# bpp/bpp

Hardware: AMD Instinct MI355X
Metric: MCMC iterations/sec (A00) + site-lnL updates/sec, 10k loci, 1/2/4/8 GPU (higher is better)
Workload: dtype f64; 1 GPU; C2: A00, 10000 loci x 1000 sites, 4 taxa, JC69, 1 rate cat; 10000 loci on rank 0, 5.2 patterns/locus; parallelism=1 GPU, moves=program

## Files before the change

### bpp_amd/api.py

```python
import ctypes as C
import os
import numpy as np

HERE = os.path.dirname(os.path.abspath(__file__))
LIB_PATH = os.path.join(HERE, "libbpp_amd.so")

DATA_DNA, DATA_AA = 0, 1
MODEL_JC69, MODEL_GTR, MODEL_LG = 0, 7, 10
ATTRIB_ARCH_HIP = 1 << 6
SCALE_BUFFER_NONE = -1
PARAM_FREQS, PARAM_SUBST, PARAM_RATES = 1, 2, 4


class BpaError(RuntimeError):
    pass


class Op(C.Structure):
    _fields_ = [("parent_clv", C.c_uint32), ("parent_scaler", C.c_int32),
                ("left_clv", C.c_uint32), ("left_pmatrix", C.c_uint32), ("left_scaler", C.c_int32),
                ("right_clv", C.c_uint32), ("right_pmatrix", C.c_uint32), ("right_scaler", C.c_int32)]


OP_DTYPE = np.dtype([("parent_clv", "<u4"), ("parent_scaler", "<i4"), ("left_clv", "<u4"),
# ... 25 lines not shown
        return _lib
    if not os.path.exists(LIB_PATH):
        raise BpaError(f"{LIB_PATH} is missing: run `python -m bpp_amd.build` (hipcc, gfx950). "
                       "bpp_amd has no CPU fallback.")
    L = C.CDLL(LIB_PATH)
    vp, u, i, d = C.c_void_p, C.c_uint, C.c_int, C.c_double
    dp, up = C.POINTER(C.c_double), C.POINTER(C.c_uint)
    sig = {
        "bpa_version": (C.c_char_p, []),
        "bpa_last_error": (C.c_char_p, []),
        "bpa_experimental_build": (i, []),
        "bpa_device_count": (i, []),
        "bpa_engine_create": (vp, [i, vp]),
        "bpa_engine_destroy": (None, [vp]),
        "bpa_engine_synchronize": (i, [vp]),
        "bpa_engine_set_options": (None, [vp, i, d]),
        "bpa_locus_create": (vp, [vp] + [u] * 11),
        "bpa_locus_destroy": (None, [vp]),
        "bpa_set_tip_states": (i, [vp, u, up, C.c_char_p]),
        "bpa_set_pattern_weights": (None, [vp, up]),
        "bpa_set_frequencies": (None, [vp, u, dp]),
        "bpa_set_subst_params": (None, [vp, u, dp]),
        "bpa_set_category_rates": (None, [vp, dp]),
        "bpa_set_category_weights": (None, [vp, dp]),
        "bpa_set_param_indices": (None, [vp, up]),
        "bpa_set_diploid": (i, [vp, i, C.POINTER(C.c_ulong), C.POINTER(C.c_ulong), C.c_ulong, up]),
        "bpa_map_nt": (up, []),
        "bpa_map_aa": (up, []),
        "bpa_locus_update_matrices": (i, [vp, up, dp, u]),
        "bpa_locus_update_partials": (i, [vp, C.POINTER(Op), u]),
        "bpa_locus_root_loglikelihood": (d, [vp, u, i, up, dp]),
        "bpa_locus_update_all_matrices": (i, [vp, C.POINTER(GTreeView), dp]),
        "bpa_locus_update_all_partials": (i, [vp, C.POINTER(GTreeView)]),
        "bpa_core_update_pmatrix": (i, [vp, C.POINTER(dp), u, u, dp, dp, up, up, C.POINTER(dp),
                                        C.POINTER(dp), C.POINTER(dp), u, u]),
        "bpa_update_eigen": (i, [vp, dp, dp, dp, dp, dp, u]),
        "bpa_compute_gamma_cats": (i, [d, d, u, dp]),
        "bpa_compress_site_patterns": (i, [C.POINTER(C.c_char_p), up, i, C.POINTER(i), i, up]),
        "bpa_locus_get_clv": (i, [vp, u, dp]),
        "bpa_locus_set_clv": (i, [vp, u, dp]),
        "bpa_locus_get_pmatrix": (i, [vp, u, dp]),
        "bpa_locus_set_pmatrix": (i, [vp, u, dp]),
        "bpa_locus_get_scaler": (i, [vp, u, up]),
        "bpa_locus_set_scaler": (i, [vp, u, up]),
        "bpa_locus_get_eigen": (i, [vp, u, dp, dp, dp]),
        "bpa_locus_get_category_rates": (i, [vp, dp]),
        "bpa_plan_create": (vp, [vp, C.POINTER(Batch)]),
        "bpa_plan_destroy": (None, [vp]),
        "bpa_plan_set_lengths": (i, [vp, dp]),
        "bpa_plan_launch": (i, [vp]),
        "bpa_plans_launch": (i, [C.POINTER(vp), u]),
        "bpa_plan_get_lnl": (i, [vp, dp]),
        "bpa_plan_lnl_device": (vp, [vp]),
        "bpa_plan_enable_sum": (i, [vp, vp]),
        "bpa_plan_get_sum": (i, [vp, dp]),
        "bpa_plan_enable_partial_sums": (i, [vp, vp, C.POINTER(C.c_uint)]),
        "bpa_p2p_create": (vp, [vp, i, i, u, vp]),
        "bpa_p2p_connect": (i, [vp, vp]),
        "bpa_p2p_allreduce": (i, [vp, vp, u]),
        "bpa_p2p_status": (i, [vp]),
        "bpa_p2p_set_timeout": (None, [vp, u]),
        "bpa_plans_launch_exchange": (i, [vp, u, vp, vp, u]),
        "bpa_p2p_destroy": (None, [vp]),
        "bpa_batch_evaluate": (i, [vp, C.POINTER(Batch), dp]),
        "bpa_batch_begin": (i, [vp, C.POINTER(Batch)]),
        "bpa_batch_fill": (i, [vp, C.POINTER(Batch), u, u]),
        "bpa_batch_end": (i, [vp, C.POINTER(Batch), dp]),
        "bpa_batch_end_async": (i, [vp, C.POINTER(Batch)]),
        "bpa_batch_wait": (i, [vp, dp]),
        "bpa_engine_stage": (vp, [vp, vp, C.c_size_t]),
        "bpa_plan_set_params": (i, [vp, i, dp]),
        "bpa_plan_set_params_device": (i, [vp, i, vp]),
        "bpa_plan_work": (i, [vp, dp, dp, dp, C.POINTER(C.c_ulong), C.POINTER(C.c_ulong)]),
        "bpa_sampler_create": (vp, [vp, C.POINTER(vp), u, C.c_ulong]),
        "bpa_sampler_destroy": (None, [vp]),
        "bpa_sampler_set_tree": (i, [vp, u, C.POINTER(i), C.POINTER(i), dp, i]),
        "bpa_sampler_set_species_tree": (i, [vp, i, C.POINTER(i), dp, dp]),
        "bpa_sampler_set_tip_species": (i, [vp, u, C.POINTER(i)]),
        "bpa_sampler_set_finetune": (None, [vp, d, d, d, d]),
        "bpa_finetune_onestep": (d, [d, d]),
        "bpa_sampler_adapt_finetune": (i, [vp, dp, dp]),
        "bpa_sampler_burnin": (i, [vp, u, dp]),
        "bpa_burnin_schedule": (u, [u, C.POINTER(u), u]),
        "bpa_sampler_set_tau_prior": (None, [vp, d, d]),
        "bpa_sampler_set_theta_prior": (None, [vp, d, d, d]),
        "bpa_sampler_get_thetas": (i, [vp, dp]),
        "bpa_sampler_set_allreduce": (i, [vp, vp, vp, vp, u]),
        "bpa_sampler_get_taus": (i, [vp, dp]),
        "bpa_sampler_get_tree_msc": (i, [vp, u, C.POINTER(i), dp]),
        "bpa_sampler_initialize": (i, [vp]),
        "bpa_sampler_iterate": (i, [vp, u]),
        "bpa_sampler_get_tree": (i, [vp, u, C.POINTER(i), C.POINTER(i), C.POINTER(i), dp, C.POINTER(i),
                                     C.POINTER(i), C.POINTER(i), dp]),
        "bpa_sampler_summary": (i, [vp, dp, C.POINTER(C.c_ulong), C.POINTER(C.c_ulong), C.POINTER(C.c_ulong)]),
        "bpa_sampler_enable_timing": (i, [vp, u]),
        "bpa_sampler_set_subst_model": (i, [vp, u, dp, dp, d]),
        "bpa_sampler_get_subst_model": (i, [vp, u, dp, dp, dp]),
        "bpa_sampler_set_subst_moves": (None, [vp, d, d, d, d, d]),
        "bpa_sampler_set_locus_rates": (i, [vp, dp]),
        "bpa_sampler_get_locus_rates": (i, [vp, dp, dp]),
        "bpa_sampler_set_locusrate_moves": (i, [vp, d, d, d, d, d, d]),
        "bpa_sampler_locusrate_counters": (i, [vp, C.POINTER(C.c_ulong), C.POINTER(C.c_ulong)]),
        "bpa_sampler_timing": (i, [vp, dp, C.POINTER(C.c_ulong), dp, C.POINTER(C.c_ulong)]),
        "bpa_sampler_work": (i, [vp, dp, C.POINTER(C.c_ulong), C.POINTER(C.c_ulong), C.POINTER(C.c_ulong)]),
        "bpa_sampler_kind": (i, [vp]),
        "bpa_sampler_streams": (i, [vp]),
        "bpa_sampler_set_p2p": (i, [vp, vp, u]),
        "bpa_sampler_set_proposal_kernel": (i, [vp, i]),
        "bpa_sampler_set_program_moves": (i, [vp, i, d]),
        "bpa_sampler_gibbs_counters": (i, [vp, C.POINTER(C.c_ulong), C.POINTER(C.c_ulong)]),
        "bpa_engine_enable_timing": (None, [vp, i]),
        "bpa_engine_set_timing_stride": (None, [vp, u]),
        "bpa_engine_timing": (i, [vp, dp, dp, dp, C.POINTER(C.c_ulong)]),
        "bpa_engine_timing_work": (i, [vp, C.POINTER(C.c_ulong), dp]),
        "bpa_engine_timing_work_codes": (i, [vp, dp]),
        "bpa_plan_work_codes": (i, [vp, dp]),
    }
    for name, (res, args) in sig.items():
        f = getattr(L, name)
        f.restype, f.argtypes = res, args
    _lib = L
    return L


EXPORTED = ["bpa_version", "bpa_last_error", "bpa_experimental_build", "bpa_device_count", "bpa_engine_create",
            "bpa_engine_destroy", "bpa_engine_synchronize", "bpa_engine_set_options",
            "bpa_locus_create", "bpa_locus_destroy", "bpa_set_tip_states",
            "bpa_set_pattern_weights", "bpa_set_frequencies", "bpa_set_subst_params",
            "bpa_set_category_rates", "bpa_set_category_weights", "bpa_set_param_indices",
            "bpa_set_diploid", "bpa_map_nt", "bpa_map_aa", "bpa_locus_update_matrices",
            "bpa_locus_update_partials", "bpa_locus_root_loglikelihood",
            "bpa_locus_update_all_matrices", "bpa_locus_update_all_partials",
            "bpa_core_update_pmatrix", "bpa_update_eigen", "bpa_compute_gamma_cats",
            "bpa_compress_site_patterns", "bpa_locus_get_clv", "bpa_locus_set_clv",
            "bpa_locus_get_pmatrix", "bpa_locus_set_pmatrix", "bpa_locus_get_scaler", "bpa_locus_set_scaler",
            "bpa_locus_get_eigen", "bpa_locus_get_category_rates", "bpa_plan_create", "bpa_plan_destroy", "bpa_plan_set_lengths",
            "bpa_plan_launch", "bpa_plan_get_lnl", "bpa_plan_lnl_device", "bpa_batch_evaluate", "bpa_batch_begin", "bpa_batch_fill", "bpa_batch_end", "bpa_batch_end_async", "bpa_batch_wait",
            "bpa_plan_enable_sum", "bpa_plan_enable_partial_sums", "bpa_plan_get_sum",
            "bpa_p2p_create", "bpa_p2p_connect", "bpa_p2p_allreduce", "bpa_p2p_status", "bpa_p2p_destroy", "bpa_p2p_set_timeout", "bpa_plans_launch_exchange", "bpa_plans_launch",
            "bpa_plan_set_params", "bpa_plan_set_params_device", "bpa_engine_stage",
            "bpa_plan_work", "bpa_engine_enable_timing", "bpa_engine_timing", "bpa_engine_set_timing_stride", "bpa_engine_timing_work", "bpa_engine_timing_work_codes", "bpa_plan_work_codes",
            "bpa_sampler_create", "bpa_sampler_destroy", "bpa_sampler_set_tree", "bpa_sampler_initialize",
            "bpa_sampler_set_species_tree", "bpa_sampler_set_tip_species", "bpa_sampler_set_finetune",
            "bpa_finetune_onestep", "bpa_sampler_adapt_finetune", "bpa_sampler_burnin", "bpa_burnin_schedule",
            "bpa_sampler_set_tau_prior", "bpa_sampler_get_taus", "bpa_sampler_get_tree_msc",
            "bpa_sampler_set_theta_prior", "bpa_sampler_get_thetas", "bpa_sampler_set_allreduce",
            "bpa_sampler_iterate", "bpa_sampler_get_tree", "bpa_sampler_summary",
            "bpa_sampler_enable_timing", "bpa_sampler_timing", "bpa_sampler_work", "bpa_sampler_kind", "bpa_sampler_streams", "bpa_sampler_set_p2p", "bpa_sampler_set_proposal_kernel",
            "bpa_sampler_set_program_moves", "bpa_sampler_gibbs_counters",
            "bpa_sampler_set_subst_model", "bpa_sampler_get_subst_model", "bpa_sampler_set_subst_moves",
            "bpa_sampler_set_locus_rates", "bpa_sampler_get_locus_rates", "bpa_sampler_set_locusrate_moves", "bpa_sampler_locusrate_counters"]


def _err():
    return lib().bpa_last_error().decode()


def _chk(ok):
    if not ok:
        raise BpaError(_err())


def _dp(a):
    return a.ctypes.data_as(C.POINTER(C.c_double))


def _up(a):
    return a.ctypes.data_as(C.POINTER(C.c_uint))


def _f64(a):
    return np.ascontiguousarray(a, dtype=np.float64)


def _u32(a):
    return np.ascontiguousarray(a, dtype=np.uint32)


def map_nt():
    return np.ctypeslib.as_array(lib().bpa_map_nt(), shape=(256,)).copy()


def map_aa():
    return np.ctypeslib.as_array(lib().bpa_map_aa(), shape=(256,)).copy()


def compute_gamma_cats(alpha, beta, categories):
    out = np.zeros(categories)
    _chk(lib().bpa_compute_gamma_cats(alpha, beta, categories, _dp(out)))
    return out


def compress_site_patterns(seqs, dna=True, jc69=False):
    L = lib()
    count, length = len(seqs), len(seqs[0])
    bufs = [C.create_string_buffer(s.encode() if isinstance(s, str) else s, length + 1) for s in seqs]
    arr = (C.c_char_p * count)(*[C.cast(b, C.c_char_p) for b in bufs])
    ln = C.c_int(length)
    w = np.zeros(length, dtype=np.uint32)
    n = L.bpa_compress_site_patterns(arr, L.bpa_map_nt() if dna else L.bpa_map_aa(), count,
                                     C.byref(ln), int(jc69), _up(w))
    if not n:
        raise BpaError("compress_site_patterns failed")
    return [b.raw[:n].decode() for b in bufs], w[:n].copy()


class Engine:

    def __init__(self, device=0, stream=None):
        L = lib()
        self.h = L.bpa_engine_create(device, stream)
        if not self.h:
            raise BpaError(_err())
        self.loci = []

    def set_options(self, usedata=1, bfbeta=1.0):
        lib().bpa_engine_set_options(self.h, int(usedata), float(bfbeta))

    def stage(self, array):
        return _stage(self, array)

    def synchronize(self):
        _chk(lib().bpa_engine_synchronize(self.h))

    def enable_timing(self, on=True, stride=1):
        lib().bpa_engine_set_timing_stride(self.h, int(stride))
        lib().bpa_engine_enable_timing(self.h, int(on))
# ... 617 lines not shown
```

### bpp_amd/csrc/sampler.hpp

```cpp
#pragma once
#include "bpp_amd_host.h"

namespace smp {

constexpr int MAXTIPS = 8;
constexpr int MAXN    = 16;
constexpr int MAXBUF  = 2*(MAXTIPS - 1);
constexpr int MAXPM   = 2*(2*MAXTIPS - 2);
constexpr int MAXPOP  = 16;
constexpr int TPB     = 16;
constexpr int BS      = 64;

struct Tree
{
  int8_t   left[MAXN], right[MAXN], parent[MAXN], clv[MAXN], pmat[MAXN], pop[MAXN];
  double   time[MAXN];
  double   lnl, logpr;
  a00_rng_t rng;
  int32_t  root, tips;
  uint32_t proposals, accepted;
  uint32_t sw_nupd, sw_nbr;
  uint32_t al_nupd, al_nbr, al_neval, pad_;
};
static_assert(sizeof(Tree) % 16 == 0 && offsetof(Tree, lnl) % 16 == 0, "Tree is copied as uint4");
// ... 980 lines not shown
  double * wg_part = nullptr; unsigned long long * stamps = nullptr; int * dec_err = nullptr;
  bool fuse_decision = false;
  DevBuf<int8_t> pop_nc;
  smp::Species sp{};
  bool has_theta[smp::MAXPOP] = {};
  struct Timed { hipEvent_t e0, e1; int kind; };
  std::vector<Timed> timed;
  unsigned timing_stride = 0, timing_phase = 0;
  double timed_ms[2] = {0, 0}; unsigned long timed_n[2] = {0, 0};
  bpa_allreduce_fn allreduce = nullptr;
  void * allreduce_ctx = nullptr;
  double * sum_ext = nullptr;
  unsigned locus_offset = 0;
  std::vector<unsigned> stream_index;
  struct bpa_composite * comp = nullptr;
  std::vector<double> h_taus;
  std::vector<smp::Tree> h_trees;
  bool generic = false;
  std::vector<gsm::GTree> g_trees;
  DevBuf<gsm::GTree> g_dev, g_undo;
  DevBuf<gsm::GLocus> g_loc;
  DevBuf<double> g_lnl, g_lnlcur, g_hast, g_logpr, g_delta, g_site, g_len, g_lograt;
  DevBuf<double> g_t2h3, g_progout;
  DevBuf<gsm::GDecState> g_dst; DevBuf<double> g_dsum; bool gp_dev = false;
  hipEvent_t gp_pace[4] = {nullptr, nullptr, nullptr, nullptr}; unsigned long gp_pace_n = 0;
  unsigned long long gp_seq = 0;
  double * gp_pin = nullptr, * gp_pin_dev = nullptr;
  DevBuf<uint32_t> g_arrive;
  long long gp_k[smp::MAXPOP] = {}; double gp_T[smp::MAXPOP] = {}; bool gp_ok = false, gp_pre_valid = false; double gp_pre_window = 0;
  double gp_tau[smp::MAXPOP] = {}, gp_theta[smp::MAXPOP] = {}; bool gp_mirror = false;
  unsigned long long gp_pj[10] = {}, gp_pj_base[4] = {};
  bool g_split = false, g_forked = false;
  static constexpr int GPARTS = 4;
  unsigned g_np = 1, g_pi[GPARTS + 1] = {}, g_ps[GPARTS + 1] = {}, g_pb[GPARTS + 1] = {}, g_pt[GPARTS + 1] = {};
  hipStream_t g_st[GPARTS] = {nullptr, nullptr, nullptr, nullptr};
  hipEvent_t g_ev_fork = nullptr, g_ev_join[GPARTS] = {nullptr, nullptr, nullptr, nullptr};
  int env_parts = 0;
  DevBuf<uint8_t> g_active;
  DevBuf<uint4> g_recs;
  DevBuf<MatRec2> g_mat2;
  DevBuf<uint32_t> g_bmo;
  unsigned g_units = 0, g_maxmat = 0, g_pend = 0, g_npat = 0, g_rmax = 1, g_pack_epoch = 0;
  bool g_alljc = true;
  bool big = false;
  std::vector<gbig::BTree> b_trees;
  DevBuf<gbig::BTree> b_dev, b_undo;
  DevBuf<uint32_t> b_thr;
  bool g_s20 = false;
  unsigned g_ntiles = 0, g_maxops = 0;
  DevBuf<OpDev> g_ops20;
  DevBuf<uint32_t> g_oprng, g_root20, g_mtask, g_mpm, g_tlocus, g_tpat, g_ttask, g_tn0;
  DevBuf<int32_t> g_rscaler;
  std::vector<double> g_sm_host;
  DevBuf<double> g_sm, g_sm_old;
  DevBuf<uint32_t> g_ids;
  double g_ft[3] = {0, 0, 0}, g_alpha_a = 1, g_alpha_b = 1;
  unsigned g_pend_mode = 0, g_pend_k = 0;
  std::vector<double> g_mui_host;
  gsm::GLrState g_lr_host{1.0, 0.0, 0ull, 0ull};
  DevBuf<double> g_mui, g_mui_old;
  DevBuf<gsm::GLrState> g_lr;
  double g_lr_ft[2] = {0, 0}, g_a_mui = 0, g_a_mubar = 0, g_b_mubar = 0;
  bool g_eigen_dirty = false;
  bool g_level_eval = false;
  bool g_root_stale = false;
  bool g_pm_fused = false;
  unsigned long g_evals = 0;
  unsigned nblocks = 0, epoch = 0;
  bool logpr_stale = false;
  uint32_t env_dbg = 0; int env_gage = -1, env_gspr = -1; bool env_trace = false, env_nomix = false;
  int env_fusea = -1; bool env_noeigfuse = false, env_fusepm = true, env_pmgroup = true, env_hostdec = false, env_rootstore = false; int env_chain = -1, env_pinout = 2;
  long env_inject = 0; uint32_t env_inject_bit = 1024u; long v2_launch_no = 0;
  bool mix_pending = false;
  a00_rng_t grng = 0;
  unsigned long seed = 0, launches = 0, sweeps = 0;
  bool uploaded = false;
  uint32_t h_counters[4] = {0, 0, 0, 0};
  bool host_current = false;
  bool v2_ok = false, env_v1 = false;
  int v2_nt = 0;
  int v2_retries = 0;
  bool v2_prog = false;
  unsigned v2_nwaves = 0, v2_nwg = 0, v2_lwaves = 0;
  size_t v2_lds = 0;
  DevBuf<uint32_t> v2_wave_off;
  DevBuf<smp2::Loc> v2_loc;
  DevBuf<uint2> v2_pat;
  DevBuf<unsigned long long> v2_xbuf;
  DevBuf<a00_rng_t> v2_grng;
  DevBuf<int> v2_err;
  DevBuf<unsigned long long> v2_pj;
  DevBuf<double> v2_prof, v2_declog;
  DevBuf<smp::Species> v2_sp;
  smp::Species v2_sp_sent{};
  struct V2Launch { a00_rng_t grng_before; unsigned chunk; bool mix_pending, logpr_stale; };
  std::vector<V2Launch> v2_log;
  bool kernel_bpp = false, v2_grng_sent = false;
  bpa_p2p * p2p = nullptr;
  unsigned long v2_iters = 0;
};

static bpa_sampler * comp_create(bpa_engine_t * e, bpa_locus_t * const * loci, unsigned nloci, unsigned long seed, bool * plain);
static void comp_destroy(bpa_sampler * s);
static int comp_invalidate(bpa_sampler * s);
static int comp_upload(bpa_sampler * s);
static int comp_set_allreduce(bpa_sampler * s, bpa_allreduce_fn fn, void * ctx, double * device_sum, unsigned first_locus);
static int comp_run(bpa_sampler * s, int what, unsigned n);
static int comp_summary(bpa_sampler * s, double * total_lnl, unsigned long * proposals, unsigned long * accepted, unsigned long * launches);
static int comp_timing(bpa_sampler * s, double * sweep_ms, unsigned long * sweep_launches, double * allloci_ms, unsigned long * allloci_launches);
static int comp_work(bpa_sampler * s, double * bytes, unsigned long * node_updates, unsigned long * pattern_updates, unsigned long * sweeps);
static bpa_sampler * comp_part(bpa_sampler * s, unsigned i, unsigned * j);
static bpa_sampler * comp_part0(bpa_sampler * s);
template <class F> static int comp_each(bpa_sampler * s, F f);
#define COMP_FAIL(msg) do { if (s->comp) return fail(msg); } while (0)

static bpa_sampler * sampler_create_plain(bpa_engine_t * e, bpa_locus_t * const * loci, unsigned nloci, unsigned long seed);
extern "C" bpa_sampler_t * bpa_sampler_create(bpa_engine_t * e, bpa_locus_t * const * loci, unsigned nloci,
                                              unsigned long seed)
{
  if (!e || !loci || !nloci) { fail("bpa_sampler_create: null argument"); return nullptr; }
  std::lock_guard<std::recursive_mutex> lock_(e->mtx);
  bool plain = true;
  bpa_sampler * c = comp_create(e, loci, nloci, seed, &plain);
  if (c || !plain) return c;
  return sampler_create_plain(e, loci, nloci, seed);
}

static bpa_sampler * sampler_create_plain(bpa_engine_t * e, bpa_locus_t * const * loci, unsigned nloci, unsigned long seed)
{
  bpa_sampler * s = new bpa_sampler();
  s->eng = e; s->nloci = nloci; s->seed = seed; s->grng = a00_rng_seed(seed, A00_GLOBAL_STREAM);
  s->sp.theta_slide_prob = 0.1;
  s->loci.assign(loci, loci + nloci);
  bool fits_sweep = !smp_env_generic(), fits_generic = true, all_jc = true, all_kl = true;
  unsigned n20 = 0, nbig = 0;
  const bool force_big = smp_env_big();
  for (unsigned i = 0; i < nloci; ++i)
  {
    const bpa_locus * l = loci[i];
    const bool counts = l && l->eng == e && l->alive && l->tips >= 2 && l->clv_buffers == 2*(l->tips - 1) && l->prob_matrices == 2*(2*l->tips - 2);
    const bool wants_big = counts && l->states == 4 && (force_big || l->tips > (unsigned)gsm::NT || l->scale_buffers != 0 || l->dev.unphased_length);
    if (wants_big)
    {
      if (l->tips > (unsigned)gbig::BT || (l->scale_buffers != 0 && l->scale_buffers != 2*(l->tips - 1)))
      {
        fail("bpa_sampler_create: a locus of the big-tree sampler has <= 64 tips and no or 2 (tips - 1) scale buffers (method.c:4110-4146)");
        delete s; return nullptr;
      }
      ++nbig; s->maxtips = std::max(s->maxtips, l->tips); s->g_rmax = std::max(s->g_rmax, l->rate_cats);
      continue;
    }
    const bool base = counts && (l->states == 4 || l->states == 20) && l->scale_buffers == 0 && !l->dev.unphased_length;
    if (!base)
    {
      fail("bpa_sampler_create: loci must be 4- or 20-state (20-state: without scalers, not diploid), with the buffer counts of method.c:4110-4146");
      delete s; return nullptr;
    }
    if (l->states == 20) { ++n20; fits_sweep = false; fits_generic = fits_generic && l->tips <= (unsigned)gsm::NT && l->rate_cats <= 4; all_jc = false;
                           s->maxtips = std::max(s->maxtips, l->tips); s->g_rmax = std::max(s->g_rmax, l->rate_cats); continue; }
    fits_sweep = fits_sweep && l->rate_cats == 1 && l->dev.model == 0 && l->tips <= (unsigned)smp::MAXTIPS && l->sites <= (unsigned)smp::BS;
    fits_generic = fits_generic && l->tips <= (unsigned)gsm::NT && l->rate_cats <= 8 && l->sites*l->rate_cats < PACK_BS;
    all_jc = all_jc && l->rate_cats == 1 && l->dev.model == 0;
    all_kl = all_kl && l->rate_cats > 1;
    s->maxtips = std::max(s->maxtips, l->tips);
    s->g_rmax = std::max(s->g_rmax, l->rate_cats);
  }
  if (nbig)
  {
    for (unsigned i = 0; i < nloci; ++i)
      if (loci[i]->states != 4 || loci[i]->tips > (unsigned)gbig::BT || (loci[i]->scale_buffers != 0 && loci[i]->scale_buffers != 2*(loci[i]->tips - 1)))
      {
        fail("bpa_sampler_create: the loci of a big-tree sampler are all 4-state with <= 64 tips");
        delete s; return nullptr;
      }
    for (unsigned i = 0; i < nloci; ++i) { s->maxtips = std::max(s->maxtips, loci[i]->tips); s->g_rmax = std::max(s->g_rmax, loci[i]->rate_cats); }
    s->big = true;
    s->b_trees.assign(nloci, gbig::BTree{});
  }
  else if (n20)
  {
    if (n20 != nloci || !fits_generic)
    {
      fail("bpa_sampler_create: 20-state loci go together (no 4-state locus in the same sampler), with <= 16 tips and <= 4 rate categories");
      delete s; return nullptr;
    }
    s->generic = true; s->g_alljc = false; s->g_s20 = true;
    s->g_trees.assign(nloci, gsm::GTree{});
  }
  else if (!fits_sweep)
  {
    if (!fits_generic || !(all_jc || all_kl))
    {
      fail("bpa_sampler_create: beyond the sweep kernel (JC69, 1 rate category, <= 8 tips, <= 64 patterns) the loci must all be JC69 with "
           "one rate category or all have several categories, with <= 16 tips and < 256 patterns x categories");
      delete s; return nullptr;
    }
    s->generic = true; s->g_alljc = all_jc;
    s->g_trees.assign(nloci, gsm::GTree{});
  }
  s->h_trees.assign(nloci, smp::Tree{});
  if (const char * dv = getenv("BPA_SMP_DBG")) s->env_dbg = (uint32_t)atoi(dv);
  if (const char * st = BPA_EXP_SWITCH("BPA_SMP_STEPS")) { unsigned g = 0, q = 0; if (sscanf(st, "%u,%u", &g, &q) == 2) { s->env_gage = (int)g; s->env_gspr = (int)q; } }
  s->env_trace = getenv("BPA_SMP_TRACE") != nullptr; s->env_nomix = BPA_EXP_SWITCH("BPA_SMP_NOMIX") != nullptr;
  if (const char * inj = getenv("BPA_SMP_INJECT")) { s->env_inject = atol(inj); s->env_inject_bit = strstr(inj, ",w") ? 2048u : 1024u; }
  s->fuse_decision = BPA_EXP_SWITCH("BPA_SMP_FUSE") != nullptr;
  { const char * v;
    v = BPA_EXP_SWITCH("BPA_GS_FUSEA");     s->env_fusea = v ? (v[0] == '1' ? 1 : 0) : -1;
    v = BPA_EXP_SWITCH("BPA_GS_FUSEPM");    s->env_fusepm = !(v && v[0] == '0');
    v = BPA_EXP_SWITCH("BPA_S20_PMGROUP");  s->env_pmgroup = !(v && v[0] == '0');
    v = BPA_EXP_SWITCH("BPA_GS_PARTS");    s->env_parts = v ? atoi(v) : 0;
    s->env_noeigfuse = BPA_EXP_SWITCH("BPA_GS_NOEIGFUSE") != nullptr;
    v = getenv("BPA_GS_CHAIN");     s->env_chain = v ? (v[0] != '0' ? 1 : 0) : -1;
    v = BPA_EXP_SWITCH("BPA_GS_PINOUT");    s->env_pinout = v ? (v[0] == '0' ? 0 : v[0] == '1' ? 1 : 2) : 2;
    s->env_hostdec = getenv("BPA_GS_HOSTDEC") != nullptr;
    s->env_rootstore = BPA_EXP_SWITCH("BPA_GS_ROOTSTORE") != nullptr; }
  s->env_v1 = getenv("BPA_SMP_V1") != nullptr;
  s->sp.ft_gage = 0.004; s->sp.ft_gspr = 0.004; s->sp.ft_tau = 0.001; s->sp.ft_mix = 0.3;
  return s;
}

static int sampler_download(bpa_sampler * s);
extern "C" void bpa_sampler_destroy(bpa_sampler_t * s)
{
  if (!s) return;
  std::lock_guard<std::recursive_mutex> lock_(s->eng->mtx);
  if (s->comp) comp_destroy(s);
  (void)set_device(s->eng);
  if (s->generic && s->uploaded && s->g_root_stale && s->g_pack_epoch == s->eng->pack_epoch && !sampler_download(s)) fprintf(stderr, "[bpp_amd] bpa_sampler_destroy: the loci's root buffers could not be brought level (%s)\n", bpa_last_error());
  (void)hipStreamSynchronize(s->eng->stream);
  for (auto & t : s->timed) { (void)hipEventDestroy(t.e0); (void)hipEventDestroy(t.e1); }
  s->blk_task_off.free(); s->lane_rec.free(); s->task_rec.free(); s->flag.free();
  s->counters.free(); s->trees.free(); s->snap.free(); s->mix_delta.free(); s->mix_sum.free(); s->taus.free(); s->pop_t2h.free(); s->theta_sums.free(); s->pop_nc.free(); s->lograt.free(); s->uc.free();
  for (int p_ = 1; p_ < bpa_sampler::GPARTS; ++p_)
  {
    if (s->g_st[p_]) { (void)hipStreamSynchronize(s->g_st[p_]); (void)hipStreamDestroy(s->g_st[p_]); s->g_st[p_] = nullptr; }
    if (s->g_ev_join[p_]) { (void)hipEventDestroy(s->g_ev_join[p_]); s->g_ev_join[p_] = nullptr; }
  }
  if (s->g_ev_fork) { (void)hipEventDestroy(s->g_ev_fork); s->g_ev_fork = nullptr; }
  s->g_t2h3.free(); s->g_progout.free(); s->g_arrive.free(); s->gp_mirror = false; s->g_dst.free(); s->g_dsum.free();
  if (s->gp_pin) { (void)hipHostFree(s->gp_pin); s->gp_pin = s->gp_pin_dev = nullptr; }
  for (auto & ev : s->gp_pace) if (ev) { (void)hipEventDestroy(ev); ev = nullptr; }
  s->g_dev.free(); s->g_undo.free(); s->g_loc.free(); s->g_lnl.free(); s->g_lnlcur.free(); s->g_hast.free(); s->g_logpr.free(); s->g_delta.free(); s->g_site.free();
  s->g_len.free(); s->g_lograt.free(); s->g_active.free(); s->g_recs.free(); s->g_mat2.free(); s->g_bmo.free();
  s->g_sm.free(); s->g_sm_old.free(); s->g_ids.free();
  s->g_mui.free(); s->g_mui_old.free(); s->g_lr.free();
  s->b_dev.free(); s->b_undo.free(); s->b_thr.free();
  s->g_ops20.free(); s->g_oprng.free(); s->g_root20.free(); s->g_mtask.free(); s->g_mpm.free(); s->g_tlocus.free(); s->g_tpat.free(); s->g_ttask.free(); s->g_tn0.free(); s->g_rscaler.free();
  s->v2_wave_off.free(); s->v2_loc.free(); s->v2_pat.free(); s->v2_xbuf.free(); s->v2_grng.free(); s->v2_err.free(); s->v2_prof.free(); s->v2_declog.free(); s->v2_sp.free();
  delete s;
}

static int sampler_download(bpa_sampler * s);
static bool v2_wants_prog(const bpa_sampler * s);
static int sampler_invalidate(bpa_sampler * s)
{
  if (s->uploaded)
  {
    bpa_engine * e = s->eng;
    if (!set_device(e) || !sampler_download(s)) return 0;
    HIPCHK(hipMemcpy(s->h_taus.data(), s->taus.p, s->h_taus.size()*sizeof(double), hipMemcpyDeviceToHost));
    HIPCHK(hipMemcpy(s->h_counters, s->counters.p, sizeof s->h_counters, hipMemcpyDeviceToHost));
  }
  s->uploaded = false; s->host_current = false;
  return 1;
}

template <class TR, int MAXNODES>
static int set_tree_fields(TR & t, int tips, const int * left, const int * right, const double * times, int root, a00_rng_t rng)
{
  const int n = 2*tips - 1;
  std::memset(&t, 0, sizeof(t));
  for (int k = 0; k < MAXNODES; ++k) { t.left[k] = t.right[k] = t.parent[k] = -1; t.clv[k] = t.pmat[k] = (int8_t)k; t.pop[k] = (int8_t)(k < tips ? k : -1); }
  for (int k = 0; k < n; ++k)
  {
    t.left[k] = (int8_t)left[k]; t.right[k] = (int8_t)right[k]; t.time[k] = times[k];
    if ((left[k] < 0) != (k < tips) || (right[k] < 0) != (k < tips) || left[k] >= n || right[k] >= n)
      return fail("bpa_sampler_set_tree: nodes 0..tips-1 are the tips (no children), the others have two");
    if (left[k] >= 0) { t.parent[left[k]] = (int8_t)k; t.parent[right[k]] = (int8_t)k; }
  }
  t.root = root; t.tips = tips; t.rng = rng; t.lnl = 0;
  return 1;
}

static unsigned stream_of(const bpa_sampler * s, unsigned i) { return s->stream_index.empty() ? s->locus_offset + i : s->stream_index[i]; }
static a00_rng_t stream_seed(const bpa_sampler * s, unsigned stream)
{
  const a00_rng_t z = a00_rng_seed(s->seed, stream);
  return s->kernel_bpp ? (a00_rng_t)(unsigned int)(z >> 16) : z;
}

extern "C" int bpa_sampler_set_proposal_kernel(bpa_sampler_t * s, int kind)
{
  std::lock_guard<std::recursive_mutex> lock_(s->eng->mtx);
  if (s->comp && kind != BPA_KERNEL_UNIFORM) return fail("bpa_sampler_set_proposal_kernel: loci of several kinds run the library's own proposal kernel (BPP's lives inside the persistent kernel's single launch)");
  if (s->comp) return 1;
  if (kind != BPA_KERNEL_UNIFORM && kind != BPA_KERNEL_BPP) return fail("bpa_sampler_set_proposal_kernel: BPA_KERNEL_UNIFORM or BPA_KERNEL_BPP");
  if (s->uploaded) return fail("bpa_sampler_set_proposal_kernel: before bpa_sampler_initialize (as a00_set_proposal_kernel)");
  s->kernel_bpp = kind == BPA_KERNEL_BPP;
  for (unsigned i = 0; i < s->nloci; ++i) (s->big ? s->b_trees[i].rng : s->generic ? s->g_trees[i].rng : s->h_trees[i].rng) = stream_seed(s, stream_of(s, i));
  s->grng = stream_seed(s, A00_GLOBAL_STREAM);
  s->v2_grng_sent = false;
  return 1;
}

extern "C" int bpa_sampler_set_program_moves(bpa_sampler_t * s, int on, double slide_prob)
{
  std::lock_guard<std::recursive_mutex> lock_(s->eng->mtx);
  if (s->comp) return on ? fail("bpa_sampler_set_program_moves: loci of several kinds run the library's own moves") : 1;
  if (on && !(slide_prob >= 0 && slide_prob <= 1)) return fail("bpa_sampler_set_program_moves: slide_prob is a probability");
  if (on && !s->kernel_bpp) return fail("bpa_sampler_set_program_moves: the program's moves draw from BPP's proposal kernel (bpa_sampler_set_proposal_kernel(s, BPA_KERNEL_BPP) first)");
  s->sp.program_moves = on ? 1 : 0;
  if (on) s->sp.theta_slide_prob = slide_prob;
  if (s->uploaded && s->v2_ok && v2_wants_prog(s) != s->v2_prog) return sampler_invalidate(s);
  return 1;
}

extern "C" int bpa_sampler_gibbs_counters(bpa_sampler_t * s, unsigned long * proposals, unsigned long * accepted)
{
  std::lock_guard<std::recursive_mutex> lock_(s->eng->mtx);
  if (s->comp) { if (proposals) *proposals = 0; if (accepted) *accepted = 0; return 1; }
  if (!sampler_download(s)) return 0;
  uint32_t c[4];
  HIPCHK(hipMemcpy(c, s->counters.p, sizeof c, hipMemcpyDeviceToHost));
  if (proposals) *proposals = c[2];
  if (accepted) *accepted = c[3];
  return 1;
}

extern "C" int bpa_sampler_set_tree(bpa_sampler_t * s, unsigned i, const int * left, const int * right,
                                    const double * times, int root)
{
  std::lock_guard<std::recursive_mutex> lock_(s->eng->mtx);
  if (s->comp) { unsigned j; bpa_sampler * p = comp_part(s, i, &j); if (!p) return fail("bpa_sampler_set_tree: locus index out of range"); return comp_invalidate(s) && bpa_sampler_set_tree(p, j, left, right, times, root); }
  if (i >= s->nloci) return fail("bpa_sampler_set_tree: locus index out of range");
  const int tips = (int)s->loci[i]->tips;
  const a00_rng_t rng = stream_seed(s, stream_of(s, i));
  if (!sampler_invalidate(s)) return 0;
  if (s->big) return set_tree_fields<gbig::BTree, gbig::BN>(s->b_trees[i], tips, left, right, times, root, rng);
  if (s->generic) return set_tree_fields<gsm::GTree, gsm::NN>(s->g_trees[i], tips, left, right, times, root, rng);
  return set_tree_fields<smp::Tree, smp::MAXN>(s->h_trees[i], tips, left, right, times, root, rng);
}

template <class TR>
static int assign_pops_host(const bpa_sampler * s, TR & t)
{
  const int n = 2*t.tips - 1;
  std::vector<int> order;
  for (int k = t.tips; k < n; ++k) order.push_back(k);
  std::stable_sort(order.begin(), order.end(), [&](int a, int b) { return t.time[a] < t.time[b]; });
  for (int k = 0; k < t.tips; ++k) if (t.pop[k] < 0 || t.pop[k] >= s->sp.S) return fail("bpa_sampler: tip species out of range");
  for (int v : order)
  {
    int c = t.pop[t.left[v]];
    while (!((s->sp.anc[t.pop[t.right[v]]] >> c) & 1u)) c = s->sp.parent[c];
    if (t.time[v] < s->h_taus[c]) return fail("bpa_sampler: a gene-tree node is younger than the divergence of its descendants' species");
    while (s->sp.parent[c] >= 0 && s->h_taus[s->sp.parent[c]] <= t.time[v]) c = s->sp.parent[c];
    t.pop[v] = (int8_t)c;
  }
  return 1;
}
static int gs_upload(bpa_sampler * s);
static int sampler_launch(bpa_sampler * s, unsigned mode, double mix_c, double mix_lnc, unsigned tau_q, double tau_u, double dec_uacc);
static int gs_initialize(bpa_sampler * s);
static int gs_iterate(bpa_sampler * s, unsigned iterations);
static int gs_download(bpa_sampler * s);
static int gb_upload(bpa_sampler * s);
static int gb_initialize(bpa_sampler * s);
static int gb_iterate(bpa_sampler * s, unsigned iterations);
static int gb_download(bpa_sampler * s);

template <int NT> static size_t v2_lds_base(bool prog)
{
  return ((sizeof(smp2::WgLDS<NT>) + 15) & ~(size_t)15) + sizeof(smp2::WaveLDS<NT>)*(size_t)(smp2::Cfg<NT>::WAVES - (prog ? 1 : 0));
}
static bool v2_wants_prog(const bpa_sampler * s)
{
  if (!(s->kernel_bpp && s->sp.program_moves && s->sp.theta_alpha > 0 && s->sp.npop > s->sp.S)) return false;
  for (int p = 0; p < s->sp.npop; ++p) if (s->has_theta[p]) return true;
  return false;
}
static int sampler_upload_v2(bpa_sampler * s, const std::vector<smp::TaskRec> & task_rec)
{
  s->v2_ok = false;
  if (s->env_v1 || s->generic || s->big) return 1;
  const unsigned T = s->nloci;
  const int npop = s->sp.npop;
  if (s->maxtips > 8 || npop > 15) return 1;
  const int NT = (s->maxtips <= 4 && npop <= 7) ? 4 : 8;
  for (unsigned i = 0; i < T; ++i)
  {
    const smp::Tree & t = s->h_trees[i];
    const int n = 2*t.tips - 1, inner = t.tips - 1, edges = 2*t.tips - 2;
    if (t.root != n - 1) return 1;
    for (int k = 0; k < n; ++k)
    {
      if (k < t.tips ? t.clv[k] != k : (t.clv[k] != k && t.clv[k] != k + inner)) return 1;
      if (k != t.root && t.pmat[k] != k && t.pmat[k] != k + edges) return 1;
    }
  }
  const unsigned G = NT == 4 ? 8 : 16, LPW = 64/G, WAVES = NT == 4 ? (unsigned)smp2::Cfg<4>::WAVES : (unsigned)smp2::Cfg<8>::WAVES;
  std::vector<uint32_t> woff{0};
  std::vector<smp2::Loc> loc(T);
  std::vector<uint2> pat;
  unsigned cnt = 0, used = 0;
  for (unsigned t = 0; t < T; ++t)
  {
    const bpa_locus * l = s->loci[t];
    const unsigned np = l->sites, tips = l->tips;
    if (cnt == LPW || used + np > 64u) { woff.push_back(t); cnt = 0; used = 0; }
    ++cnt; used += np;
    smp2::Loc & L = loc[t];
    const smp::TaskRec & r = task_rec[t];
    L.clv = r.clv; L.pmat = r.pmat; L.rate = r.rate; L.rw = r.rw; L.f0 = r.f0; L.f1 = r.f1; L.f2 = r.f2; L.f3 = r.f3;
    L.np = np; L.tips = tips; L.pat_off = (uint32_t)pat.size(); L.pad = 0;
    for (int p = 0; p < 16; ++p) L.gl[p] = r.gl[p];
    for (unsigned n = 0; n < np; ++n)
    {
      uint32_t codes = 0;
      for (unsigned tip = 0; tip < tips; ++tip) codes |= (uint32_t)(l->tipcodes[(size_t)tip*np + n] & 15u) << (4*tip);
      pat.push_back(make_uint2(l->weights[n], codes));
    }
  }
  woff.push_back(T);
  const bool prog = v2_wants_prog(s);
  hipDeviceProp_t prop;
  HIPCHK(hipGetDeviceProperties(&prop, s->eng->device));
  const unsigned nwaves = (unsigned)woff.size() - 1;
  const unsigned LMAX = WAVES - (prog ? 1u : 0u), ncu = (unsigned)std::max(prop.multiProcessorCount, 1);
  unsigned LWAVES = (LMAX > 4u && nwaves <= 4u*ncu) ? 4u : LMAX;
  if (const char * ev = BPA_EXP_SWITCH("BPA_SMP_LWAVES")) { const unsigned v = (unsigned)std::atoi(ev); if (v >= 1 && v <= LMAX) LWAVES = v; }
  const unsigned nwg = (nwaves + LWAVES - 1)/LWAVES;
  const size_t base = NT == 4 ? v2_lds_base<4>(prog) : v2_lds_base<8>(prog);
  const size_t lds_max = std::min<size_t>((size_t)prop.sharedMemPerBlock > 65536 ? (size_t)prop.sharedMemPerBlock : 160*1024, 160*1024) - 256;
  if (base > lds_max) return 1;
  const unsigned per_cu = (unsigned)std::min<size_t>(std::max<size_t>(lds_max/base, 1), 8/WAVES ? 8/WAVES : 1);
  if (nwg > per_cu*(unsigned)prop.multiProcessorCount) return 1;
  s->v2_lds = base;
  s->v2_nt = NT; s->v2_nwaves = nwaves; s->v2_nwg = nwg; s->v2_prog = prog; s->v2_lwaves = LWAVES;
  const int zero2v[3] = {0, 0, 0};
  if (!upload(s->v2_wave_off, woff.data(), woff.size()) || !upload(s->v2_loc, loc.data(), loc.size()) ||
      !upload(s->v2_pat, pat.data(), pat.size()) || !s->v2_xbuf.reserve((size_t)2*smp2::XN) || !s->v2_grng.reserve(1) ||
      !upload(s->v2_err, zero2v, 3) || !s->v2_prof.reserve(40 + (size_t)nwg) || !s->v2_declog.reserve(4*2048) || !s->v2_sp.reserve(1) || !s->v2_pj.reserve(16))
    return 0;
  HIPCHK(hipMemset(s->v2_pj.p, 0, 16*sizeof(unsigned long long)));
  HIPCHK(hipMemset(s->v2_prof.p, 0, (40 + (size_t)nwg)*sizeof(double)));
  {
    void (*k0)(const smp2::Args) = NT == 4 ? smp2::iter_kernel<4, false> : smp2::iter_kernel<8, false>;
    void (*k1)(const smp2::Args) = NT == 4 ? smp2::iter_kernel<4, true> : smp2::iter_kernel<8, true>;
    HIPCHK(hipFuncSetAttribute(reinterpret_cast<const void *>(k0), hipFuncAttributeMaxDynamicSharedMemorySize, (int)s->v2_lds));
    HIPCHK(hipFuncSetAttribute(reinterpret_cast<const void *>(k1), hipFuncAttributeMaxDynamicSharedMemorySize, (int)s->v2_lds));
    void (*k2)(const smp2::Args) = NT == 4 ? smp2::iter_kernel<4, true, true> : smp2::iter_kernel<8, true, true>;
    HIPCHK(hipFuncSetAttribute(reinterpret_cast<const void *>(k2), hipFuncAttributeMaxDynamicSharedMemorySize, (int)s->v2_lds));
  }
  std::memset(&s->v2_sp_sent, 0xff, sizeof s->v2_sp_sent);
  s->v2_ok = true;
  return 1;
}

static int sampler_upload(bpa_sampler * s)
{
  bpa_engine * e = s->eng;
  if (s->uploaded) return 1;
  if (!set_device(e) || !flush(e)) return 0;
  const unsigned T = s->nloci;
  if (!s->sp.npop) return fail("bpa_sampler: set the species tree first (bpa_sampler_set_species_tree)");
  if (s->big) return gb_upload(s);
  if (s->generic) return gs_upload(s);
  for (unsigned i = 0; i < T; ++i) if (!assign_pops_host(s, s->h_trees[i])) return 0;
  for (int p = 0; p < smp::MAXPOP; ++p) s->has_theta[p] = p >= s->sp.S && p < s->sp.npop;
  for (unsigned i = 0; i < T; ++i)
  {
    int cnt[smp::MAXPOP] = {0};
    const smp::Tree & t = s->h_trees[i];
    for (int k = 0; k < t.tips; ++k) if (++cnt[t.pop[k]] >= 2) s->has_theta[t.pop[k]] = true;
  }
  std::vector<uint32_t> blk_off{0};
  std::vector<smp::LaneRec> lane_rec;
  std::vector<smp::TaskRec> task_rec(T);
  const smp::LaneRec idle{0xffffffffu, 0, 0, 0, nullptr, nullptr};
  unsigned used = 0, ntask = 0;
  for (unsigned t = 0; t < T; ++t)
  {
    const bpa_locus * l = s->loci[t];
    const unsigned np = l->sites, tips = l->tips;
    if (used + np > (unsigned)smp::BS || ntask == (unsigned)smp::TPB)
    { lane_rec.resize(blk_off.size()*smp::BS, idle); blk_off.push_back(t); used = 0; ntask = 0; }
    for (unsigned n = 0; n < np; ++n)
    {
      uint32_t codes = 0;
      for (unsigned tip = 0; tip < tips; ++tip) codes |= (uint32_t)(l->tipcodes[(size_t)tip*np + n] & 15u) << (4*tip);
      lane_rec.push_back(smp::LaneRec{t, l->weights[n], codes, n | np << 8 | tips << 16, l->dev.clv + (size_t)n*4, l->dev.pmat});
    }
    used += np; ++ntask;
    smp::TaskRec & r = task_rec[t];
    const double * f = l->par.data() + par_matrix(1, 4, 0) + pm_freqs(4);
    r.clv = l->dev.clv; r.pmat = l->dev.pmat; r.rate = l->par[par_rates(1)]; r.rw = l->par[par_rate_weights(1)];
    r.f0 = f[0]; r.f1 = f[1]; r.f2 = f[2]; r.f3 = f[3];
    const smp::Tree & tr = s->h_trees[t];
    for (int p = 0; p < smp::MAXPOP; ++p) r.gl[p] = r.nin[p] = 0;
    for (unsigned k = 0; k < tips; ++k)
    {
      r.nin[tr.pop[k]]++;
      for (int q = tr.pop[k]; q >= 0; q = s->sp.parent[q]) r.gl[q]++;
    }
  }
  lane_rec.resize(blk_off.size()*smp::BS, idle);
  blk_off.push_back(T);
  s->nblocks = (unsigned)blk_off.size() - 1;
  uint32_t zero2[2] = {0, 0};
  if (!upload(s->blk_task_off, blk_off.data(), blk_off.size()) ||
      !upload(s->lane_rec, lane_rec.data(), lane_rec.size()) || !upload(s->task_rec, task_rec.data(), T) ||
      !upload(s->trees, s->h_trees.data(), T) || !upload(s->snap, s->h_trees.data(), T) ||
      !upload(s->flag, zero2, 1) || !upload(s->counters, s->h_counters, 4) || !s->mix_delta.reserve(T) || !s->mix_sum.reserve(1) ||
      !upload(s->taus, s->h_taus.data(), s->h_taus.size()) || !s->pop_t2h.reserve((size_t)T*smp::MAXPOP) ||
      !s->pop_nc.reserve((size_t)T*smp::MAXPOP) || !s->theta_sums.reserve(smp::MAXPOP) || !s->lograt.reserve(smp::MAXN*smp::MAXN))
    return 0;
  {
    const size_t nb = ((size_t)s->nblocks + 1)*8;
    s->uc.free();
    if (!s->uc.reserve(2*nb + 64)) return fail("bpa_sampler: out of (uncached) device memory");
    s->wg_part = reinterpret_cast<double *>(s->uc.p);
    s->stamps = reinterpret_cast<unsigned long long *>(reinterpret_cast<char *>(s->uc.p) + nb);
    s->dec_err = reinterpret_cast<int *>(reinterpret_cast<char *>(s->uc.p) + 2*nb);
  }
  if (s->allreduce)
  {
    double m[smp::MAXPOP];
    for (int p = 0; p < smp::MAXPOP; ++p) m[p] = s->has_theta[p] ? 1.0 : 0.0;
    double * ar = s->sum_ext ? s->sum_ext : s->theta_sums.p;
    HIPCHK(hipMemcpyAsync(ar, m, sizeof m, hipMemcpyHostToDevice, e->stream));
    if (!s->allreduce(s->allreduce_ctx, ar, (unsigned)smp::MAXPOP, (void *)e->stream)) return fail("bpa_sampler: the all-reduce callback failed");
    HIPCHK(hipMemcpyAsync(m, ar, sizeof m, hipMemcpyDeviceToHost, e->stream));
    HIPCHK(hipStreamSynchronize(e->stream));
    for (int p = 0; p < smp::MAXPOP; ++p) s->has_theta[p] = m[p] > 0.5;
  }
// ... 312 lines not shown
extern "C" int bpa_sampler_get_taus(bpa_sampler_t * s, double * taus)
{
  bpa_engine * e = s->eng;
  std::lock_guard<std::recursive_mutex> lock_(e->mtx);
  if (s->comp) return comp_upload(s) && bpa_sampler_get_taus(comp_part0(s), taus);
  if (!set_device(e)) return 0;
  const size_t np = (size_t)s->sp.npop;
  if (!s->uploaded) { for (size_t i = 0; i < np; ++i) taus[i] = s->h_taus[i]; return (int)np; }
  HIPCHK(hipStreamSynchronize(e->stream));
  HIPCHK(hipMemcpy(taus, s->taus.p, np*sizeof(double), hipMemcpyDeviceToHost));
  return (int)np;
}

extern "C" int bpa_sampler_initialize(bpa_sampler_t * s)
{
  std::lock_guard<std::recursive_mutex> lock_(s->eng->mtx);
  if (s->comp) return comp_run(s, 0, 0);
  if (!sampler_upload(s)) return 0;
  s->host_current = false;
  if (s->big) return gb_initialize(s);
  if (s->generic) return gs_initialize(s);
  return sampler_launch(s, 3, 1.0);
}

static int sampler_sum(bpa_sampler * s)
{
  bpa_engine * e = s->eng;
  double * out = s->sum_ext ? s->sum_ext : s->mix_sum.p;
  hipLaunchKernelGGL(lnl_sum_kernel, dim3(1), dim3(1024), 0, e->stream, s->wg_part, s->nblocks, out);
  HIPCHK(hipGetLastError());
  if (s->allreduce && !s->allreduce(s->allreduce_ctx, out, 1u, (void *)e->stream)) return fail("bpa_sampler: the all-reduce callback failed");
  return 1;
}

static int sampler_decide(bpa_sampler * s, double uacc, int tau_q, int theta_p, double win_u, double mix_c, double mix_lnc)
{
  bpa_engine * e = s->eng;
  s->epoch++;
  if (!s->allreduce)
    hipLaunchKernelGGL(smp::sum_decide_kernel, dim3(1), dim3(1024), 0, e->stream, s->wg_part, s->nblocks, uacc, s->epoch,
                       s->flag.p, s->counters.p, s->taus.p, s->sp, tau_q, theta_p, win_u, mix_c, mix_lnc);
  else
  {
    if (!sampler_sum(s)) return 0;
    hipLaunchKernelGGL(smp::decide_kernel, dim3(1), dim3(1), 0, e->stream, s->sum_ext ? s->sum_ext : s->mix_sum.p, uacc, s->epoch,
                       s->flag.p, s->counters.p, s->taus.p, s->sp, tau_q, theta_p, win_u, mix_c, mix_lnc);
  }
  HIPCHK(hipGetLastError());
  s->launches += s->allreduce ? 2 : 1;
  s->mix_pending = true;
  return 1;
}

extern "C" int bpa_sampler_set_allreduce(bpa_sampler_t * s, bpa_allreduce_fn fn, void * ctx, double * device_sum,
                                         unsigned first_locus)
{
  std::lock_guard<std::recursive_mutex> lock_(s->eng->mtx);
  if (s->comp) return comp_set_allreduce(s, fn, ctx, device_sum, first_locus);
  s->allreduce = fn; s->allreduce_ctx = ctx; s->sum_ext = device_sum;
  if (first_locus != s->locus_offset)
  {
    if (!sampler_invalidate(s)) return 0;
    s->locus_offset = first_locus;
    for (unsigned i = 0; i < s->nloci; ++i)
      (s->big ? s->b_trees[i].rng : s->generic ? s->g_trees[i].rng : s->h_trees[i].rng) = stream_seed(s, first_locus + i);
    s->uploaded = false;
  }
  return 1;
}

static int sampler_iterate_v2(bpa_sampler * s, unsigned iterations, bool in_kernel_allloci)
{
  bpa_engine * e = s->eng;
  const int npop = s->sp.npop, S = s->sp.S;
  uint32_t theta_mask = 0;
  if (s->sp.theta_alpha > 0) for (int p = 0; p < npop; ++p) if (s->has_theta[p]) theta_mask |= 1u << p;
  const bool allloci = in_kernel_allloci && !s->env_nomix;
  const bool program = s->v2_prog;
  const unsigned XV = (unsigned)smp2::XV;
  const bool merged = program;
  const unsigned x_theta = !theta_mask ? 0u : program ? (2u*(unsigned)__builtin_popcount(theta_mask) + (merged ? 5u : 0u) + XV - 1u)/XV : ((unsigned)npop + XV - 1u)/XV;
  const unsigned x_per_iter = allloci ? x_theta + (unsigned)(npop - S) - (merged ? 1u : 0u) + 1u : 0u;
  const unsigned draws_per_iter = allloci ? 2u*(unsigned)__builtin_popcount(theta_mask) + 2u*(unsigned)(npop - S) + 2u : 0u;
  void (*kern)(const smp2::Args) = s->v2_prog   ? (s->v2_nt == 4 ? smp2::iter_kernel<4, true, true> : smp2::iter_kernel<8, true, true>)
                                 : s->kernel_bpp ? (s->v2_nt == 4 ? smp2::iter_kernel<4, true> : smp2::iter_kernel<8, true>)
                                                 : (s->v2_nt == 4 ? smp2::iter_kernel<4, false> : smp2::iter_kernel<8, false>);
  const unsigned bs = s->v2_nt == 4 ? smp2::Cfg<4>::BS : smp2::Cfg<8>::BS;
  while (iterations)
  {
    const unsigned chunk = std::min(iterations, 4096u);
    smp2::Args a{};
    a.wave_off = s->v2_wave_off.p; a.loc = s->v2_loc.p; a.pat = s->v2_pat.p; a.trees = s->trees.p; a.taus = s->taus.p;
    if (s->v2_log.size() >= 65536u && !sampler_download(s)) return 0;
    s->v2_log.push_back({s->grng, chunk, s->mix_pending, s->logpr_stale});
    a.snap = s->snap.p; a.mix_flag = s->flag.p; a.epoch = s->mix_pending ? s->epoch : 0u; a.refresh_logpr = s->logpr_stale ? 1u : 0u;
    s->mix_pending = false; s->logpr_stale = false;
    a.counters = s->counters.p; a.lograt = s->lograt.p; a.pop_nc = s->pop_nc.p; a.pop_t2h = s->pop_t2h.p;
    a.ntasks = s->nloci; a.nwaves = s->v2_nwaves; a.nwg = s->v2_nwg; a.lwaves = s->v2_lwaves; a.xbuf = s->v2_xbuf.p;
    a.err = s->v2_err.p; a.grng = s->v2_grng.p; a.niter = chunk; a.pj = s->v2_pj.p;
    a.nsteps_gage = s->maxtips - 1; a.nsteps_gspr = 2*s->maxtips - 2;
    if (s->env_gage >= 0) { a.nsteps_gage = (uint32_t)s->env_gage; a.nsteps_gspr = (uint32_t)s->env_gspr; }
    a.theta_mask = theta_mask; a.do_allloci = allloci ? 1u : 0u; a.dbg = s->env_dbg;
    if (allloci && ++s->v2_launch_no == s->env_inject) a.dbg |= s->env_inject_bit;
    if (s->p2p && allloci)
    {
      a.peers = s->p2p->d_peer.p; a.mail = s->p2p->mail; a.rank = s->p2p->rank; a.world = s->p2p->world; a.slot_bytes = s->p2p->slot_bytes;
      a.seq0 = s->p2p->seq; a.spin_limit = s->p2p->spin_limit; a.p2p_err = s->p2p->d_err.p;
      s->p2p->seq += (unsigned long long)chunk*x_per_iter;
    }
    else { a.world = 1; a.rank = 0; }
    a.bfbeta = e->usedata ? e->bfbeta : 0.0; a.prof = s->v2_prof.p; a.declog = s->v2_declog.p; a.sp = s->v2_sp.p;
    if (std::memcmp(&s->v2_sp_sent, &s->sp, sizeof(smp::Species)) != 0)
    {
      HIPCHK(hipMemcpyAsync(s->v2_sp.p, &s->sp, sizeof(smp::Species), hipMemcpyHostToDevice, e->stream));
      s->v2_sp_sent = s->sp;
    }
    if (s->env_dbg & 256u) HIPCHK(hipMemsetAsync(s->v2_declog.p, 0, 4*2048*sizeof(double), e->stream));
    if (allloci)
    {
      if (!s->kernel_bpp || !s->v2_grng_sent)
        HIPCHK(hipMemcpyAsync(s->v2_grng.p, &s->grng, sizeof(a00_rng_t), hipMemcpyHostToDevice, e->stream));
      s->v2_grng_sent = true;
      HIPCHK(hipMemsetAsync(s->v2_xbuf.p, 0, (size_t)2*smp2::XN*sizeof(unsigned long long), e->stream));
    }
    if (s->timing_stride && (s->timing_phase++ % s->timing_stride) == 0)
    {
      if (s->timed.size() >= 4096 && !sampler_timing_drain(s)) return 0;
      bpa_sampler::Timed t{nullptr, nullptr, 0};
      HIPCHK(hipEventCreate(&t.e0)); HIPCHK(hipEventCreate(&t.e1));
      hipExtLaunchKernelGGL(kern, dim3(s->v2_nwg), dim3(bs), s->v2_lds, e->stream, t.e0, t.e1, 0, a);
      s->timed.push_back(t);
    }
    else
      hipLaunchKernelGGL(kern, dim3(s->v2_nwg), dim3(bs), s->v2_lds, e->stream, a);
    HIPCHK(hipGetLastError());
    if (!s->kernel_bpp) for (unsigned long k = 0; k < (unsigned long)chunk*draws_per_iter; ++k) (void)a00_rndu(&s->grng);
    s->launches++; s->sweeps += chunk; s->v2_iters += chunk;
    iterations -= chunk;
  }
  return 1;
}

extern "C" int bpa_sampler_set_p2p(bpa_sampler_t * s, bpa_p2p_t * p, unsigned first_locus)
{
  std::lock_guard<std::recursive_mutex> lock_(s->eng->mtx);
  COMP_FAIL("bpa_sampler_set_p2p: loci of several kinds exchange through bpa_sampler_set_allreduce (the mailboxes are read by the persistent kernel's single launch)");
  if (p && (!p->connected || p->eng != s->eng)) return fail("bpa_sampler_set_p2p: connect the exchange first (same engine)");
  if (p && p->nmax < 16u) return fail("bpa_sampler_set_p2p: the mailboxes must hold at least 16 values");
  if (p && (s->generic || s->big)) return fail("bpa_sampler_set_p2p: the in-kernel exchange needs the persistent kernel (JC69 loci of <= 8 tips, <= 64 patterns); use bpa_sampler_set_allreduce");
  if (!sampler_invalidate(s)) return 0;
  s->p2p = p;
  if (first_locus != s->locus_offset)
  {
    s->locus_offset = first_locus;
    for (unsigned i = 0; i < s->nloci; ++i)
    {
      const a00_rng_t r = stream_seed(s, first_locus + i);
      if (s->big) s->b_trees[i].rng = r; else if (s->generic) s->g_trees[i].rng = r; else s->h_trees[i].rng = r;
    }
  }
  return 1;
}

extern "C" int bpa_sampler_iterate(bpa_sampler_t * s, unsigned iterations)
{
  bpa_engine * e = s->eng;
  std::lock_guard<std::recursive_mutex> lock_(e->mtx);
  if (s->comp) return comp_run(s, 1, iterations);
  if (s->generic && (s->g_lr_ft[0] > 0 || s->g_lr_ft[1] > 0) && (s->allreduce || s->p2p))
    return fail("bpa_sampler_iterate: the locus-rate moves run on one rank (an all-reduce callback or the mailboxes are installed: the sum of the rates over the ranks is not exchanged)");
  if (!sampler_upload(s)) return 0;
  s->host_current = false;
  if (s->big) return gb_iterate(s, iterations);
  if (s->generic) return gs_iterate(s, iterations);
  if (s->v2_ok && !s->allreduce && !s->env_trace) return sampler_iterate_v2(s, iterations, true);
  if (s->kernel_bpp) return fail("bpa_sampler: BPP's proposal kernel runs in the persistent iteration kernel only (one GPU, or several with bpa_sampler_set_p2p)");
  const bool v2_sweep = s->v2_ok && !s->env_trace;
  const bool fused = s->fuse_decision && !s->allreduce && !s->env_trace;
  for (unsigned it = 0; it < iterations; ++it)
  {
    if (v2_sweep) { if (!sampler_iterate_v2(s, 1, false)) return 0; }
    else
    {
      if (!sampler_launch(s, 0, 1.0)) return 0;
      s->sweeps++;
    }
    if (s->env_nomix) continue;
    if (s->sp.theta_alpha > 0)
    {
      smp::ThetaArgs ta{};
      for (int p = 0; p < s->sp.npop; ++p)
        if (s->has_theta[p]) { ta.on[p] = 1u; ta.win_u[p] = a00_rndu(&s->grng); ta.uacc[p] = a00_rndu(&s->grng); }
      if (!s->allreduce)
        hipLaunchKernelGGL(smp::theta_sum_decide_kernel, dim3(s->sp.npop), dim3(1024), 0, e->stream, s->pop_nc.p, s->pop_t2h.p,
                           s->nloci, s->taus.p, s->sp, ta, s->counters.p, (double *)nullptr, (const double *)nullptr, 1);
      else
      {
        hipLaunchKernelGGL(smp::theta_sum_decide_kernel, dim3(s->sp.npop), dim3(1024), 0, e->stream, s->pop_nc.p, s->pop_t2h.p,
                           s->nloci, s->taus.p, s->sp, ta, s->counters.p, s->theta_sums.p, (const double *)nullptr, 0);
        double * ar = s->sum_ext ? s->sum_ext : s->theta_sums.p;
        const size_t nb = (size_t)s->sp.npop*sizeof(double);
        if (ar != s->theta_sums.p) HIPCHK(hipMemcpyAsync(ar, s->theta_sums.p, nb, hipMemcpyDeviceToDevice, e->stream));
        if (!s->allreduce(s->allreduce_ctx, ar, (unsigned)s->sp.npop, (void *)e->stream)) return fail("bpa_sampler: the all-reduce callback failed");
        if (ar != s->theta_sums.p) HIPCHK(hipMemcpyAsync(s->theta_sums.p, ar, nb, hipMemcpyDeviceToDevice, e->stream));
        hipLaunchKernelGGL(smp::theta_sum_decide_kernel, dim3(s->sp.npop), dim3(1024), 0, e->stream, s->pop_nc.p, s->pop_t2h.p,
                           s->nloci, s->taus.p, s->sp, ta, s->counters.p, (double *)nullptr, (const double *)s->theta_sums.p, 1);
      }
      s->logpr_stale = true;
      HIPCHK(hipGetLastError());
      s->launches += 1;
    }
    for (int q = s->sp.S; q < s->sp.npop; ++q)
    {
      const double uprop = a00_rndu(&s->grng), uacc_t = a00_rndu(&s->grng);
      if (fused)
      {
        if (!sampler_launch(s, 4, 1.0, 0.0, (unsigned)q, uprop, uacc_t)) return 0;
        s->epoch++; s->mix_pending = true;
        continue;
      }
      if (!sampler_launch(s, 4, 1.0, 0.0, (unsigned)q, uprop)) return 0;
      if (!sampler_decide(s, uacc_t, q, -1, uprop, 1.0, 0.0)) return 0;
    }
    const double lnc = s->sp.ft_mix*(a00_rndu(&s->grng) - 0.5), c = std::exp(lnc);
    const double uacc = a00_rndu(&s->grng);
    if (fused)
    {
      if (!sampler_launch(s, 1, c, lnc, 0, 0.0, uacc)) return 0;
      s->epoch++; s->mix_pending = true;
      continue;
    }
    if (!sampler_launch(s, 1, c, lnc)) return 0;
    if (!sampler_decide(s, uacc, -1, -1, 0.0, c, lnc)) return 0;
  }
  return 1;
}

static int sampler_download(bpa_sampler * s)
{
  bpa_engine * e = s->eng;
  if (!sampler_upload(s)) return 0;
  if (s->host_current) return 1;
  if (s->big) { if (!gb_download(s)) return 0; s->host_current = true; return 1; }
  if (s->generic) { if (!gs_download(s)) return 0; s->host_current = true; return 1; }
  if (!sampler_launch(s, 2, 1.0)) return 0;
  HIPCHK(hipMemcpyAsync(s->h_trees.data(), s->trees.p, s->nloci*sizeof(smp::Tree), hipMemcpyDeviceToHost, e->stream));
  HIPCHK(hipStreamSynchronize(e->stream));
  int err = 0;
  HIPCHK(hipMemcpy(&err, s->dec_err, sizeof err, hipMemcpyDeviceToHost));
  if (err) return fail("bpa_sampler: an in-launch decision timed out waiting for a workgroup's sum (BPA_SMP_FUSE is set: unset it)");
  if (s->v2_ok)
  {
    if (s->env_dbg & 16u)
    {
      double pr[16]; HIPCHK(hipMemcpy(pr, s->v2_prof.p, sizeof pr, hipMemcpyDeviceToHost));
      fprintf(stderr, "[smp2] cycles of lane 0 of workgroup 0, last launch: propose %.0f evaluate %.0f decide %.0f theta %.0f tau %.0f mix %.0f | exchange: theta %.0f tau+mix %.0f | inside the exchanges: first barrier %.0f sums %.0f barrier %.0f arrival + poll %.0f last barrier %.0f | of theta / tau / mix: the decision's arithmetic after the totals %.0f %.0f, MIX's re-draws inside the wait %.0f\n",
              pr[0], pr[1], pr[2], pr[3], pr[4], pr[5], pr[6], pr[7], pr[8], pr[9], pr[10], pr[11], pr[12], pr[13], pr[14], pr[15]);
      double p2[24]; HIPCHK(hipMemcpy(p2, s->v2_prof.p + 16 + s->v2_nwg, sizeof p2, hipMemcpyDeviceToHost));
      fprintf(stderr, "[smp2] sweep cycles of the waves of workgroup 0:");
      for (int w = 0; w < 8; ++w) fprintf(stderr, " %.0f", p2[8 + w]);
      fprintf(stderr, "\n");
      if (s->v2_prog)
        fprintf(stderr, "[smp2] (program-moves kernel: the numbers above are the control wave's — before B1 | wait for the loci | push | poll | THETA decision | TAU decisions | MIX decision | next proposal)\n");
    }
    if (s->env_dbg & 256u)
    {
      std::vector<double> r(4*2048); HIPCHK(hipMemcpy(r.data(), s->v2_declog.p, r.size()*sizeof(double), hipMemcpyDeviceToHost));
      for (unsigned k = 1000; k < 2048; ++k) if (r[4*k] != 0) fprintf(stderr, "[smp2dbg] %u: %g %.17g %.17g %.17g\n", k, r[4*k], r[4*k+1], r[4*k+2], r[4*k+3]);
      for (unsigned k = 0; k < 1000 && r[4*k] != 0; ++k)
        fprintf(stderr, "[smp2] %s %d lnacc %.17g u %.17g -> %d\n", r[4*k] >= 300 ? "mix" : r[4*k] >= 200 ? "tau" : "theta",
                (int)r[4*k] % 100, r[4*k + 1], r[4*k + 2], (int)r[4*k + 3]);
    }
    if (s->env_dbg & 32u)
    {
      std::vector<double> w(s->v2_nwg); HIPCHK(hipMemcpy(w.data(), s->v2_prof.p + 16, w.size()*sizeof(double), hipMemcpyDeviceToHost));
      double mn = 1e300, mx = 0, sm = 0; unsigned imx = 0;
      for (unsigned i = 0; i < w.size(); ++i) { mn = std::min(mn, w[i]); if (w[i] > mx) { mx = w[i]; imx = i; } sm += w[i]; }
      fprintf(stderr, "[smp2] sweep cycles per workgroup, last launch: min %.0f mean %.0f max %.0f (workgroup %u of %u)\n", mn, sm/w.size(), mx, imx, s->v2_nwg);
    }
    int verr[3] = {0, 0, 0};
    HIPCHK(hipMemcpy(verr, s->v2_err.p, sizeof verr, hipMemcpyDeviceToHost));
    err = verr[0];
    if (!err && s->p2p) { HIPCHK(hipMemcpy(&err, s->p2p->d_err.p, sizeof err, hipMemcpyDeviceToHost)); if (err) return fail("bpa_sampler: the exchange between the GPUs timed out inside the persistent kernel (a rank is missing or slow; install an all-reduce callback instead)"); }
    if (err)
    {
      const int zero2[2] = {0, 0};
      HIPCHK(hipMemcpy(s->v2_err.p, zero2, sizeof zero2, hipMemcpyHostToDevice));
      if (s->p2p || verr[1] <= 0) return fail("bpa_sampler: the persistent iteration kernel timed out waiting for a workgroup's sum (is the device shared? BPA_SMP_V1=1 selects one launch per step)");
      fprintf(stderr, "[bpp_amd] the persistent iteration kernel timed out waiting for a workgroup (is the device shared?): %d iterations are run again\n", verr[1]);
      {
        long left = verr[1];
        while (left > 0 && !s->v2_log.empty())
        {
          const bpa_sampler::V2Launch l = s->v2_log.back(); s->v2_log.pop_back();
          left -= (long)l.chunk;
          s->launches--; s->sweeps -= l.chunk; s->v2_iters -= l.chunk;
          if (!s->kernel_bpp) s->grng = l.grng_before;
          s->mix_pending = l.mix_pending; s->logpr_stale = l.logpr_stale;
        }
        if (left != 0) return fail("bpa_sampler: the persistent kernel reports iterations it did not run that no launch of the log accounts for");
      }
      s->v2_log.clear();
      if (++s->v2_retries > 3)
      {
        if (s->kernel_bpp) return fail("bpa_sampler: the persistent iteration kernel keeps timing out (a shared device: its workgroups must all be resident at once) and BPP's proposal kernel has no other path");
        s->v2_ok = false;
      }
      if (!bpa_sampler_iterate(s, (unsigned)verr[1])) return 0;
      return sampler_download(s);
    }
    s->v2_retries = 0; s->v2_log.clear();
    if (verr[2])
    {
      const int z = 0;
      HIPCHK(hipMemcpy(s->v2_err.p + 2, &z, sizeof z, hipMemcpyHostToDevice));
      return fail("bpa_sampler: an all-loci step was ACCEPTED with a locus's term of 256 log units or more in its sum (the coarse companion accumulator: 2^-10 resolution); the chain is not to be trusted from there on");
    }
  }
  s->host_current = true;
  return 1;
}

extern "C" int bpa_sampler_get_tree(bpa_sampler_t * s, unsigned i, int * left, int * right, int * parent,
                                    double * times, int * clv, int * pmat, int * root, double * lnl)
{
  std::lock_guard<std::recursive_mutex> lock_(s->eng->mtx);
  if (s->comp) { unsigned j; bpa_sampler * p = comp_part(s, i, &j); if (!p) return fail("bpa_sampler_get_tree: locus index out of range"); return comp_upload(s) && bpa_sampler_get_tree(p, j, left, right, parent, times, clv, pmat, root, lnl); }
  if (i >= s->nloci) return fail("bpa_sampler_get_tree: locus index out of range");
  if (!sampler_download(s)) return 0;
  auto out = [&](const auto & t)
  {
    const int n = 2*t.tips - 1;
    for (int k = 0; k < n; ++k)
    {
      if (left) left[k] = t.left[k]; if (right) right[k] = t.right[k]; if (parent) parent[k] = t.parent[k];
      if (times) times[k] = t.time[k]; if (clv) clv[k] = t.clv[k]; if (pmat) pmat[k] = t.pmat[k];
    }
    if (root) *root = t.root;
    if (lnl) *lnl = t.lnl;
  };
  if (s->big) out(s->b_trees[i]); else if (s->generic) out(s->g_trees[i]); else out(s->h_trees[i]);
  return 1;
}

// ... 104 lines not shown
```

### bpp_amd/csrc/sweep2.hpp

```cpp
#pragma once

namespace smp2 {

using smp::Tree; using smp::Species; using smp::ByteArr; using smp::MAXPOP; using smp::MAXN;
using smp::rndu; using smp::reflect; using smp::msc_term; using smp::nth_bit; using smp::Op; using smp::make_op;

template <int NT> struct Cfg
{
  static constexpr int G     = NT <= 4 ? 8 : NT <= 8 ? 16 : 32;
  static constexpr int LPW   = 64/G;
  static constexpr int NN    = 2*NT;
  static constexpr int W     = NN/4;
  static constexpr int NBUF  = 2*(NT - 1);
  static constexpr int NPM   = 2*(2*NT - 2);
#ifndef SMP2_WAVES
#define SMP2_WAVES 8
#endif
  static constexpr int WAVES = NT <= 4 ? SMP2_WAVES : 4;
  static constexpr int BS    = 64*WAVES;
  static_assert(G == NN, "lane i of a group is node i");
};

struct Loc
{
  double * clv, * pmat;
  double rate, rw, f0, f1, f2, f3;
  uint32_t np, tips, pat_off, pad;
  int8_t gl[16];
};

struct Args
{
  const uint32_t * wave_off;
  const Loc * loc;
  const uint2 * pat;
  Tree * trees;
  const Tree * snap; const uint32_t * mix_flag; uint32_t epoch, refresh_logpr;
  double * taus;
  uint32_t * counters;
  const double * lograt;
  int8_t * pop_nc; double * pop_t2h;
  uint32_t ntasks, nwaves, nwg;
  uint32_t lwaves;
  unsigned long long * xbuf;
  int * err;
  a00_rng_t * grng;
  uint32_t niter, nsteps_gage, nsteps_gspr, theta_mask, do_allloci, dbg;
  double bfbeta;
  double * prof, * declog;
  unsigned char * const * peers; unsigned char * mail; int32_t rank, world; unsigned long long slot_bytes, seq0, spin_limit; int * p2p_err;
  const Species * sp;
  unsigned long long * pj;
};

constexpr int XN = 128;
constexpr int XV = 15;

template <int NT> struct Slot
{
  double time[Cfg<NT>::NN];
  double ab[Cfg<NT>::NPM][2];
  double contrib[Cfg<NT>::G], contrib_new[Cfg<NT>::G];
  double rate, rw, f[4];
};
template <int NT> struct WaveLDS
{
  double clv[Cfg<NT>::NBUF][64][4];
  double term[64];
  uint2  pat[64];
  Slot<NT> slot[Cfg<NT>::LPW];
};
struct PopFit { double k, T, a, b, c; };
struct Redraw { double tn, l2t, T, a, b, c; };
struct WgBase
{
  double tau[3*MAXPOP];
  double xtot[32];
  Species sp;
  struct { unsigned long long grng; uint32_t accm, rd_mask, acc_step, run_ok; double lnacc_step, lnacc_theta; double tn[16], l2t[16], lnacc[16]; } dec;
  PopFit pf[16];
  Redraw rd[16];
  struct { int32_t q, mix; double tq_old, tq_lo, tq_hi, tq_new, minf, maxf, lminf, lmaxf, mix_c, mix_lnc; } stepp;
};
template <int NT> struct WgLDS : WgBase
{
  double lograt[(2*NT)*(2*NT)];
  unsigned long long accfx[32];
  uint32_t anc[16];
  uint32_t abort_, bad_, xbad_, coarse_;
  unsigned long long xprev[2][XN];
  long long prof[24];
  long long wsweep[16];
  uint32_t xcoarse_, late_;
};

template <int G> __device__ __forceinline__ uint32_t gballot(bool p, uint32_t gbase)
{
  return (uint32_t)(__ballot(p) >> gbase) & (G >= 32 ? 0xffffffffu : ((1u << (G & 31)) - 1u));
}
__device__ __forceinline__ void wsync()
{
  __builtin_amdgcn_fence(__ATOMIC_ACQ_REL, "wavefront");
  __builtin_amdgcn_wave_barrier();
}

template <int NT> struct GTree
{
  ByteArr<Cfg<NT>::W> left, right, parent, pop;
  uint32_t cf, pf;
  int32_t root, tips;
  __device__ __forceinline__ int cidx(int i) const { return i + (((cf >> i) & 1u) ? tips - 1 : 0); }
  __device__ __forceinline__ int pidx(int i) const { return i + (((pf >> i) & 1u) ? 2*tips - 2 : 0); }
};

__device__ __forceinline__ uint32_t splat(int v) { return (uint32_t)(v & 0xff)*0x01010101u; }
__device__ __forceinline__ uint32_t byte_eq(uint32_t w, uint32_t s)
{
  const uint32_t x = w ^ s;
  const uint32_t z = ~(((x & 0x7f7f7f7fu) + 0x7f7f7f7fu) | x | 0x7f7f7f7fu);
  return (z - (z >> 7)) | z;
}
template <int NT> __device__ __forceinline__ void swap_ids(GTree<NT> & t, double * time, int a, int b)
{
  constexpr int W = Cfg<NT>::W;
  const uint32_t sa = splat(a), sb = splat(b), x = sa ^ sb;
#pragma unroll
  for (int k = 0; k < W; ++k)
  {
    t.left.w[k]   ^= x & (byte_eq(t.left.w[k], sa)   | byte_eq(t.left.w[k], sb));
    t.right.w[k]  ^= x & (byte_eq(t.right.w[k], sa)  | byte_eq(t.right.w[k], sb));
    t.parent.w[k] ^= x & (byte_eq(t.parent.w[k], sa) | byte_eq(t.parent.w[k], sb));
  }
  const int la = t.left[a], ra = t.right[a], pa = t.parent[a], qa = t.pop[a];
  const int lb = t.left[b], rb = t.right[b], pb = t.parent[b], qb = t.pop[b];
  t.left.set(a, lb); t.right.set(a, rb); t.parent.set(a, pb); t.pop.set(a, qb);
  t.left.set(b, la); t.right.set(b, ra); t.parent.set(b, pa); t.pop.set(b, qa);
  const double ta = time[a], tb = time[b];
  time[a] = tb; time[b] = ta;
  t.root = t.root == a ? b : t.root == b ? a : t.root;
}
template <int NT> __device__ __forceinline__ uint32_t path_mask(const GTree<NT> & t, int v)
{
  uint32_t m = 0;
#pragma unroll
  for (int d = 0; d < NT; ++d) { if (v >= 0) { m |= 1u << v; v = t.parent[v]; } }
  return m;
}

struct PopLane
{
  double tau, ptau, theta, l2t;
  int32_t parent;
  uint32_t anc, below;
};

struct Prop { uint32_t chain, brm, ndm; double hast; };

template <bool BPP> struct Stream
{
  a00_rng_t r;
  __device__ __forceinline__ double u()
  {
    if (!BPP) return rndu(&r);
    uint32_t z = (uint32_t)r*69069u + 1u;
    if (z == 0u) z = 12345671u;
    r = z;
    return (double)z*(1.0/4294967296.0);
  }
  __device__ __forceinline__ double window()
  {
    if (!BPP) return rndu(&r) - 0.5;
    const double uu = u() - 0.5;
    const double rr = log(1 - 2*fabs(uu))*0.70710678118654752440;
    const double lap = uu >= 0 ? -rr : rr;
    double v = 0.90 + lap*sqrt(1 - 0.90*0.90);
    if (u() < 0.5) v = -v;
// ... 287 lines not shown
    wg.dec.lnacc[lane] = lnacc_p; wg.dec.l2t[lane] = l2_p;
    if (apply_now && ((accm >> lane) & 1u)) { wg.tau[MAXPOP + lane] = tn; wg.tau[2*MAXPOP + lane] = l2_p; }
  }
  if (lane == 0) { wg.dec.accm = accm; wg.dec.run_ok = run_ok ? 1u : 0u; }
  __builtin_amdgcn_fence(__ATOMIC_ACQ_REL, "wavefront");
  __builtin_amdgcn_wave_barrier();
  return z;
}

__device__ __forceinline__ uint32_t prog_tau_decide(uint32_t z, uint32_t theta_mask, int q, int base, double lnacc0, bool prefit = false)
{
  WgBase & wg = wg_base();
  const uint32_t lane = threadIdx.x & 63u, pl16 = lane & 15u, role = lane >> 4;
  const double qnan = prog_qnan();
  constexpr double FX = 1099511627776.0, FXC = 1024.0;
  double lnacc = (wg.xtot[base] + wg.xtot[base + 1]*(FX/FXC)) + lnacc0;
  const int cl = wg.sp.left[q], cr = wg.sp.right[q];
  const bool run_ok = wg.dec.run_ok != 0u;
  const PopFit f = wg.pf[pl16];
  const bool aff = lane < 16u && ((int)lane == q || (int)lane == cl || (int)lane == cr);
  const bool have = aff && ((theta_mask >> pl16) & 1u) && run_ok;
  const double Cn = have ? wg.xtot[base + ((int)lane == q ? 2 : (int)lane == cl ? 3 : 4)] : qnan;
  double fa = qnan, fb = qnan, tn = qnan, l2t = 0;
  if (prefit) { if (have && Cn == Cn) { fa = wg.rd[pl16].a; fb = wg.rd[pl16].b; } }
  else if (have && Cn == Cn) a00_theta_conditional_invgamma_fast(wg.sp.theta_alpha, wg.sp.theta_beta, (long)f.k, Cn, &fa, &fb);
  const uint32_t rd_mask = (uint32_t)__ballot(have && fa == fa && f.a == f.a) & 0xffffu;
  double xl;
  const double s_fa = __shfl(fa, (int)pl16, 64), s_fb = __shfl(fb, (int)pl16, 64);
  const double g = draw_gammas(z, lane, (unsigned long long)q | ((unsigned long long)cl << 4) | ((unsigned long long)cr << 8), 3, rd_mask, fa, role == 1u ? s_fb : s_fa, xl);
  const double lb = __shfl(xl, 16 + (int)pl16, 64), la = __shfl(xl, 32 + (int)pl16, 64);
  const double c1 = fa*lb - lgamma_with_log(fa, la);
  if (lane < 16u && ((rd_mask >> pl16) & 1u)) tn = 1.0/(g/fb);
  const double x = redraw_ratio(wg, lane, f.k, tn, fa, fb, c1, Cn, f.a, f.b, f.c, f.T, l2t);
  for (int j = 0; j < 3; ++j)
  {
    const int p = j == 0 ? q : j == 1 ? cl : cr;
    if (!((theta_mask >> p) & 1u)) continue;
    const double xp = __shfl(x, p, 64);
    lnacc += run_ok && ((rd_mask >> p) & 1u) ? xp : qnan;
  }
  const bool accept = lnacc >= -1e-10 || prog_lcg(z) < exp(lnacc);
  if (lane < 16u) { Redraw & r = wg.rd[lane]; r.tn = tn; r.l2t = l2t; r.T = Cn; r.a = fa; r.b = fb; r.c = c1; }
  if (lane == 0) { wg.dec.acc_step = accept ? 1u : 0u; wg.dec.rd_mask = rd_mask; wg.dec.lnacc_step = lnacc; }
  __builtin_amdgcn_fence(__ATOMIC_ACQ_REL, "wavefront");
  __builtin_amdgcn_wave_barrier();
  return z;
}

__device__ __forceinline__ uint32_t prog_mix_redraw(uint32_t z, uint32_t theta_mask, double mix_c)
{
  WgBase & wg = wg_base();
  const uint32_t lane = threadIdx.x & 63u, pl16 = lane & 15u, role = lane >> 4;
  const int npop = wg.sp.npop, pm = (int)pl16;
  const double qnan = prog_qnan();
  const bool run_ok = wg.dec.run_ok != 0u;
  const PopFit f = wg.pf[pl16];
  const bool have = lane < 32u && pm < npop && ((theta_mask >> pm) & 1u) && run_ok;
  const double Ts = f.T*mix_c;
  double fa = qnan, fb = qnan, tn = qnan, l2t = 0;
  if (have) a00_theta_conditional_invgamma_fast(wg.sp.theta_alpha, wg.sp.theta_beta, (long)f.k, role == 0u ? Ts : Ts/mix_c, &fa, &fb);
  const double fao = __shfl(fa, 16 + pm, 64), fbo = __shfl(fb, 16 + pm, 64);
  const uint32_t rd_mask = (uint32_t)__ballot(lane < 16u && have && fa == fa && fao == fao) & 0xffffu;
  double xl;
  const double s_fa = __shfl(fa, pm, 64), s_fb = __shfl(fb, pm, 64);
  const double g = draw_gammas(z, lane, 0xfedcba9876543210ull, npop, rd_mask, fa, role == 1u ? s_fb : role == 2u ? s_fa : fbo, xl);
  const double lb = __shfl(xl, 16 + pm, 64), la = __shfl(xl, 32 + pm, 64), lbo = __shfl(xl, 48 + pm, 64), lao = log(fao);
  const double c1 = fa*lb - lgamma_with_log(fa, la), co = fao*lbo - lgamma_with_log(fao, lao);
  if (lane < 16u && ((rd_mask >> pl16) & 1u)) tn = 1.0/(g/fb);
  const double x = redraw_ratio(wg, lane, f.k, tn, fa, fb, c1, Ts, fao, fbo, co, f.T, l2t);
  double lnacc_theta = 0;
  for (int p = 0; p < npop; ++p)
    if ((theta_mask >> p) & 1u)
    {
      const double xp = __shfl(x, p, 64);
      lnacc_theta += run_ok && ((rd_mask >> p) & 1u) ? xp : qnan;
    }
  if (lane < 16u) { Redraw & r = wg.rd[lane]; r.tn = tn; r.l2t = l2t; r.T = Ts; r.a = fa; r.b = fb; r.c = c1; }
  if (lane == 0) { wg.dec.rd_mask = rd_mask; wg.dec.lnacc_theta = lnacc_theta; }
  __builtin_amdgcn_fence(__ATOMIC_ACQ_REL, "wavefront");
  __builtin_amdgcn_wave_barrier();
  return z;
}

template <int NT, bool BPP, bool PROG = false>
__global__ void __launch_bounds__(Cfg<NT>::BS) iter_kernel(const Args A)
{
  using C = Cfg<NT>;
  constexpr int G = C::G, LPW = C::LPW, NN = C::NN, W = C::W, NBUF = C::NBUF, NPM = C::NPM, WAVES = C::WAVES;
  extern __shared__ __attribute__((aligned(16))) unsigned char smem[];
  WgLDS<NT> & wg = *reinterpret_cast<WgLDS<NT> *>(smem);
  WaveLDS<NT> * wl_all = reinterpret_cast<WaveLDS<NT> *>(smem + ((sizeof(WgLDS<NT>) + 15) & ~(size_t)15));
  const uint32_t tid = threadIdx.x, wv = tid >> 6, lane = tid & 63u, b = blockIdx.x;
  const int li = (int)(lane & (uint32_t)(G - 1)); const uint32_t gbase = lane - (uint32_t)li, slot = lane/(uint32_t)G;
  WaveLDS<NT> & wl = wl_all[PROG ? (wv ? wv - 1u : 0u) : wv];
  Slot<NT> & S = wl.slot[slot];
  const uint32_t lw = PROG ? wv - 1u : wv;
  const uint32_t gw = lw < A.lwaves ? b*A.lwaves + lw : 0xffffffffu;
  {
    const uint32_t * src = reinterpret_cast<const uint32_t *>(A.sp);
    uint32_t * dst = reinterpret_cast<uint32_t *>(&wg.sp);
    for (uint32_t i = tid; i < sizeof(Species)/4; i += C::BS) dst[i] = src[i];
    if (tid < 24u) wg.prof[tid] = 0;
    if (tid < 16u) wg.wsweep[tid] = 0;
  }
  __syncthreads();
  const Species & SP = wg.sp;
  const int npop = SP.npop, nsp = SP.S;

  for (uint32_t i = tid; i < (uint32_t)(3*MAXPOP); i += C::BS) wg.tau[i] = A.taus[i];
  for (uint32_t i = tid; i < (uint32_t)((2*NT)*(2*NT)); i += C::BS) wg.lograt[i] = A.lograt[(i/(2*NT))*MAXN + i % (2*NT)];
  if (tid < 16u) wg.anc[tid] = tid < (uint32_t)MAXPOP ? (uint32_t)SP.anc[tid] : 0u;
  if (tid == 0) { wg.abort_ = __hip_atomic_load(A.err, __ATOMIC_RELAXED, __HIP_MEMORY_SCOPE_AGENT) != 0 ? 2u : 0u; wg.late_ = 0; wg.bad_ = 0; wg.xbad_ = 0; wg.coarse_ = 0; wg.xcoarse_ = 0; }
  if (tid < 32u) wg.accfx[tid] = 0ull;
  for (uint32_t i = tid; i < 2u*XN; i += C::BS) (&wg.xprev[0][0])[i] = 0ull;
  PopLane pl;
  {
    pl.parent = li < npop ? (int)SP.parent[li < MAXPOP ? li : 0] : -1;
    pl.anc = li < npop ? (uint32_t)SP.anc[li < MAXPOP ? li : 0] : 0u;
    uint32_t below = 0;
    for (int q2 = 0; q2 < npop; ++q2) if (q2 != li && (((uint32_t)SP.anc[q2] >> li) & 1u)) below |= 1u << q2;
    pl.below = li < npop ? below : 0u;
  }
  __syncthreads();
  if (wg.abort_ == 2u)
  {
    if (b == 0 && tid == 0) (void)atomicAdd(A.err + 1, (int)A.niter);
    return;
  }
  auto load_pop = [&]()
  {
    const int i = li < MAXPOP ? li : 0;
    pl.tau = wg.tau[i]; pl.theta = wg.tau[MAXPOP + i]; pl.l2t = wg.tau[2*MAXPOP + i];
    pl.ptau = pl.parent >= 0 ? wg.tau[pl.parent] : -1.0;
  };
  load_pop();
  Stream<BPP> grng{*A.grng};

  const bool prof_on = (A.dbg & 16u) && b == 0 && tid == 0;
  long long pf_t = prof_on ? clock64() : 0;
#define SMP2_TICK(i_) do { if (prof_on) { const long long t1_ = clock64(); wg.prof[i_] += t1_ - pf_t; pf_t = t1_; } } while (0)
  long long pf_s = 0;
#define SMP2_SUB0() do { if (prof_on) pf_s = clock64(); } while (0)
#define SMP2_SUB(i_) do { if (prof_on) wg.prof[i_] += clock64() - pf_s; } while (0)

  constexpr double FX = 1099511627776.0;
  constexpr double FXC = 1024.0;
  auto fx_add = [&](int v, double x, bool coarse)
  {
    if (fabs(x) < 256.0)
      (void)__hip_atomic_fetch_add(&wg.accfx[v], (unsigned long long)__double2ll_rn(x*FX), __ATOMIC_RELAXED, __HIP_MEMORY_SCOPE_WORKGROUP);
    else if (coarse && fabs(x) < 274877906944.0)
    {
      wg.coarse_ = 1u;
      (void)__hip_atomic_fetch_add(&wg.accfx[v + 1], (unsigned long long)__double2ll_rn(x*FXC), __ATOMIC_RELAXED, __HIP_MEMORY_SCOPE_WORKGROUP);
    }
    else wg.bad_ = 1u;
  };
  uint32_t nx = 0;
  unsigned long long gseq = A.seq0;
#define XT(i_) do { if (prof_on) { const long long t1_ = clock64(); wg.prof[8 + i_] += t1_ - xt0; xt0 = t1_; } } while (0)
  long long xt0 = 0;
  constexpr bool solo = PROG;
  auto xpush = [&](int v0, int nv)
  {
    const uint32_t par = nx & 1u; ++nx;
    unsigned long long * acc = A.xbuf + (size_t)par*XN + (size_t)(b & 7u)*16u;
    if (tid < (uint32_t)nv)
    {
      const unsigned long long fx = wg.accfx[v0 + (int)tid];
      wg.accfx[v0 + (int)tid] = 0ull;
      const unsigned long long old = __hip_atomic_fetch_add(acc + tid, fx, __ATOMIC_RELAXED, __HIP_MEMORY_SCOPE_AGENT);
      asm volatile("s_waitcnt vmcnt(0)" :: "v"(old) : "memory");
    }
    XT(1);
    if (!solo) __syncthreads();
    XT(2);
    if (tid == 0) (void)__hip_atomic_fetch_add(acc + XV, 1ull + ((unsigned long long)wg.bad_ << 32) + ((unsigned long long)wg.coarse_ << 48), __ATOMIC_RELAXED, __HIP_MEMORY_SCOPE_AGENT);
  };
  auto xpoll = [&](int v0, int nv, bool last, bool hold) -> bool
  {
    const uint32_t par = (nx - 1u) & 1u;
    unsigned long long * set = A.xbuf + (size_t)par*XN;
    if (wv == 0)
    {
      const unsigned long long t_wait = wall_clock64();
      const unsigned long long prev0 = wg.xprev[par][lane], prev1 = wg.xprev[par][64u + lane];
// ... 90 lines not shown
    if (hold || solo)
    {
      if (wv == 0 && nval > XV && wg.xbad_) { if (lane < (uint32_t)nval) wg.xtot[lane] = __longlong_as_double(0x7ff8000000000000ll); wsync(); }
      return true;
    }
    if (nval > XV && wg.xbad_)
    {
      __syncthreads();
      if (tid < (uint32_t)nval) wg.xtot[tid] = __longlong_as_double(0x7ff8000000000000ll);
      __syncthreads();
    }
    mine_tot = wg.xtot[want & 31];
    return true;
  };
  auto exchange = [&](int nval, int want, double & mine_tot) -> bool
  {
    exchange_begin(nval);
    return exchange_end(want, mine_tot);
  };
#undef XT

  if constexpr (PROG)
  {
    if (wv == 0)
    {
      Stream<true> g{*A.grng};
      const uint32_t tm = A.theta_mask;
      const int nth = 2*__popc(tm);
      const double qnan = __longlong_as_double(0x7ff8000000000000ll);
      uint32_t cnt_prop = 0, cnt_acc = 0, cnt_gprop = 0, cnt_gacc = 0, ndec = 0;
      uint32_t pj_tau = 0, pj_tau_acc = 0, pj_mix = 0, pj_mix_acc = 0;
      const bool declog = (A.dbg & 256u) && b == 0;
      int q = -1; bool mix = false;
      double tq_old = 0, tq_new = 0, mix_c = 1, mix_lnc = 0, lnprior = 0;
      auto make_step = [&](int stepq)
      {
        mix = stepq == npop; q = mix ? -1 : stepq;
        const double wprop = g.window();
        double tq_lo = 0, tq_hi = 0, minf = 1, maxf = 1, lminf = 0, lmaxf = 0;
        tq_old = 0; tq_new = 0; mix_c = 1; mix_lnc = 0; lnprior = 0;
        if (!mix)
        {
          const int pq = SP.parent[q], cl = SP.left[q], cr = SP.right[q];
          tq_old = wg.tau[q]; tq_lo = fmax(wg.tau[cl], wg.tau[cr]); tq_hi = pq >= 0 ? wg.tau[pq] : 999.0;
          tq_new = reflect(tq_old + SP.ft_tau*wprop, tq_lo, tq_hi);
          minf = (tq_new - tq_lo)/(tq_old - tq_lo); maxf = (tq_new - tq_hi)/(tq_old - tq_hi);
          const double lg = log(lane == 0 ? minf : lane == 1u ? maxf : tq_new/tq_old);
          lminf = __shfl(lg, 0, 64); lmaxf = __shfl(lg, 1, 64);
          if (pq < 0 && SP.tau_alpha > 0) lnprior = (SP.tau_alpha - 1 - (nsp - 1) + 1)*__shfl(lg, 2, 64) - SP.tau_beta*(tq_new - tq_old);
        }
        else { mix_lnc = SP.ft_mix*wprop; mix_c = exp(mix_lnc); }
        if (lane == 0)
        {
          wg.stepp.q = q; wg.stepp.mix = mix ? 1 : 0; wg.stepp.tq_old = tq_old; wg.stepp.tq_lo = tq_lo; wg.stepp.tq_hi = tq_hi; wg.stepp.tq_new = tq_new;
          wg.stepp.minf = minf; wg.stepp.maxf = maxf; wg.stepp.lminf = lminf; wg.stepp.lmaxf = lmaxf; wg.stepp.mix_c = mix_c; wg.stepp.mix_lnc = mix_lnc;
        }
      };
      uint32_t slidem = 0; double tslide = 0;
      auto theta_choices = [&]()
      {
        slidem = 0; tslide = 0;
        for (int p = 0; p < npop; ++p)
          if ((tm >> p) & 1u)
          {
            if (!(g.u() < SP.theta_slide_prob)) continue;
            slidem |= 1u << p;
            const double tn = reflect(wg.tau[MAXPOP + p] + SP.ft_theta*g.window(), 0.0, 999.0);
            if (p == (int)lane) tslide = tn;
          }
      };
      bool aborted = false;
      if (A.do_allloci && A.niter) { make_step(nsp); theta_choices(); }
      __syncthreads();
      for (uint32_t it = 0; it < A.niter && A.do_allloci && !aborted; ++it)
      {
        for (int stepq = nsp; stepq <= npop && !aborted; ++stepq)
        {
          const bool first = stepq == nsp;
          const int base = first ? nth : 0;
          if (mix) { SMP2_SUB0(); g.r = prog_mix_redraw((uint32_t)g.r, tm, mix_c); SMP2_SUB(15); }
          SMP2_TICK(0);
          __syncthreads();
          SMP2_TICK(1);
          double dummy = 0;
          exchange_begin(base + (mix ? 2 : 5));
          SMP2_TICK(2);
          const bool okx = exchange_end(0, dummy);
          SMP2_TICK(3);
          if (!okx) { aborted = true; __syncthreads(); __syncthreads(); break; }
          bool accept = false; double lnacc = 0; uint32_t rd_mask = 0;
          if (first)
          {
            g.r = prog_theta_decide((uint32_t)g.r, tm, slidem, tslide, 1, q, base);
            const uint32_t accm = wg.dec.accm;
            cnt_prop += (uint32_t)__popc(tm); cnt_acc += (uint32_t)__popc(accm);
            cnt_gprop += (uint32_t)__popc(tm & ~slidem); cnt_gacc += (uint32_t)__popc(accm & tm & ~slidem);
            if (declog && lane < (uint32_t)npop && ((tm >> lane) & 1u))
            {
              const uint32_t k = ndec + (uint32_t)__popc(tm & ((1u << lane) - 1u));
              if (k < 1000u) { double * r = A.declog + 4*k; r[0] = (((slidem >> lane) & 1u) ? 100 : 200) + (int)lane; r[1] = wg.dec.lnacc[lane]; r[2] = -1.0; r[3] = (accm >> lane) & 1u ? 1 : 0; }
            }
            ndec += (uint32_t)__popc(tm);
            SMP2_TICK(4);
          }
          if (!mix)
          {
            g.r = prog_tau_decide((uint32_t)g.r, tm, q, base, lnprior, first);
            accept = wg.dec.acc_step != 0u; rd_mask = wg.dec.rd_mask; lnacc = wg.dec.lnacc_step;
          }
          else
          {
            lnacc = (wg.xtot[0] + wg.xtot[1]*(FX/FXC)) + (double)(nsp - 1)*mix_lnc;
            if (SP.tau_alpha > 0)
            {
              const double troot = wg.tau[npop - 1];
              lnacc += (SP.tau_alpha - 1)*mix_lnc - SP.tau_beta*(troot*mix_c - troot) - (double)(nsp - 2)*mix_lnc;
            }
            lnacc += wg.dec.lnacc_theta; rd_mask = wg.dec.rd_mask;
            accept = g.accept(lnacc);
            if (lane == 0) wg.dec.acc_step = accept ? 1u : 0u;
          }
          if (accept && wg.xcoarse_ && b == 0 && lane == 0) (void)atomicAdd(A.err + 2, 1);
          ++cnt_prop; cnt_acc += accept ? 1u : 0u;
          if (mix) { ++pj_mix; pj_mix_acc += accept ? 1u : 0u; } else { ++pj_tau; pj_tau_acc += accept ? 1u : 0u; }
          if (declog && lane == 0 && ndec < 1000u) { double * r = A.declog + 4*ndec; r[0] = mix ? 300 : 200 + q; r[1] = lnacc; r[2] = -1.0; r[3] = accept ? 1 : 0; }
          ++ndec;
          if (accept)
          {
            if (!mix) { if (lane == 0) wg.tau[q] = tq_new; }
            else if (lane < (uint32_t)npop) wg.tau[lane] *= mix_c;
            if (lane < 16u)
            {
              const Redraw r = wg.rd[lane];
              if ((rd_mask >> lane) & 1u) { wg.tau[MAXPOP + lane] = r.tn; wg.tau[2*MAXPOP + lane] = r.l2t; }
              const bool moved = mix ? lane < (uint32_t)npop && ((tm >> lane) & 1u)
                                     : ((tm >> lane) & 1u) && ((int)lane == q || (int)lane == SP.left[q] || (int)lane == SP.right[q]);
              if (moved) { PopFit & f = wg.pf[lane]; f.T = r.T; f.a = r.a; f.b = r.b; f.c = r.c; }
            }
          }
          wsync();
          if (mix) SMP2_TICK(6); else SMP2_TICK(5);
          SMP2_TICK(7);
          __syncthreads();
          if (stepq < npop) make_step(stepq + 1);
          else if (it + 1 < A.niter) { make_step(nsp); theta_choices(); }
          __syncthreads();
        }
      }
      if (!aborted)
      {
        if (lane == 0) wg.late_ = __hip_atomic_load(A.err, __ATOMIC_ACQUIRE, __HIP_MEMORY_SCOPE_AGENT) != 0 ? 1u : 0u;
        __syncthreads();
        if (wg.late_) { aborted = true; if (b == 0 && lane == 0) (void)atomicAdd(A.err + 1, (int)A.niter); }
      }
      if (b == 0)
      {
        if (lane == 0 && !aborted)
        {
          *A.grng = g.r;
          A.counters[0] += cnt_prop; A.counters[1] += cnt_acc; A.counters[2] += cnt_gprop; A.counters[3] += cnt_gacc;
          A.pj[4] += pj_tau; A.pj[5] += pj_tau_acc; A.pj[6] += pj_mix; A.pj[7] += pj_mix_acc;
          A.pj[8] += (cnt_prop - pj_tau - pj_mix) - cnt_gprop; A.pj[9] += (cnt_acc - pj_tau_acc - pj_mix_acc) - cnt_gacc;
        }
        if (!aborted && lane < (uint32_t)(3*MAXPOP)) A.taus[lane] = wg.tau[lane];
        if (prof_on) for (int i = 0; i < 24; ++i) A.prof[(i < 16 ? 0 : (int)A.nwg) + i] = (double)wg.prof[i];
        if (prof_on) for (int i = 0; i < 16; ++i) A.prof[(int)A.nwg + 24 + i] = (double)wg.wsweep[i];
      }
      return;
    }
  }

  const uint32_t t0 = gw < A.nwaves ? A.wave_off[gw] : 0u, nt = gw < A.nwaves ? A.wave_off[gw + 1] - t0 : 0u;
  const bool act = slot < nt;
  const uint32_t task = t0 + (act ? slot : 0u);
  GTree<NT> T;
  Stream<BPP> rng{0};
  double lnl_cur = 0, logpr_cur = 0;
  uint32_t np = 0, pb = 0, nprop_done = 0, nacc = 0, w_nupd = 0, w_nbr = 0, a_nupd = 0, a_nbr = 0, a_neval = 0;
  int gl_i = 0;
  for (int k = 0; k < W; ++k) { T.left.w[k] = T.right.w[k] = T.parent.w[k] = T.pop.w[k] = 0xffffffffu; }
  T.cf = T.pf = 0; T.root = 0; T.tips = 2;
  if (act && nt)
  {
    const Loc & L = A.loc[task];
    const uint32_t flag_now = __hip_atomic_load(A.mix_flag, __ATOMIC_RELAXED, __HIP_MEMORY_SCOPE_AGENT);
    const bool restore_mix = A.epoch != 0u && flag_now == A.epoch;
    const Tree * trp = A.trees + task;
    if (restore_mix) trp = A.snap + task;
    const Tree & tr = *trp;
    const Tree & cur = A.trees[task];
    np = L.np;
    double * g_pmat = L.pmat;
    if (li == 0) { S.rate = L.rate; S.rw = L.rw; S.f[0] = L.f0; S.f[1] = L.f1; S.f[2] = L.f2; S.f[3] = L.f3; }
    gl_i = L.gl[li & 15];
    for (int k = 0; k < W; ++k)
    {
      T.left.w[k] = reinterpret_cast<const uint32_t *>(tr.left)[k]; T.right.w[k] = reinterpret_cast<const uint32_t *>(tr.right)[k];
      T.parent.w[k] = reinterpret_cast<const uint32_t *>(tr.parent)[k]; T.pop.w[k] = reinterpret_cast<const uint32_t *>(tr.pop)[k];
    }
    T.root = tr.root; T.tips = tr.tips; rng.r = cur.rng; lnl_cur = tr.lnl; logpr_cur = tr.logpr;
    const int n = 2*T.tips - 1;
    T.cf = gballot<G>(li >= T.tips && li < n && tr.clv[li] != li, gbase);
    T.pf = gballot<G>(li < n && tr.pmat[li] != li, gbase);
    S.time[li] = li < n ? tr.time[li] : 0.0;
    for (uint32_t i = (uint32_t)li; i < (uint32_t)(4*(2*T.tips - 2)); i += G) (&S.ab[0][0])[i] = g_pmat[i];
  }
  {
    uint32_t acc = 0;
#pragma unroll
    for (int s2 = 0; s2 < LPW; ++s2)
    {
      const uint32_t n2 = (uint32_t)__builtin_amdgcn_readlane((int)np, s2*G);
      if ((uint32_t)s2 == slot) pb = acc;
      acc += n2;
    }
  }
  if (act)
  {
    const Loc & L = A.loc[task];
    const double * g_clv = L.clv;
    for (uint32_t q = (uint32_t)li; q < np; q += G) wl.pat[pb + q] = A.pat[L.pat_off + q];
    const uint32_t nbuf = 2u*(uint32_t)(T.tips - 1);
    for (uint32_t i = (uint32_t)li; i < nbuf*np; i += G)
    {
      const uint32_t c = i/np, q = i - c*np;
      const double2 * src = reinterpret_cast<const double2 *>(g_clv + ((size_t)c*np + q)*4);
      const double2 u = src[0], w = src[1];
      double * d = wl.clv[c][pb + q];
      d[0] = u.x; d[1] = u.y; d[2] = w.x; d[3] = w.y;
    }
  }
  const int tips = T.tips, n = 2*tips - 1;
  const bool inner_i = li >= tips && li < n;

  uint32_t mync = 0; double t2h_cur = 0, t2h_new = 0;
  uint32_t mynodes = 0, mync_new = 0; int mynin_new = 0;
  Op opw[NT - 1]; int nops = 0;
  for (int k = 0; k < NT - 1; ++k) opw[k] = 0;

  auto density_counts = [&]()
  {
    const int pop_i = T.pop[li];
    int below = 0;
#pragma unroll
    for (int q = 0; q < G - 1; ++q)
    {
      const uint32_t m = gballot<G>(inner_i && pop_i == q, gbase);
      if (li == q) mynodes = m;
      below += ((pl.below >> q) & 1u) ? __popc(m) : 0;
    }
    mync_new = (uint32_t)__popc(mynodes);
    mynin_new = gl_i - below;
  };
  auto density_term = [&](const double * tk)
  {
    uint32_t nodes = mynodes;
    const int ncoal = (int)mync_new, nin = mynin_new;
    int steps = ncoal + (pl.ptau >= 0 ? 1 : 0);
    if (nin == steps) --steps;
    double T2h = 0, prev = pl.tau;
    int nn = nin;
#pragma unroll
    for (int k = 0; k < NT; ++k)
      if (k < steps)
      {
        double tkk = pl.ptau;
        if (k < ncoal)
        {
          int best = -1; double tb = 0;
#pragma unroll
          for (int j = 0; j < NT - 1; ++j)
            if (((nodes >> (tips + j)) & 1u) && (best < 0 || tk[j] < tb)) { best = tips + j; tb = tk[j]; }
          tkk = tb; nodes &= ~(1u << best);
        }
        T2h += nn*(nn - 1)*(tkk - prev);
        prev = tkk; --nn;
      }
    double c = 0;
    if (ncoal) c += ncoal*pl.l2t;
    if (T2h) c -= T2h/(pl.theta*1.0);
    S.contrib_new[li] = c; t2h_new = T2h;
  };
  auto evaluate = [&](const Prop & pr, bool with_lnl, double & lp_new) -> double
  {
    double tk[NT - 1];
#pragma unroll
    for (int j = 0; j < NT - 1; ++j) tk[j] = S.time[(tips + j) & (NN - 1)];
    const double myage = S.time[li];
    density_counts();
    if ((pr.chain >> li) & 1u) density_term(tk);
    T.pf ^= pr.brm; T.cf ^= pr.ndm;
    if ((pr.brm >> li) & 1u)
    {
      const int par = T.parent[li];
      const double len = (S.time[par & (NN - 1)] - myage)*1.0;
      double a_, b_;
      jc69_ab(len, S.rate, a_, b_);
      const int pi = T.pidx(li);
      S.ab[pi][0] = a_; S.ab[pi][1] = b_;
    }
    nops = __popc(pr.ndm);
    {
      int rank = 0;
#pragma unroll
      for (int j = 0; j < NT - 1; ++j)
        rank += (((pr.ndm >> (tips + j)) & 1u) && (tk[j] < myage || (tk[j] == myage && tips + j < li))) ? 1 : 0;
      const bool mine = (pr.ndm >> li) & 1u;
#pragma unroll
      for (int k = 0; k < NT - 1; ++k)
        if (k < nops)
        {
          const int x = __ffs(gballot<G>(mine && rank == k, gbase)) - 1;
          const int l = T.left[x], r = T.right[x];
          opw[k] = make_op(T.cidx(x), T.cidx(l), T.pidx(l), T.cidx(r), T.pidx(r));
        }
    }
    wsync();
    double lnl = 0;
    if (with_lnl)
    {
      for (uint32_t base = 0; base < np; base += G)
      {
        const uint32_t q = base + (uint32_t)li; const bool pact = q < np;
        const uint32_t ps = pb + (pact ? q : 0u);
        const uint2 pi = wl.pat[ps];
        double last[4] = {0, 0, 0, 0}; uint32_t last_c = 0xffffffffu;
#pragma unroll
        for (int k = 0; k < NT - 1; ++k)
          if (k < nops)
          {
            const Op o = opw[k];
            const uint32_t opar = (uint32_t)o & 255u, lc = (uint32_t)(o >> 8) & 255u, lp = (uint32_t)(o >> 16) & 255u,
                           rc = (uint32_t)(o >> 24) & 255u, rp = (uint32_t)(o >> 32) & 255u;
            double lv[4], rv[4], x[4], y[4];
            if (lc < (uint32_t)tips) expand_code((pi.y >> (4*lc)) & 15u, lv);
            else if (lc == last_c) { lv[0] = last[0]; lv[1] = last[1]; lv[2] = last[2]; lv[3] = last[3]; }
            else { const double * c = wl.clv[lc - tips][ps]; lv[0] = c[0]; lv[1] = c[1]; lv[2] = c[2]; lv[3] = c[3]; }
            if (rc < (uint32_t)tips) expand_code((pi.y >> (4*rc)) & 15u, rv);
            else if (rc == last_c) { rv[0] = last[0]; rv[1] = last[1]; rv[2] = last[2]; rv[3] = last[3]; }
            else { const double * c = wl.clv[rc - tips][ps]; rv[0] = c[0]; rv[1] = c[1]; rv[2] = c[2]; rv[3] = c[3]; }
            matvec4_ab(S.ab[lp][0], S.ab[lp][1], lv, x);
            matvec4_ab(S.ab[rp][0], S.ab[rp][1], rv, y);
            last[0] = x[0]*y[0]; last[1] = x[1]*y[1]; last[2] = x[2]*y[2]; last[3] = x[3]*y[3]; last_c = opar;
            if (pact) { double * out = wl.clv[opar - tips][ps]; out[0] = last[0]; out[1] = last[1]; out[2] = last[2]; out[3] = last[3]; }
          }
        const double tr_ = dot4_pair(S.f[0], S.f[1], S.f[2], S.f[3], last);
        if (pact) wl.term[ps] = log(0 + tr_*S.rw)*pi.x;
      }
      wsync();
      for (uint32_t base = 0; base < np; base += 8)
      {
        double v[8];
#pragma unroll
        for (int j = 0; j < 8; ++j) v[j] = base + (uint32_t)j < np ? wl.term[pb + base + (uint32_t)j] : 0.0;
#pragma unroll
        for (int j = 0; j < 8; ++j) lnl += v[j];
      }
      lnl = A.bfbeta == 1.0 ? lnl : A.bfbeta == 0.0 ? 0.0 : A.bfbeta*lnl;
    }
    else wsync();
    double lp = 0;
    {
      double v[G];
#pragma unroll
      for (int p = 0; p < G; ++p) v[p] = p < npop ? (((pr.chain >> p) & 1u) ? S.contrib_new[p] : S.contrib[p]) : 0.0;
#pragma unroll
      for (int p = 0; p < G; ++p) lp += v[p];
    }
    lp_new = lp;
    return lnl;
  };
  auto commit_density = [&](uint32_t chain)
  {
    if ((chain >> li) & 1u) { S.contrib[li] = S.contrib_new[li]; t2h_cur = t2h_new; }
    mync = mync_new;
  };

  const uint32_t allpop = (1u << npop) - 1u;
  if (act)
  {
    wsync();
    double tk[NT - 1];
#pragma unroll
    for (int j = 0; j < NT - 1; ++j) tk[j] = S.time[(tips + j) & (NN - 1)];
    density_counts();
    if (li < npop) density_term(tk);
    commit_density(allpop);
    wsync();
    if (A.refresh_logpr)
    {
      double lp = 0;
      for (int p = 0; p < npop; ++p) lp += S.contrib[p];
      logpr_cur = lp;
    }
  }

  const double qnan = __longlong_as_double(0x7ff8000000000000ll);
  uint32_t cnt_prop = 0, cnt_acc = 0;
  uint32_t cnt_gprop = 0, cnt_gacc = 0;
  uint32_t pj_tau = 0, pj_tau_acc = 0, pj_mix = 0, pj_mix_acc = 0, pj_gage = 0, pj_gage_acc = 0;
  const bool declog = (A.dbg & 256u) && b == 0;
  uint32_t ndec = 0;
  const bool wgprof = (A.dbg & 32u) && tid == 0;
  long long wg_sweep = 0;
  bool aborted = false;

  if constexpr (PROG) __syncthreads();
  for (uint32_t it = 0; it < A.niter && !aborted; ++it)
  {
    const uint32_t nprop = A.nsteps_gage + A.nsteps_gspr;
    const long long wg_t0 = wgprof ? clock64() : 0;
    const bool wvprof = (A.dbg & 16u) && b == 0 && lane == 0;
    const long long wv_t0 = wvprof ? clock64() : 0;
    for (uint32_t step = 0; step < nprop; ++step)
    {
      const GTree<NT> U = T;
      double tsave = 0, lnl = 0, lp_new = 0;
      Prop pr{0, 0, 0, 0.0};
      bool ok = false;
      if (act)
      {
        tsave = S.time[li];
        ok = step < A.nsteps_gage
          ? propose_gage<NT, BPP>(T, rng, S.time, (int)step, pl, wg.anc, wg.tau, SP.ft_gage, li, gbase, pr)
          : propose_gspr<NT, BPP>(T, rng, S.time, (int)(step - A.nsteps_gage), pl, gl_i, wg.anc, wg.tau, wg.lograt, SP.ft_gspr, li, gbase, pr);
      }
      SMP2_TICK(0);
      if (ok)
      {
        wsync();
        lnl = evaluate(pr, true, lp_new);
        SMP2_TICK(1);
      }
      if (ok)
      {
        w_nupd += (uint32_t)nops; w_nbr += (uint32_t)__popc(pr.brm);
        const double lnacc = (lp_new - logpr_cur) + (lnl - lnl_cur) + pr.hast;
        ++nprop_done;
        const bool gage_step = step < A.nsteps_gage;
        pj_gage += gage_step ? 1u : 0u;
        if (rng.accept(lnacc)) { lnl_cur = lnl; logpr_cur = lp_new; ++nacc; pj_gage_acc += gage_step ? 1u : 0u; commit_density(pr.chain); }
        else { T = U; S.time[li] = tsave; }
        wsync();
        SMP2_TICK(2);
      }
      else if (act) { T = U; S.time[li] = tsave; wsync(); }
    }
    if (wgprof) wg_sweep += clock64() - wg_t0;
    if (wvprof) wg.wsweep[wv] += clock64() - wv_t0;
    if (!A.do_allloci) continue;

    constexpr bool program = PROG;
    bool mix = false; int q = -1;
    double wprop = 0, uacc = -1.0;
    double tq_old = 0, tq_lo = 0, tq_hi = 0, minf = 1, maxf = 1, lminf = 0, lmaxf = 0, tq_new = 0, mix_c = 1, mix_lnc = 0;
    double lnacc_theta = 0;
    double rd_tn = qnan, rd_l2t = 0, rd_T = 0, rd_a = qnan, rd_b = qnan, rd_c = qnan;
    uint32_t rd_mask = 0;
    uint32_t cf0 = 0, pf0 = 0;
    double tsave = 0, lnl_new = 0, lp_new = 0, lnprior = 0, dl_tot = 0, lnacc = 0;
    bool evaluated = false, accept = false;
    auto step_begin = [&](int stepq)
    {
      rd_mask = 0; lnprior = 0; accept = false; lnacc_theta = 0;
      if constexpr (PROG)
      {
        (void)stepq;
        mix = wg.stepp.mix != 0; q = wg.stepp.q;
        tq_old = wg.stepp.tq_old; tq_lo = wg.stepp.tq_lo; tq_hi = wg.stepp.tq_hi; tq_new = wg.stepp.tq_new;
        minf = wg.stepp.minf; maxf = wg.stepp.maxf; lminf = wg.stepp.lminf; lmaxf = wg.stepp.lmaxf; mix_c = wg.stepp.mix_c; mix_lnc = wg.stepp.mix_lnc;
      }
      else
      {
        mix = stepq == npop;
        q = mix ? -1 : stepq;
        wprop = mix && !BPP ? grng.u() - 0.5 : grng.window(); uacc = BPP ? -1.0 : grng.u();
        tq_old = 0; tq_lo = 0; tq_hi = 0; minf = 1; maxf = 1; lminf = 0; lmaxf = 0; tq_new = 0; mix_c = 1; mix_lnc = 0;
        if (!mix)
        {
          const int pq = SP.parent[q], cl = SP.left[q], cr = SP.right[q];
          tq_old = wg.tau[q]; tq_lo = fmax(wg.tau[cl], wg.tau[cr]); tq_hi = pq >= 0 ? wg.tau[pq] : 999.0;
          tq_new = reflect(tq_old + SP.ft_tau*wprop, tq_lo, tq_hi);
          minf = (tq_new - tq_lo)/(tq_old - tq_lo); maxf = (tq_new - tq_hi)/(tq_old - tq_hi);
          lminf = log(minf); lmaxf = log(maxf);
        }
        else { mix_lnc = SP.ft_mix*wprop; mix_c = exp(mix_lnc); }
      }
      if (!mix)
      {
        if (li == q) pl.tau = tq_new;
        if (pl.parent == q) pl.ptau = tq_new;
      }
      else
      {
        pl.tau *= mix_c;
        if (pl.parent >= 0) pl.ptau *= mix_c;
      }
    };
    auto step_locus = [&](int base)
    {
      cf0 = T.cf; pf0 = T.pf;
      tsave = act ? S.time[li] : 0.0;
      lnl_new = lnl_cur; lp_new = logpr_cur;
      evaluated = false;
      if (act)
      {
        Prop pr{allpop, 0, 0, 0.0};
        double hast = 0, hast2 = 0;
        if (!mix)
        {
          const int cl = SP.left[q], cr = SP.right[q];
          const int pk = T.pop[li];
          const double tk_ = tsave;
          const bool moved = inner_i && (pk == q || pk == cl || pk == cr) && !(tk_ < tq_lo || tk_ > tq_hi);
          const bool up = moved && tk_ >= tq_old;
          if (moved) S.time[li] = up ? tq_hi + maxf*(tk_ - tq_hi) : tq_lo + minf*(tk_ - tq_lo);
          const uint32_t mm = gballot<G>(moved, gbase);
          const int above = __popc(gballot<G>(up, gbase)), below = __popc(mm) - above;
          const int par = T.parent[li];
          pr.brm = gballot<G>(li < n && par >= 0 && (((mm >> li) & 1u) || ((mm >> (par & 31)) & 1u)), gbase);
          uint32_t m = mm;
          const int l = T.left[li], r = T.right[li];
#pragma unroll
          for (int d = 0; d < NT - 2; ++d) m |= gballot<G>(inner_i && (((m >> (l & 31)) & 1u) || ((m >> (r & 31)) & 1u)), gbase);
          pr.ndm = m;
          hast = below*lminf; hast2 = above*lmaxf;
        }
        else
        {
          if (inner_i) S.time[li] = tsave*mix_c;
          pr.ndm = gballot<G>(inner_i, gbase);
          pr.brm = gballot<G>(li < n && (int)T.parent[li] >= 0, gbase);
          hast = (double)(tips - 1)*mix_lnc;
        }
        wsync();
        evaluated = pr.ndm != 0;
        const double lnl = evaluate(pr, evaluated, lp_new);
        if (evaluated) { lnl_new = lnl; a_nupd += (uint32_t)nops; a_nbr += (uint32_t)__popc(pr.brm); ++a_neval; }
        const double dpr = program ? 0.0 : lp_new - logpr_cur;
        const double h = mix ? dpr + hast : (dpr + hast) + hast2;
        const double dl = evaluated ? (lnl_new - lnl_cur) + h : h;
        if (li == 0) fx_add(base, dl, true);
        if (program && !mix && li < npop && ((A.theta_mask >> li) & 1u))
        {
          const int slot = li == q ? 2 : li == SP.left[q] ? 3 : li == SP.right[q] ? 4 : -1;
          if (slot >= 0) fx_add(base + slot, t2h_new, false);
        }
      }
    };
    auto step_decide = [&](int base)
    {
      dl_tot = wg.xtot[base] + wg.xtot[base + 1]*(FX/FXC);
      lnacc = dl_tot;
      if (!mix) lnacc += lnprior;
      else
      {
        lnacc += (double)(nsp - 1)*mix_lnc;
        if (SP.tau_alpha > 0)
        {
          const double troot = wg.tau[npop - 1];
          lnacc += (SP.tau_alpha - 1)*mix_lnc - SP.tau_beta*(troot*mix_c - troot) - (double)(nsp - 2)*mix_lnc;
        }
      }
      accept = BPP ? grng.accept(lnacc) : (lnacc >= 0 || uacc < exp(lnacc));
    };
    auto step_apply = [&](bool refresh)
    {
      if constexpr (!PROG)
      {
        if (accept && wg.xcoarse_ && b == 0 && tid == 0) (void)atomicAdd(A.err + 2, 1);
        ++cnt_prop; cnt_acc += accept ? 1u : 0u;
        if (mix) { ++pj_mix; pj_mix_acc += accept ? 1u : 0u; } else { ++pj_tau; pj_tau_acc += accept ? 1u : 0u; }
        if (declog && tid == 0 && ndec < 1000u) { double * r = A.declog + 4*ndec; r[0] = mix ? 300 : 200 + q; r[1] = lnacc; r[2] = uacc; r[3] = accept ? 1 : 0; }
        ++ndec;
        __syncthreads();
        if (accept)
        {
          if (!mix) { if (tid == 0) wg.tau[q] = tq_new; }
          else if (tid < (uint32_t)npop) wg.tau[tid] *= mix_c;
        }
      }
      if (accept) { if (act) { lnl_cur = lnl_new; logpr_cur = lp_new; commit_density(allpop); } }
      else if (act) { T.cf = cf0; T.pf = pf0; S.time[li] = tsave; }
      if constexpr (!PROG) __syncthreads();
      load_pop();
      wsync();
      if (PROG && (refresh || accept) && act)
      {
        if (li < npop) S.contrib[li] = msc_term((int)mync, t2h_cur, pl.theta, pl.l2t);
        wsync();
        double lp = 0;
        for (int p = 0; p < npop; ++p) lp += S.contrib[p];
        logpr_cur = lp;
        wsync();
      }
    };
    if constexpr (PROG)
    {
      const bool on = li < npop && ((A.theta_mask >> li) & 1u);
      const int kidx = __popc(A.theta_mask & ((1u << li) - 1u)), nth = 2*__popc(A.theta_mask);
      for (int stepq = nsp; stepq <= npop && !aborted; ++stepq)
      {
        const bool first = stepq == nsp;
        step_begin(stepq);
        if (first && act && on) { fx_add(2*kidx, (double)mync, false); fx_add(2*kidx + 1, t2h_cur, false); }
        step_locus(first ? nth : 0);
        __syncthreads();
        __syncthreads();
        const bool ab = wg.abort_ != 0u;
        accept = wg.dec.acc_step != 0u;
        if (!ab) step_apply(first);
        __syncthreads();
        if (ab) { aborted = true; break; }
      }
    }
    else
    {
    if (SP.theta_alpha > 0 && A.theta_mask)
    {
      const bool on = li < npop && ((A.theta_mask >> li) & 1u);
      const double told = pl.theta, l2t_old = pl.l2t;
      double tnew = told, uacc = -1.0, my_lnacc = 0;
      bool accept = false, gibbs_me = false;
      {
        double win = 0;
        for (int p = 0; p < npop; ++p)
          if ((A.theta_mask >> p) & 1u)
          {
            const double w_ = grng.window(), a_ = BPP ? -1.0 : grng.u();
            if (p == li) { win = w_; uacc = a_; }
          }
        tnew = reflect(told + SP.ft_theta*win, 0.0, 999.0);
        const double l2t_new = log(2.0/(1.0*tnew));
        if (act && on) fx_add(li, msc_term((int)mync, t2h_cur, tnew, l2t_new) - msc_term((int)mync, t2h_cur, told, l2t_old), false);
        SMP2_TICK(3);
        double th_tot = 0;
        if (!exchange(npop, li, th_tot)) { aborted = true; break; }
        SMP2_TICK(6);
        if (BPP)
        {
          if (on) { wl.term[li] = tnew; wl.term[16 + li] = told; }
          wsync();
          for (int p = 0; p < npop; ++p)
            if ((A.theta_mask >> p) & 1u)
            {
              const double tn = wl.term[p], to = wl.term[16 + p];
              const double lnacc = wg.xtot[p] + ((SP.theta_alpha - 1)*log(tn/to) - SP.theta_beta*(tn - to));
              const bool acc = tn > 0 && grng.accept(lnacc);
              if (p == li) { accept = acc; my_lnacc = lnacc; }
            }
          wsync();
        }
        else if (on)
        {
          my_lnacc = th_tot + ((SP.theta_alpha - 1)*log(tnew/told) - SP.theta_beta*(tnew - told));
          accept = tnew > 0 && (my_lnacc >= 0 || uacc < exp(my_lnacc));
        }
      }
      const double l2t_new = log(2.0/(1.0*tnew));
      if (accept) { pl.theta = tnew; pl.l2t = l2t_new; }
      if (declog && tid < (uint32_t)G && on)
      {
        const uint32_t k = ndec + (uint32_t)__popc(A.theta_mask & ((1u << li) - 1u));
        if (k < 2048u) { double * r = A.declog + 4*k; r[0] = (gibbs_me ? 200 : 100) + li; r[1] = my_lnacc; r[2] = uacc; r[3] = accept ? 1 : 0; }
      }
      ndec += (uint32_t)__popc(A.theta_mask);
      {
        const uint32_t onm = gballot<G>(on, gbase), accm = gballot<G>(accept, gbase), gm = gballot<G>(on && gibbs_me, gbase);
        cnt_prop += (uint32_t)__popc(onm); cnt_acc += (uint32_t)__popc(accm);
        cnt_gprop += (uint32_t)__popc(gm); cnt_gacc += (uint32_t)__popc(gm & accm);
      }
      __syncthreads();
      if (tid < (uint32_t)G && accept) { wg.tau[MAXPOP + li] = tnew; wg.tau[2*MAXPOP + li] = l2t_new; }
      __syncthreads();
      if (act)
      {
        if (li < npop) S.contrib[li] = msc_term((int)mync, t2h_cur, pl.theta, pl.l2t);
        wsync();
        double lp = 0;
        for (int p = 0; p < npop; ++p) lp += S.contrib[p];
        logpr_cur = lp;
        wsync();
      }
    }
    SMP2_TICK(3);

    for (int stepq = nsp; stepq <= npop && !aborted; ++stepq)
    {
      step_begin(stepq);
      step_locus(0);
      if (mix) SMP2_TICK(5); else SMP2_TICK(4);
      if (!mix && SP.parent[q] < 0 && SP.tau_alpha > 0)
        lnprior = (SP.tau_alpha - 1 - (nsp - 1) + 1)*log(tq_new/tq_old) - SP.tau_beta*(tq_new - tq_old);
      if (!exchange(2, 0, dl_tot)) { aborted = true; break; }
      if (A.dbg & 64u) { SMP2_TICK(7); double dummy; if (!exchange(2, 0, dummy)) { aborted = true; break; } SMP2_TICK(6); }
      SMP2_TICK(7);
      SMP2_SUB0();
      step_decide(0);
      SMP2_SUB(14);
      step_apply(false);
      if (mix) SMP2_TICK(5); else SMP2_TICK(4);
    }
    }
  }
#undef SMP2_TICK
#undef SMP2_SUB0
#undef SMP2_SUB
  if (aborted || wg.abort_) return;
  if constexpr (!PROG) { if (tid == 0) wg.late_ = __hip_atomic_load(A.err, __ATOMIC_ACQUIRE, __HIP_MEMORY_SCOPE_AGENT) != 0 ? 1u : 0u; }
  __syncthreads();
  if (wg.late_)
  {
    if constexpr (!PROG) { if (b == 0 && tid == 0) (void)atomicAdd(A.err + 1, (int)A.niter); }
    return;
  }

  if (act)
  {
    Tree & tr = A.trees[task];
    double * g_clv = A.loc[task].clv, * g_pmat = A.loc[task].pmat;
    {
      uint32_t wl_ = 0, wr_ = 0, wp_ = 0, wq_ = 0;
#pragma unroll
      for (int k = 0; k < W; ++k) if (li == k) { wl_ = T.left.w[k]; wr_ = T.right.w[k]; wp_ = T.parent.w[k]; wq_ = T.pop.w[k]; }
      if (li < W)
      {
        reinterpret_cast<uint32_t *>(tr.left)[li] = wl_; reinterpret_cast<uint32_t *>(tr.right)[li] = wr_;
        reinterpret_cast<uint32_t *>(tr.parent)[li] = wp_; reinterpret_cast<uint32_t *>(tr.pop)[li] = wq_;
      }
    }
    if (li < n) { tr.time[li] = S.time[li]; tr.clv[li] = (int8_t)T.cidx(li); tr.pmat[li] = (int8_t)T.pidx(li); }
    if (li == 0)
    {
      tr.lnl = lnl_cur; tr.logpr = logpr_cur; tr.rng = rng.r; tr.root = T.root;
      tr.proposals += nprop_done; tr.accepted += nacc; tr.sw_nupd += w_nupd; tr.sw_nbr += w_nbr;
      tr.al_nupd += a_nupd; tr.al_nbr += a_nbr; tr.al_neval += a_neval;
      (void)atomicAdd(A.pj + 0, (unsigned long long)pj_gage); (void)atomicAdd(A.pj + 1, (unsigned long long)pj_gage_acc);
      (void)atomicAdd(A.pj + 2, (unsigned long long)(nprop_done - pj_gage)); (void)atomicAdd(A.pj + 3, (unsigned long long)(nacc - pj_gage_acc));
    }
    if (li < npop) { A.pop_nc[(size_t)li*A.ntasks + task] = (int8_t)mync; A.pop_t2h[(size_t)li*A.ntasks + task] = t2h_cur; }
    for (uint32_t i = (uint32_t)li; i < (uint32_t)(4*(2*tips - 2)); i += G) g_pmat[i] = (&S.ab[0][0])[i];
    const uint32_t nbuf = 2u*(uint32_t)(tips - 1);
    for (uint32_t i = (uint32_t)li; i < nbuf*np; i += G)
    {
      const uint32_t c = i/np, q = i - c*np;
      const double * d = wl.clv[c][pb + q];
      double2 u, w; u.x = d[0]; u.y = d[1]; w.x = d[2]; w.y = d[3];
      double2 * dst = reinterpret_cast<double2 *>(g_clv + ((size_t)c*np + q)*4);
      dst[0] = u; dst[1] = w;
    }
  }
  if (b == 0 && tid == 0)
  {
    *A.grng = grng.r;
    A.counters[0] += cnt_prop; A.counters[1] += cnt_acc; A.counters[2] += cnt_gprop; A.counters[3] += cnt_gacc;
    if constexpr (!PROG)
    {
      A.pj[4] += pj_tau; A.pj[5] += pj_tau_acc; A.pj[6] += pj_mix; A.pj[7] += pj_mix_acc;
      A.pj[8] += (cnt_prop - pj_tau - pj_mix) - cnt_gprop; A.pj[9] += (cnt_acc - pj_tau_acc - pj_mix_acc) - cnt_gacc;
    }
  }
  if (b == 0 && tid < (uint32_t)(3*MAXPOP)) A.taus[tid] = wg.tau[tid];
  if (prof_on) for (int i = 0; i < 24; ++i) A.prof[(i < 16 ? 0 : (int)A.nwg) + i] = (double)wg.prof[i];
  if (prof_on) for (int i = 0; i < 16; ++i) A.prof[(int)A.nwg + 24 + i] = (double)wg.wsweep[i];
  if (wgprof) A.prof[16 + b] = (double)wg_sweep;
}

}
```

### include/bpp_amd.h

```cpp
#ifndef BPP_AMD_H
#define BPP_AMD_H

#include <stddef.h>
#include <stdint.h>

#ifdef __cplusplus
extern "C" {
#endif

#define BPA_DATA_DNA          0
#define BPA_DATA_AA           1
#define BPA_DNA_MODEL_JC69    0
#define BPA_DNA_MODEL_K80     1
#define BPA_DNA_MODEL_F81     2
#define BPA_DNA_MODEL_HKY     3
#define BPA_DNA_MODEL_T92     4
#define BPA_DNA_MODEL_TN93    5
#define BPA_DNA_MODEL_F84     6
#define BPA_DNA_MODEL_GTR     7
#define BPA_AA_MODEL_MIN      9
#define BPA_AA_MODEL_LG      10
#define BPA_AA_MODEL_MAX     27

#define BPA_ATTRIB_ARCH_HIP   (1u << 6)
// ... 61 lines not shown
  const int *      right;
  const int *      parent;
  const double *   time;
  const unsigned * clv_index;
  const int *      scaler_index;
  const unsigned * pmatrix_index;
  double           rate_mui;
} bpa_gtree_view_t;
int  bpa_locus_update_all_matrices(bpa_locus_t *, const bpa_gtree_view_t *, double * lengths_out);
int  bpa_locus_update_all_partials(bpa_locus_t *, const bpa_gtree_view_t *);

int  bpa_core_update_pmatrix(bpa_engine_t * engine, double ** pmatrix, unsigned states,
                             unsigned rate_cats, const double * rates,
                             const double * branch_lengths,
                             const unsigned * matrix_indices,
                             const unsigned * param_indices,
                             double * const * eigenvals, double * const * eigenvecs,
                             double * const * inv_eigenvecs, unsigned count,
                             unsigned attrib);
int  bpa_update_eigen(bpa_engine_t * engine, double * eigenvecs, double * inv_eigenvecs,
                      double * eigenvals, const double * freqs,
                      const double * subst_params, unsigned states);
int  bpa_compute_gamma_cats(double alpha, double beta, unsigned categories, double * rates);
int  bpa_compress_site_patterns(char ** sequences, const unsigned * map, int count,
                                int * length, int jc69, unsigned * weights);

int  bpa_locus_get_clv(bpa_locus_t *, unsigned clv_index, double * out);
int  bpa_locus_set_clv(bpa_locus_t *, unsigned clv_index, const double * in);
int  bpa_locus_get_pmatrix(bpa_locus_t *, unsigned pmatrix_index, double * out);
int  bpa_locus_set_pmatrix(bpa_locus_t *, unsigned pmatrix_index, const double * in);
int  bpa_locus_get_scaler(bpa_locus_t *, unsigned scaler_index, unsigned * out);
int  bpa_locus_set_scaler(bpa_locus_t *, unsigned scaler_index, const unsigned * in);
int  bpa_locus_get_eigen(bpa_locus_t *, unsigned index, double * eigenvecs,
                         double * inv_eigenvecs, double * eigenvals);
int  bpa_locus_get_category_rates(bpa_locus_t *, double * out);

typedef struct bpa_batch
{
  unsigned             nloci;
  bpa_locus_t * const * loci;
  const unsigned *     mat_off;
  const unsigned *     mat_pmatrix;
  const double *       mat_length;
  const unsigned *     op_off;
  const bpa_op_t *     ops;
  const unsigned *     root_clv;
  const int *          root_scaler;
} bpa_batch_t;

bpa_plan_t * bpa_plan_create(bpa_engine_t *, const bpa_batch_t *);
void         bpa_plan_destroy(bpa_plan_t *);
int          bpa_plan_set_lengths(bpa_plan_t *, const double * mat_length);
int          bpa_plan_launch(bpa_plan_t *);
int          bpa_plans_launch(bpa_plan_t * const * plans, unsigned count);
int          bpa_plan_get_lnl(bpa_plan_t *, double * lnl);
void *       bpa_plan_lnl_device(bpa_plan_t *);
int          bpa_plan_enable_sum(bpa_plan_t *, void * device_out);
int          bpa_plan_enable_partial_sums(bpa_plan_t *, void * device_out, unsigned * count);
int          bpa_plan_get_sum(bpa_plan_t *, double * sum);
void *       bpa_engine_stage(bpa_engine_t *, const void * host, size_t bytes);
int          bpa_plan_set_params(bpa_plan_t *, int which, const double * values);
int          bpa_plan_set_params_device(bpa_plan_t *, int which, const double * device_values);
int          bpa_batch_evaluate(bpa_engine_t *, const bpa_batch_t *, double * lnl);
int          bpa_batch_begin(bpa_engine_t *, const bpa_batch_t *);
int          bpa_batch_fill(bpa_engine_t *, const bpa_batch_t *, unsigned t0, unsigned t1);
int          bpa_batch_end(bpa_engine_t *, const bpa_batch_t *, double * lnl);
int          bpa_batch_end_async(bpa_engine_t *, const bpa_batch_t *);
int          bpa_batch_wait(bpa_engine_t *, double * lnl);

typedef struct bpa_sampler bpa_sampler_t;
bpa_sampler_t * bpa_sampler_create(bpa_engine_t *, bpa_locus_t * const * loci, unsigned nloci,
                                   unsigned long seed);
void bpa_sampler_destroy(bpa_sampler_t *);
int  bpa_sampler_set_tree(bpa_sampler_t *, unsigned i, const int * left, const int * right,
                          const double * times, int root);
int  bpa_sampler_set_species_tree(bpa_sampler_t *, int species, const int * parent, const double * tau,
                                  const double * theta);
int  bpa_sampler_set_tip_species(bpa_sampler_t *, unsigned i, const int * species);
void bpa_sampler_set_finetune(bpa_sampler_t *, double gage, double gspr, double tau, double mix);
double bpa_finetune_onestep(double pjump, double finetune);
int  bpa_sampler_adapt_finetune(bpa_sampler_t *, double * pjump, double * finetune);
int  bpa_sampler_burnin(bpa_sampler_t *, unsigned iterations, double * finetune);
unsigned bpa_burnin_schedule(unsigned burnin, unsigned * after, unsigned cap);
#define BPA_KERNEL_UNIFORM 0
#define BPA_KERNEL_BPP     1
int  bpa_sampler_set_proposal_kernel(bpa_sampler_t *, int kind);
int  bpa_sampler_set_program_moves(bpa_sampler_t *, int on, double slide_prob);
int  bpa_sampler_gibbs_counters(bpa_sampler_t *, unsigned long * proposals, unsigned long * accepted);
void bpa_sampler_set_tau_prior(bpa_sampler_t *, double alpha, double beta);
void bpa_sampler_set_theta_prior(bpa_sampler_t *, double alpha, double beta, double finetune);
int  bpa_sampler_get_thetas(bpa_sampler_t *, double * theta);
int  bpa_sampler_get_taus(bpa_sampler_t *, double * tau);
#define BPA_SAMPLER_SUMS 16
typedef int (*bpa_allreduce_fn)(void * ctx, double * device_sums, unsigned count, void * stream);
int  bpa_sampler_set_allreduce(bpa_sampler_t *, bpa_allreduce_fn fn, void * ctx, double * device_sums,
                               unsigned first_locus);
struct bpa_p2p;
int  bpa_sampler_set_p2p(bpa_sampler_t *, struct bpa_p2p * p2p, unsigned first_locus);
int  bpa_sampler_initialize(bpa_sampler_t *);
int  bpa_sampler_iterate(bpa_sampler_t *, unsigned iterations);
int  bpa_sampler_get_tree(bpa_sampler_t *, unsigned i, int * left, int * right, int * parent,
                          double * times, int * clv, int * pmat, int * root, double * lnl);
int  bpa_sampler_get_tree_msc(bpa_sampler_t *, unsigned i, int * pop, double * logpr);
int  bpa_sampler_summary(bpa_sampler_t *, double * total_lnl, unsigned long * proposals,
                         unsigned long * accepted, unsigned long * launches);
int  bpa_sampler_set_subst_model(bpa_sampler_t *, unsigned i, const double * freqs , const double * qrates , double alpha);
int  bpa_sampler_get_subst_model(bpa_sampler_t *, unsigned i, double * freqs, double * qrates, double * alpha);
void bpa_sampler_set_subst_moves(bpa_sampler_t *, double ft_freqs, double ft_qrates, double ft_alpha, double alpha_a, double alpha_b);
int  bpa_sampler_set_locus_rates(bpa_sampler_t *, const double * mui );
int  bpa_sampler_get_locus_rates(bpa_sampler_t *, double * mui , double * mubar );
int  bpa_sampler_set_locusrate_moves(bpa_sampler_t *, double ft_mui, double ft_mubar, double a_mui, double a_mubar, double b_mubar, double mubar);
int  bpa_sampler_locusrate_counters(bpa_sampler_t *, unsigned long prop[2], unsigned long acc[2]);
int  bpa_sampler_enable_timing(bpa_sampler_t *, unsigned stride);
int  bpa_sampler_timing(bpa_sampler_t *, double * sweep_ms, unsigned long * sweep_launches,
                        double * allloci_ms, unsigned long * allloci_launches);
int  bpa_sampler_work(bpa_sampler_t *, double * bytes, unsigned long * node_updates,
                      unsigned long * pattern_updates, unsigned long * sweeps);
#define BPA_SAMPLER_SWEEP      0
#define BPA_SAMPLER_GENERIC    1
#define BPA_SAMPLER_PERSISTENT 2
#define BPA_SAMPLER_HYBRID     3
#define BPA_SAMPLER_COMPOSITE  5
#define BPA_SAMPLER_BIG        4
int  bpa_sampler_kind(bpa_sampler_t *);
int  bpa_sampler_streams(bpa_sampler_t *);

int  bpa_plan_work(bpa_plan_t *, double * bytes_partials, double * flops_partials,
                   double * bytes_pmatrix, unsigned long * node_updates,
                   unsigned long * pattern_updates);
void bpa_engine_enable_timing(bpa_engine_t *, int on);
void bpa_engine_set_timing_stride(bpa_engine_t *, unsigned stride);
int  bpa_engine_timing(bpa_engine_t *, double * pmatrix_ms, double * partials_ms,
                       double * reduce_ms, unsigned long * launches);
int  bpa_engine_timing_work(bpa_engine_t *, unsigned long * steps, double * bytes);
int  bpa_plan_work_codes(bpa_plan_t *, double * bytes_codes);
int  bpa_engine_timing_work_codes(bpa_engine_t *, double * bytes_codes);

#define BPA_P2P_HANDLE_BYTES 64
typedef struct bpa_p2p bpa_p2p_t;
bpa_p2p_t *  bpa_p2p_create(bpa_engine_t *, int rank, int world, unsigned max_doubles, void * handle_out);
int          bpa_p2p_connect(bpa_p2p_t *, const void * handles);
int          bpa_p2p_allreduce(bpa_p2p_t *, double * device_values, unsigned n);
int          bpa_plans_launch_exchange(bpa_plan_t * const * plans, unsigned count, bpa_p2p_t *, double * device_values, unsigned n);
void         bpa_p2p_set_timeout(bpa_p2p_t *, unsigned milliseconds);
int          bpa_p2p_status(bpa_p2p_t *);
void         bpa_p2p_destroy(bpa_p2p_t *);

#ifdef __cplusplus
}
#endif
#endif
```

Baseline: 8074 iterations/s.

## Hand over locus sets between waves sharing a SIMD to balance sweep makespan

For the program-moves kernel with 4 taxa, workgroups now hold five locus waves instead of four when the CU count allows it. A host-side simulator picks a schedule in which waves that share a SIMD with a partner (and so run slower) hand their locus sets to waves that run alone at chosen sweep steps. The handover state is parked in extra LDS. The aim is to shorten the slowest wave's gene-tree sweep before the barrier and to pack more loci per workgroup. The cost is larger LDS per workgroup, handover synchronisation, and hard-coded cycle-cost constants that may not match the hardware.

```diff
diff --git a/bpp_amd/api.py b/bpp_amd/api.py
--- a/bpp_amd/api.py
+++ b/bpp_amd/api.py
@@ -131,6 +131,7 @@
         "bpa_sampler_adapt_finetune": (i, [vp, dp, dp]),
         "bpa_sampler_burnin": (i, [vp, u, dp]),
         "bpa_burnin_schedule": (u, [u, C.POINTER(u), u]),
+        "bpa_sweep_schedule": (i, [u, u, d, d, u, C.c_char_p]),
         "bpa_sampler_set_tau_prior": (None, [vp, d, d]),
         "bpa_sampler_set_theta_prior": (None, [vp, d, d, d]),
         "bpa_sampler_get_thetas": (i, [vp, dp]),
@@ -191,7 +192,7 @@
             "bpa_plan_work", "bpa_engine_enable_timing", "bpa_engine_timing", "bpa_engine_set_timing_stride", "bpa_engine_timing_work", "bpa_engine_timing_work_codes", "bpa_plan_work_codes",
             "bpa_sampler_create", "bpa_sampler_destroy", "bpa_sampler_set_tree", "bpa_sampler_initialize",
             "bpa_sampler_set_species_tree", "bpa_sampler_set_tip_species", "bpa_sampler_set_finetune",
-            "bpa_finetune_onestep", "bpa_sampler_adapt_finetune", "bpa_sampler_burnin", "bpa_burnin_schedule",
+            "bpa_finetune_onestep", "bpa_sampler_adapt_finetune", "bpa_sampler_burnin", "bpa_burnin_schedule", "bpa_sweep_schedule",
             "bpa_sampler_set_tau_prior", "bpa_sampler_get_taus", "bpa_sampler_get_tree_msc",
             "bpa_sampler_set_theta_prior", "bpa_sampler_get_thetas", "bpa_sampler_set_allreduce",
             "bpa_sampler_iterate", "bpa_sampler_get_tree", "bpa_sampler_summary",
diff --git a/bpp_amd/csrc/sampler.hpp b/bpp_amd/csrc/sampler.hpp
--- a/bpp_amd/csrc/sampler.hpp
+++ b/bpp_amd/csrc/sampler.hpp
@@ -1086,6 +1086,7 @@
   int v2_retries = 0;
   bool v2_prog = false;
   unsigned v2_nwaves = 0, v2_nwg = 0, v2_lwaves = 0;
+  bool v2_sched_on = false; DevBuf<smp2::Sched> v2_sched;
   size_t v2_lds = 0;
   DevBuf<uint32_t> v2_wave_off;
   DevBuf<smp2::Loc> v2_loc;
@@ -1250,7 +1251,7 @@
   s->g_mui.free(); s->g_mui_old.free(); s->g_lr.free();
   s->b_dev.free(); s->b_undo.free(); s->b_thr.free();
   s->g_ops20.free(); s->g_oprng.free(); s->g_root20.free(); s->g_mtask.free(); s->g_mpm.free(); s->g_tlocus.free(); s->g_tpat.free(); s->g_ttask.free(); s->g_tn0.free(); s->g_rscaler.free();
-  s->v2_wave_off.free(); s->v2_loc.free(); s->v2_pat.free(); s->v2_xbuf.free(); s->v2_grng.free(); s->v2_err.free(); s->v2_prof.free(); s->v2_declog.free(); s->v2_sp.free();
+  s->v2_wave_off.free(); s->v2_loc.free(); s->v2_pat.free(); s->v2_xbuf.free(); s->v2_grng.free(); s->v2_err.free(); s->v2_prof.free(); s->v2_sched.free(); s->v2_declog.free(); s->v2_sp.free();
   delete s;
 }
 
@@ -1376,6 +1377,121 @@
 template <int NT> static size_t v2_lds_base(bool prog)
 {
   return ((sizeof(smp2::WgLDS<NT>) + 15) & ~(size_t)15) + sizeof(smp2::WaveLDS<NT>)*(size_t)(smp2::Cfg<NT>::WAVES - (prog ? 1 : 0));
+}
+template <int NT> static size_t v2_lds_handover(unsigned L)
+{
+  return ((sizeof(smp2::WgLDS<NT>) + 15) & ~(size_t)15) + (sizeof(smp2::WaveLDS<NT>) + (size_t)smp2::Cfg<NT>::PARK*64*sizeof(uint32_t))*(size_t)L;
+}
+
+struct SweepSim { double makespan; bool ok; };
+static SweepSim sweep_simulate(const smp2::Sched & sc, unsigned steps, double c_alone, double c_young)
+{
+  const unsigned R = sc.nroles, nalone = R - 2u*sc.npairs;
+  struct Lane { unsigned seg, left, done_total; double frac; bool waiting, finished; int set; } ln[8];
+  double parked_at[8][smp2::SCHED_SEGS]; int parked_set[8][smp2::SCHED_SEGS]; unsigned set_steps[8];
+  for (unsigned r = 0; r < 8; ++r) for (int k = 0; k < smp2::SCHED_SEGS; ++k) { parked_at[r][k] = -1; parked_set[r][k] = -1; }
+  auto seg_steps = [&](unsigned r, unsigned seg, unsigned done) { return seg + 1u < sc.nseg && done + sc.n[r][seg] < steps ? (unsigned)sc.n[r][seg] : steps - done; };
+  for (unsigned r = 0; r < R; ++r) { set_steps[r] = 0; ln[r] = Lane{0, seg_steps(r, 0, 0), 0, 0.0, false, false, (int)r}; }
+  double t = 0;
+  for (unsigned guard = 0; guard < 4096; ++guard)
+  {
+    bool moved = true;
+    while (moved)
+    {
+      moved = false;
+      for (unsigned r = 0; r < R; ++r)
+      {
+        Lane & l = ln[r];
+        if (l.finished) continue;
+        if (!l.waiting && l.left == 0)
+        {
+          if (l.seg + 1u >= sc.nseg) { l.finished = true; moved = true; continue; }
+          ++l.seg;
+          if (sc.src[r][l.seg] != r) { parked_at[r][l.seg] = t; parked_set[r][l.seg] = l.set; l.set = -1; l.waiting = true; }
+          else l.left = seg_steps(r, l.seg, set_steps[l.set]);
+          moved = true;
+        }
+        if (l.waiting)
+        {
+          const unsigned src = sc.src[r][l.seg];
+          if (src < R && parked_at[src][l.seg] >= 0 && parked_set[src][l.seg] >= 0)
+          {
+            l.set = parked_set[src][l.seg]; parked_set[src][l.seg] = -1; l.waiting = false;
+            l.left = seg_steps(r, l.seg, set_steps[l.set]);
+            moved = true;
+          }
+        }
+      }
+    }
+    double dt = -1; double rate[8];
+    bool any = false;
+    for (unsigned r = 0; r < R; ++r)
+    {
+      const Lane & l = ln[r];
+      rate[r] = 0;
+      if (l.finished || l.waiting || l.left == 0) continue;
+      double c = c_alone;
+      if (r >= nalone && ((r - nalone) & 1u)) { const Lane & o = ln[r - 1]; if (!(o.finished || o.waiting || o.left == 0)) c = c_young; }
+      rate[r] = 1.0/c; any = true;
+      const double need = (1.0 - l.frac)/rate[r];
+      if (dt < 0 || need < dt) dt = need;
+    }
+    if (!any)
+    {
+      bool all = true;
+      for (unsigned r = 0; r < R; ++r) all = all && ln[r].finished;
+      if (!all) return SweepSim{0, false};
+      for (unsigned r = 0; r < R; ++r) if (set_steps[r] != steps) return SweepSim{0, false};
+      return SweepSim{t, true};
+    }
+    t += dt;
+    for (unsigned r = 0; r < R; ++r)
+      if (rate[r] > 0)
+      {
+        Lane & l = ln[r];
+        l.frac += dt*rate[r];
+        if (l.frac >= 1.0 - 1e-12) { l.frac = 0; --l.left; ++set_steps[l.set]; }
+      }
+  }
+  return SweepSim{0, false};
+}
+extern "C" int bpa_sweep_schedule(unsigned lwaves, unsigned steps, double cost_alone, double cost_young, unsigned hand_overs, unsigned char * out)
+{
+  if (!out || lwaves < 1 || lwaves > 8 || steps < 1 || steps > 255 || !(cost_alone > 0) || !(cost_young >= cost_alone)) return 0;
+  smp2::Sched id{};
+  const unsigned npairs = lwaves > 4 ? lwaves - 4 : 0, nalone = lwaves - 2*npairs;
+  id.nseg = 1; id.nroles = (uint8_t)lwaves; id.npairs = (uint8_t)npairs;
+  for (unsigned r = 0; r < 8; ++r) for (int k = 0; k < smp2::SCHED_SEGS; ++k) { id.src[r][k] = (uint8_t)r; id.n[r][k] = 0; }
+  for (unsigned r = 0; r < lwaves; ++r) id.n[r][0] = (uint8_t)steps;
+  if (hand_overs > 3) return 0;
+  smp2::Sched sc = id; double best = 0;
+  const unsigned m = hand_overs, groups = m ? std::min(nalone/m, npairs) : 0u;
+  if (groups)
+  {
+    const SweepSim t_id = sweep_simulate(id, steps, cost_alone, cost_young);
+    best = t_id.ok ? t_id.makespan : 0;
+    for (unsigned d = 1; m*(1 + d) < steps; ++d)
+    {
+      smp2::Sched c = id;
+      c.nseg = (uint8_t)(m + 1);
+      for (unsigned j = 0; j < groups; ++j)
+      {
+        const unsigned y = nalone + 2*j + 1;
+        for (unsigned i = 0; i < m; ++i)
+        {
+          const unsigned ai = j*m + i, q = (i + 1)*(1 + d);
+          c.n[y][i] = 1; c.src[y][i + 1] = (uint8_t)ai; c.n[y][i + 1] = i + 1 < m ? 1 : (uint8_t)(steps - q);
+          c.n[ai][0] = (uint8_t)q;
+          for (unsigned k = 1; k <= i; ++k) c.n[ai][k] = 0;
+          c.src[ai][i + 1] = (uint8_t)y; c.n[ai][i + 1] = (uint8_t)(steps - (i ? i*(1 + d) + 1 : 1));
+        }
+      }
+      const SweepSim t = sweep_simulate(c, steps, cost_alone, cost_young);
+      if (t.ok && t_id.ok && t.makespan < best) { best = t.makespan; sc = c; }
+    }
+  }
+  std::memcpy(out, &sc, sizeof sc);
+  return sc.nseg;
 }
 static bool v2_wants_prog(const bpa_sampler * s)
 {
@@ -1431,23 +1547,30 @@
   HIPCHK(hipGetDeviceProperties(&prop, s->eng->device));
   const unsigned nwaves = (unsigned)woff.size() - 1;
   const unsigned LMAX = WAVES - (prog ? 1u : 0u), ncu = (unsigned)std::max(prop.multiProcessorCount, 1);
-  unsigned LWAVES = (LMAX > 4u && nwaves <= 4u*ncu) ? 4u : LMAX;
+  unsigned LWAVES = (LMAX > 4u && nwaves <= 4u*ncu) ? 4u : (prog && NT == 4 && LMAX >= 5u && nwaves <= 5u*ncu) ? 5u : LMAX;
+  if (s->env_dbg & 4096u) { const unsigned g = (nwaves + LMAX - 1)/LMAX; LWAVES = std::max((nwaves + g - 1)/std::max(g, 1u), 1u); }
   if (const char * ev = BPA_EXP_SWITCH("BPA_SMP_LWAVES")) { const unsigned v = (unsigned)std::atoi(ev); if (v >= 1 && v <= LMAX) LWAVES = v; }
   const unsigned nwg = (nwaves + LWAVES - 1)/LWAVES;
-  const size_t base = NT == 4 ? v2_lds_base<4>(prog) : v2_lds_base<8>(prog);
+  smp2::Sched sched{};
+  const unsigned nprop_sweep = s->env_gage >= 0 ? (unsigned)(s->env_gage + s->env_gspr) : (unsigned)(3*s->maxtips - 3);
+  constexpr double SWEEP_STEP_ALONE = 11.9, SWEEP_STEP_YOUNG = 18.1;
+  bool sched_on = false;
+  if (prog && NT == 4 && LWAVES == 5 && !(s->env_dbg & 8192u) && nprop_sweep <= 255u)
+    sched_on = bpa_sweep_schedule(LWAVES, nprop_sweep, SWEEP_STEP_ALONE, SWEEP_STEP_YOUNG, ((s->env_dbg >> 14) & 3u) ? (s->env_dbg >> 14) & 3u : 3u, reinterpret_cast<unsigned char *>(&sched)) > 1;
+  const size_t base = sched_on ? v2_lds_handover<4>(LWAVES) : NT == 4 ? v2_lds_base<4>(prog) : v2_lds_base<8>(prog);
   const size_t lds_max = std::min<size_t>((size_t)prop.sharedMemPerBlock > 65536 ? (size_t)prop.sharedMemPerBlock : 160*1024, 160*1024) - 256;
   if (base > lds_max) return 1;
   const unsigned per_cu = (unsigned)std::min<size_t>(std::max<size_t>(lds_max/base, 1), 8/WAVES ? 8/WAVES : 1);
   if (nwg > per_cu*(unsigned)prop.multiProcessorCount) return 1;
   s->v2_lds = base;
-  s->v2_nt = NT; s->v2_nwaves = nwaves; s->v2_nwg = nwg; s->v2_prog = prog; s->v2_lwaves = LWAVES;
+  s->v2_nt = NT; s->v2_nwaves = nwaves; s->v2_nwg = nwg; s->v2_prog = prog; s->v2_lwaves = LWAVES; s->v2_sched_on = sched_on;
   const int zero2v[3] = {0, 0, 0};
   if (!upload(s->v2_wave_off, woff.data(), woff.size()) || !upload(s->v2_loc, loc.data(), loc.size()) ||
       !upload(s->v2_pat, pat.data(), pat.size()) || !s->v2_xbuf.reserve((size_t)2*smp2::XN) || !s->v2_grng.reserve(1) ||
-      !upload(s->v2_err, zero2v, 3) || !s->v2_prof.reserve(40 + (size_t)nwg) || !s->v2_declog.reserve(4*2048) || !s->v2_sp.reserve(1) || !s->v2_pj.reserve(16))
+      !upload(s->v2_err, zero2v, 3) || !s->v2_prof.reserve(64 + (size_t)nwg) || !upload(s->v2_sched, &sched, 1) || !s->v2_declog.reserve(4*2048) || !s->v2_sp.reserve(1) || !s->v2_pj.reserve(16))
     return 0;
   HIPCHK(hipMemset(s->v2_pj.p, 0, 16*sizeof(unsigned long long)));
-  HIPCHK(hipMemset(s->v2_prof.p, 0, (40 + (size_t)nwg)*sizeof(double)));
+  HIPCHK(hipMemset(s->v2_prof.p, 0, (64 + (size_t)nwg)*sizeof(double)));
   {
     void (*k0)(const smp2::Args) = NT == 4 ? smp2::iter_kernel<4, false> : smp2::iter_kernel<8, false>;
     void (*k1)(const smp2::Args) = NT == 4 ? smp2::iter_kernel<4, true> : smp2::iter_kernel<8, true>;
@@ -1455,6 +1578,11 @@
     HIPCHK(hipFuncSetAttribute(reinterpret_cast<const void *>(k1), hipFuncAttributeMaxDynamicSharedMemorySize, (int)s->v2_lds));
     void (*k2)(const smp2::Args) = NT == 4 ? smp2::iter_kernel<4, true, true> : smp2::iter_kernel<8, true, true>;
     HIPCHK(hipFuncSetAttribute(reinterpret_cast<const void *>(k2), hipFuncAttributeMaxDynamicSharedMemorySize, (int)s->v2_lds));
+    if (sched_on)
+    {
+      void (*k3)(const smp2::Args) = smp2::iter_kernel<4, true, true, true>;
+      HIPCHK(hipFuncSetAttribute(reinterpret_cast<const void *>(k3), hipFuncAttributeMaxDynamicSharedMemorySize, (int)s->v2_lds));
+    }
   }
   std::memset(&s->v2_sp_sent, 0xff, sizeof s->v2_sp_sent);
   s->v2_ok = true;
@@ -1933,7 +2061,8 @@
   const unsigned x_theta = !theta_mask ? 0u : program ? (2u*(unsigned)__builtin_popcount(theta_mask) + (merged ? 5u : 0u) + XV - 1u)/XV : ((unsigned)npop + XV - 1u)/XV;
   const unsigned x_per_iter = allloci ? x_theta + (unsigned)(npop - S) - (merged ? 1u : 0u) + 1u : 0u;
   const unsigned draws_per_iter = allloci ? 2u*(unsigned)__builtin_popcount(theta_mask) + 2u*(unsigned)(npop - S) + 2u : 0u;
-  void (*kern)(const smp2::Args) = s->v2_prog   ? (s->v2_nt == 4 ? smp2::iter_kernel<4, true, true> : smp2::iter_kernel<8, true, true>)
+  void (*kern)(const smp2::Args) = s->v2_sched_on ? smp2::iter_kernel<4, true, true, true>
+                                 : s->v2_prog   ? (s->v2_nt == 4 ? smp2::iter_kernel<4, true, true> : smp2::iter_kernel<8, true, true>)
                                  : s->kernel_bpp ? (s->v2_nt == 4 ? smp2::iter_kernel<4, true> : smp2::iter_kernel<8, true>)
                                                  : (s->v2_nt == 4 ? smp2::iter_kernel<4, false> : smp2::iter_kernel<8, false>);
   const unsigned bs = s->v2_nt == 4 ? smp2::Cfg<4>::BS : smp2::Cfg<8>::BS;
@@ -1949,6 +2078,7 @@
     a.counters = s->counters.p; a.lograt = s->lograt.p; a.pop_nc = s->pop_nc.p; a.pop_t2h = s->pop_t2h.p;
     a.ntasks = s->nloci; a.nwaves = s->v2_nwaves; a.nwg = s->v2_nwg; a.lwaves = s->v2_lwaves; a.xbuf = s->v2_xbuf.p;
     a.err = s->v2_err.p; a.grng = s->v2_grng.p; a.niter = chunk; a.pj = s->v2_pj.p;
+    a.sched = s->v2_sched.p; a.sched_on = s->v2_sched_on ? 1u : 0u;
     a.nsteps_gage = s->maxtips - 1; a.nsteps_gspr = 2*s->maxtips - 2;
     if (s->env_gage >= 0) { a.nsteps_gage = (uint32_t)s->env_gage; a.nsteps_gspr = (uint32_t)s->env_gspr; }
     a.theta_mask = theta_mask; a.do_allloci = allloci ? 1u : 0u; a.dbg = s->env_dbg;
@@ -2111,6 +2241,14 @@
       fprintf(stderr, "[smp2] sweep cycles of the waves of workgroup 0:");
       for (int w = 0; w < 8; ++w) fprintf(stderr, " %.0f", p2[8 + w]);
       fprintf(stderr, "\n");
+      double p3[17]; HIPCHK(hipMemcpy(p3, s->v2_prof.p + 40 + s->v2_nwg, sizeof p3, hipMemcpyDeviceToHost));
+      fprintf(stderr, "[smp2] %u waves of loci a workgroup, sets change waves: %s%s", s->v2_lwaves, s->v2_sched_on ? "yes" : "no", s->v2_sched_on ? "; cycles waited at hand-overs:" : "\n");
+      if (s->v2_sched_on) {
+      for (int w = 0; w < 8; ++w) fprintf(stderr, " %.0f", p3[w]);
+      fprintf(stderr, " | sweeps of the last wave to reach B1: %.0f | SIMD:role of the waves:", p3[8]);
+      for (int w = 0; w < 8; ++w) { const unsigned v = (unsigned)p3[9 + w]; fprintf(stderr, " %u:%d%s", v & 15u, ((v >> 4) & 255u) == 255u ? -1 : (int)((v >> 4) & 255u), (v & 0x1000u) ? "*" : ""); }
+      fprintf(stderr, "\n");
+      }
       if (s->v2_prog)
         fprintf(stderr, "[smp2] (program-moves kernel: the numbers above are the control wave's — before B1 | wait for the loci | push | poll | THETA decision | TAU decisions | MIX decision | next proposal)\n");
     }
diff --git a/bpp_amd/csrc/sweep2.hpp b/bpp_amd/csrc/sweep2.hpp
--- a/bpp_amd/csrc/sweep2.hpp
+++ b/bpp_amd/csrc/sweep2.hpp
@@ -18,6 +18,7 @@
 #endif
   static constexpr int WAVES = NT <= 4 ? SMP2_WAVES : 4;
   static constexpr int BS    = 64*WAVES;
+  static constexpr int PARK  = 28 + 4*W;
   static_assert(G == NN, "lane i of a group is node i");
 };
 
@@ -28,6 +29,9 @@
   uint32_t np, tips, pat_off, pad;
   int8_t gl[16];
 };
+
+struct Sched { uint8_t nseg, nroles, npairs, pad; uint8_t src[8][4], n[8][4]; };
+constexpr int SCHED_SEGS = 4;
 
 struct Args
 {
@@ -51,6 +55,7 @@
   unsigned char * const * peers; unsigned char * mail; int32_t rank, world; unsigned long long slot_bytes, seq0, spin_limit; int * p2p_err;
   const Species * sp;
   unsigned long long * pj;
+  const Sched * sched; uint32_t sched_on;
 };
 
 constexpr int XN = 128;
@@ -91,7 +96,11 @@
   unsigned long long xprev[2][XN];
   long long prof[24];
   long long wsweep[16];
+  uint32_t roles[8];
   uint32_t xcoarse_, late_;
+  uint32_t simd[8];
+  uint32_t handoff[8][SCHED_SEGS];
+  unsigned long long b1abs; long long hwait[8], b1last;
 };
 
 template <int G> __device__ __forceinline__ uint32_t gballot(bool p, uint32_t gbase)
@@ -545,9 +554,10 @@
   return z;
 }
 
-template <int NT, bool BPP, bool PROG = false>
+template <int NT, bool BPP, bool PROG = false, bool HO = false>
 __global__ void __launch_bounds__(Cfg<NT>::BS) iter_kernel(const Args A)
 {
+  static_assert(!HO || PROG, "sets change waves in the program-moves kernel only");
   using C = Cfg<NT>;
   constexpr int G = C::G, LPW = C::LPW, NN = C::NN, W = C::W, NBUF = C::NBUF, NPM = C::NPM, WAVES = C::WAVES;
   extern __shared__ __attribute__((aligned(16))) unsigned char smem[];
@@ -555,9 +565,9 @@
   WaveLDS<NT> * wl_all = reinterpret_cast<WaveLDS<NT> *>(smem + ((sizeof(WgLDS<NT>) + 15) & ~(size_t)15));
   const uint32_t tid = threadIdx.x, wv = tid >> 6, lane = tid & 63u, b = blockIdx.x;
   const int li = (int)(lane & (uint32_t)(G - 1)); const uint32_t gbase = lane - (uint32_t)li, slot = lane/(uint32_t)G;
-  WaveLDS<NT> & wl = wl_all[PROG ? (wv ? wv - 1u : 0u) : wv];
-  Slot<NT> & S = wl.slot[slot];
   const uint32_t lw = PROG ? wv - 1u : wv;
+  WaveLDS<NT> * wl = wl_all + (PROG ? (wv && !(HO && wv > A.lwaves) ? wv - 1u : 0u) : wv);
+  Slot<NT> * S = &wl->slot[slot];
   const uint32_t gw = lw < A.lwaves ? b*A.lwaves + lw : 0xffffffffu;
   {
     const uint32_t * src = reinterpret_cast<const uint32_t *>(A.sp);
@@ -565,6 +575,13 @@
     for (uint32_t i = tid; i < sizeof(Species)/4; i += C::BS) dst[i] = src[i];
     if (tid < 24u) wg.prof[tid] = 0;
     if (tid < 16u) wg.wsweep[tid] = 0;
+    if constexpr (HO)
+    {
+      if (tid < 8u) { wg.hwait[tid] = 0; wg.roles[tid] = 0xff0u; }
+      if (tid < 8u*SCHED_SEGS) (&wg.handoff[0][0])[tid] = 0u;
+      if (tid == 0) { wg.b1last = 0; wg.b1abs = 0ull; }
+      if (lane == 0) wg.simd[wv & 7u] = (uint32_t)__builtin_amdgcn_s_getreg((1 << 11) | (4 << 6) | 4);
+    }
   }
   __syncthreads();
   const Species & SP = wg.sp;
@@ -821,6 +838,7 @@
           SMP2_TICK(0);
           __syncthreads();
           SMP2_TICK(1);
+          if constexpr (HO) if (wg.abort_) { if (b == 0 && lane == 0) (void)atomicAdd(A.err + 1, (int)A.niter); aborted = true; __syncthreads(); __syncthreads(); break; }
           double dummy = 0;
           exchange_begin(base + (mix ? 2 : 5));
           SMP2_TICK(2);
@@ -904,14 +922,15 @@
         if (!aborted && lane < (uint32_t)(3*MAXPOP)) A.taus[lane] = wg.tau[lane];
         if (prof_on) for (int i = 0; i < 24; ++i) A.prof[(i < 16 ? 0 : (int)A.nwg) + i] = (double)wg.prof[i];
         if (prof_on) for (int i = 0; i < 16; ++i) A.prof[(int)A.nwg + 24 + i] = (double)wg.wsweep[i];
+        if (HO && prof_on) { for (int i = 0; i < 8; ++i) { A.prof[(int)A.nwg + 40 + i] = (double)wg.hwait[i]; A.prof[(int)A.nwg + 49 + i] = (double)wg.roles[i]; } A.prof[(int)A.nwg + 48] = (double)wg.b1last; }
       }
       return;
     }
   }
 
   const uint32_t t0 = gw < A.nwaves ? A.wave_off[gw] : 0u, nt = gw < A.nwaves ? A.wave_off[gw + 1] - t0 : 0u;
-  const bool act = slot < nt;
-  const uint32_t task = t0 + (act ? slot : 0u);
+  bool act = slot < nt;
+  uint32_t task = t0 + (act ? slot : 0u);
   GTree<NT> T;
   Stream<BPP> rng{0};
   double lnl_cur = 0, logpr_cur = 0;
@@ -930,7 +949,7 @@
     const Tree & cur = A.trees[task];
     np = L.np;
     double * g_pmat = L.pmat;
-    if (li == 0) { S.rate = L.rate; S.rw = L.rw; S.f[0] = L.f0; S.f[1] = L.f1; S.f[2] = L.f2; S.f[3] = L.f3; }
+    if (li == 0) { S->rate = L.rate; S->rw = L.rw; S->f[0] = L.f0; S->f[1] = L.f1; S->f[2] = L.f2; S->f[3] = L.f3; }
     gl_i = L.gl[li & 15];
     for (int k = 0; k < W; ++k)
     {
@@ -941,8 +960,8 @@
     const int n = 2*T.tips - 1;
     T.cf = gballot<G>(li >= T.tips && li < n && tr.clv[li] != li, gbase);
     T.pf = gballot<G>(li < n && tr.pmat[li] != li, gbase);
-    S.time[li] = li < n ? tr.time[li] : 0.0;
-    for (uint32_t i = (uint32_t)li; i < (uint32_t)(4*(2*T.tips - 2)); i += G) (&S.ab[0][0])[i] = g_pmat[i];
+    S->time[li] = li < n ? tr.time[li] : 0.0;
+    for (uint32_t i = (uint32_t)li; i < (uint32_t)(4*(2*T.tips - 2)); i += G) (&S->ab[0][0])[i] = g_pmat[i];
   }
   {
     uint32_t acc = 0;
@@ -958,19 +977,19 @@
   {
     const Loc & L = A.loc[task];
     const double * g_clv = L.clv;
-    for (uint32_t q = (uint32_t)li; q < np; q += G) wl.pat[pb + q] = A.pat[L.pat_off + q];
+    for (uint32_t q = (uint32_t)li; q < np; q += G) wl->pat[pb + q] = A.pat[L.pat_off + q];
     const uint32_t nbuf = 2u*(uint32_t)(T.tips - 1);
     for (uint32_t i = (uint32_t)li; i < nbuf*np; i += G)
     {
       const uint32_t c = i/np, q = i - c*np;
       const double2 * src = reinterpret_cast<const double2 *>(g_clv + ((size_t)c*np + q)*4);
       const double2 u = src[0], w = src[1];
-      double * d = wl.clv[c][pb + q];
+      double * d = wl->clv[c][pb + q];
       d[0] = u.x; d[1] = u.y; d[2] = w.x; d[3] = w.y;
     }
   }
-  const int tips = T.tips, n = 2*tips - 1;
-  const bool inner_i = li >= tips && li < n;
+  int tips = T.tips, n = 2*tips - 1;
+  bool inner_i = li >= tips && li < n;
 
   uint32_t mync = 0; double t2h_cur = 0, t2h_new = 0;
   uint32_t mynodes = 0, mync_new = 0; int mynin_new = 0;
@@ -1018,25 +1037,25 @@
     double c = 0;
     if (ncoal) c += ncoal*pl.l2t;
     if (T2h) c -= T2h/(pl.theta*1.0);
-    S.contrib_new[li] = c; t2h_new = T2h;
+    S->contrib_new[li] = c; t2h_new = T2h;
   };
   auto evaluate = [&](const Prop & pr, bool with_lnl, double & lp_new) -> double
   {
     double tk[NT - 1];
 #pragma unroll
-    for (int j = 0; j < NT - 1; ++j) tk[j] = S.time[(tips + j) & (NN - 1)];
-    const double myage = S.time[li];
+    for (int j = 0; j < NT - 1; ++j) tk[j] = S->time[(tips + j) & (NN - 1)];
+    const double myage = S->time[li];
     density_counts();
     if ((pr.chain >> li) & 1u) density_term(tk);
     T.pf ^= pr.brm; T.cf ^= pr.ndm;
     if ((pr.brm >> li) & 1u)
     {
       const int par = T.parent[li];
-      const double len = (S.time[par & (NN - 1)] - myage)*1.0;
+      const double len = (S->time[par & (NN - 1)] - myage)*1.0;
       double a_, b_;
-      jc69_ab(len, S.rate, a_, b_);
+      jc69_ab(len, S->rate, a_, b_);
       const int pi = T.pidx(li);
-      S.ab[pi][0] = a_; S.ab[pi][1] = b_;
+      S->ab[pi][0] = a_; S->ab[pi][1] = b_;
     }
     nops = __popc(pr.ndm);
     {
@@ -1062,7 +1081,7 @@
       {
         const uint32_t q = base + (uint32_t)li; const bool pact = q < np;
         const uint32_t ps = pb + (pact ? q : 0u);
-        const uint2 pi = wl.pat[ps];
+        const uint2 pi = wl->pat[ps];
         double last[4] = {0, 0, 0, 0}; uint32_t last_c = 0xffffffffu;
 #pragma unroll
         for (int k = 0; k < NT - 1; ++k)
@@ -1074,24 +1093,24 @@
             double lv[4], rv[4], x[4], y[4];
             if (lc < (uint32_t)tips) expand_code((pi.y >> (4*lc)) & 15u, lv);
             else if (lc == last_c) { lv[0] = last[0]; lv[1] = last[1]; lv[2] = last[2]; lv[3] = last[3]; }
-            else { const double * c = wl.clv[lc - tips][ps]; lv[0] = c[0]; lv[1] = c[1]; lv[2] = c[2]; lv[3] = c[3]; }
+            else { const double * c = wl->clv[lc - tips][ps]; lv[0] = c[0]; lv[1] = c[1]; lv[2] = c[2]; lv[3] = c[3]; }
             if (rc < (uint32_t)tips) expand_code((pi.y >> (4*rc)) & 15u, rv);
             else if (rc == last_c) { rv[0] = last[0]; rv[1] = last[1]; rv[2] = last[2]; rv[3] = last[3]; }
-            else { const double * c = wl.clv[rc - tips][ps]; rv[0] = c[0]; rv[1] = c[1]; rv[2] = c[2]; rv[3] = c[3]; }
-            matvec4_ab(S.ab[lp][0], S.ab[lp][1], lv, x);
-            matvec4_ab(S.ab[rp][0], S.ab[rp][1], rv, y);
+            else { const double * c = wl->clv[rc - tips][ps]; rv[0] = c[0]; rv[1] = c[1]; rv[2] = c[2]; rv[3] = c[3]; }
+            matvec4_ab(S->ab[lp][0], S->ab[lp][1], lv, x);
+            matvec4_ab(S->ab[rp][0], S->ab[rp][1], rv, y);
             last[0] = x[0]*y[0]; last[1] = x[1]*y[1]; last[2] = x[2]*y[2]; last[3] = x[3]*y[3]; last_c = opar;
-            if (pact) { double * out = wl.clv[opar - tips][ps]; out[0] = last[0]; out[1] = last[1]; out[2] = last[2]; out[3] = last[3]; }
+            if (pact) { double * out = wl->clv[opar - tips][ps]; out[0] = last[0]; out[1] = last[1]; out[2] = last[2]; out[3] = last[3]; }
           }
-        const double tr_ = dot4_pair(S.f[0], S.f[1], S.f[2], S.f[3], last);
-        if (pact) wl.term[ps] = log(0 + tr_*S.rw)*pi.x;
+        const double tr_ = dot4_pair(S->f[0], S->f[1], S->f[2], S->f[3], last);
+        if (pact) wl->term[ps] = log(0 + tr_*S->rw)*pi.x;
       }
       wsync();
       for (uint32_t base = 0; base < np; base += 8)
       {
         double v[8];
 #pragma unroll
-        for (int j = 0; j < 8; ++j) v[j] = base + (uint32_t)j < np ? wl.term[pb + base + (uint32_t)j] : 0.0;
+        for (int j = 0; j < 8; ++j) v[j] = base + (uint32_t)j < np ? wl->term[pb + base + (uint32_t)j] : 0.0;
 #pragma unroll
         for (int j = 0; j < 8; ++j) lnl += v[j];
       }
@@ -1102,7 +1121,7 @@
     {
       double v[G];
 #pragma unroll
-      for (int p = 0; p < G; ++p) v[p] = p < npop ? (((pr.chain >> p) & 1u) ? S.contrib_new[p] : S.contrib[p]) : 0.0;
+      for (int p = 0; p < G; ++p) v[p] = p < npop ? (((pr.chain >> p) & 1u) ? S->contrib_new[p] : S->contrib[p]) : 0.0;
 #pragma unroll
       for (int p = 0; p < G; ++p) lp += v[p];
     }
@@ -1111,7 +1130,7 @@
   };
   auto commit_density = [&](uint32_t chain)
   {
-    if ((chain >> li) & 1u) { S.contrib[li] = S.contrib_new[li]; t2h_cur = t2h_new; }
+    if ((chain >> li) & 1u) { S->contrib[li] = S->contrib_new[li]; t2h_cur = t2h_new; }
     mync = mync_new;
   };
 
@@ -1121,7 +1140,7 @@
     wsync();
     double tk[NT - 1];
 #pragma unroll
-    for (int j = 0; j < NT - 1; ++j) tk[j] = S.time[(tips + j) & (NN - 1)];
+    for (int j = 0; j < NT - 1; ++j) tk[j] = S->time[(tips + j) & (NN - 1)];
     density_counts();
     if (li < npop) density_term(tk);
     commit_density(allpop);
@@ -1129,7 +1148,7 @@
     if (A.refresh_logpr)
     {
       double lp = 0;
-      for (int p = 0; p < npop; ++p) lp += S.contrib[p];
+      for (int p = 0; p < npop; ++p) lp += S->contrib[p];
       logpr_cur = lp;
     }
   }
@@ -1138,6 +1157,117 @@
   uint32_t cnt_prop = 0, cnt_acc = 0;
   uint32_t cnt_gprop = 0, cnt_gacc = 0;
   uint32_t pj_tau = 0, pj_tau_acc = 0, pj_mix = 0, pj_mix_acc = 0, pj_gage = 0, pj_gage_acc = 0;
+  uint32_t step = 0;
+
+  if constexpr (HO)
+  {
+    uint32_t role = 0xffu; bool handover = false;
+    if (A.sched_on && lw < A.lwaves && A.lwaves <= 7u)
+    {
+      const uint32_t L = A.lwaves;
+      uint32_t nalone = 0; bool valid = true;
+      for (uint32_t x = 0; x < L; ++x)
+      {
+        uint32_t cnt = 0;
+        for (uint32_t y = 0; y < L; ++y) cnt += (y != x && wg.simd[y + 1u] == wg.simd[x + 1u]) ? 1u : 0u;
+        valid = valid && cnt <= 1u;
+        nalone += cnt == 0u ? 1u : 0u;
+      }
+      uint32_t ia = 0, ip = 0;
+      for (uint32_t x = 0; x < L; ++x)
+      {
+        int partner = -1;
+        for (uint32_t y = 0; y < L; ++y) if (y != x && wg.simd[y + 1u] == wg.simd[x + 1u]) partner = (int)y;
+        if (partner < 0) { if (x == lw) role = ia; ++ia; }
+        else if ((uint32_t)partner > x)
+        {
+          if (x == lw) role = nalone + 2u*ip;
+          if ((uint32_t)partner == lw) role = nalone + 2u*ip + 1u;
+          ++ip;
+        }
+      }
+      handover = valid && ip == (uint32_t)A.sched->npairs && nalone + 2u*ip == (uint32_t)A.sched->nroles && role < 8u;
+    }
+    if (lane == 0) wg.roles[wv & 7u] = wg.simd[wv & 7u] | (role << 4) | (handover ? 0x1000u : 0u);
+    wsync();
+  }
+  auto park = [&]()
+  {
+    if constexpr (HO) {
+    const uint32_t myset = (uint32_t)(wl - wl_all);
+    uint32_t * r = reinterpret_cast<uint32_t *>(wl_all + A.lwaves) + (size_t)myset*(C::PARK*64) + lane;
+    int k = 0;
+    auto put = [&](uint32_t v) { r[64*k] = v; ++k; };
+    auto putd = [&](double v) { const unsigned long long u = (unsigned long long)__double_as_longlong(v); put((uint32_t)u); put((uint32_t)(u >> 32)); };
+#pragma unroll
+    for (int j = 0; j < W; ++j) { put(T.left.w[j]); put(T.right.w[j]); put(T.parent.w[j]); put(T.pop.w[j]); }
+    put(T.cf); put(T.pf); put((uint32_t)T.root); put((uint32_t)T.tips);
+    put((uint32_t)rng.r); put((uint32_t)((unsigned long long)rng.r >> 32));
+    putd(lnl_cur); putd(logpr_cur); putd(t2h_cur);
+    put(mync); put(np); put(pb); put((uint32_t)gl_i); put(task); put(act ? 1u : 0u);
+    put(nprop_done); put(nacc); put(w_nupd); put(w_nbr); put(a_nupd); put(a_nbr); put(a_neval); put(pj_gage); put(pj_gage_acc);
+    put(step);
+    }
+  };
+  auto pick_up = [&](uint32_t set)
+  {
+    if constexpr (HO) {
+    wl = wl_all + set; S = &wl->slot[slot];
+    const uint32_t * r = reinterpret_cast<const uint32_t *>(wl_all + A.lwaves) + (size_t)set*(C::PARK*64) + lane;
+    int k = 0;
+    auto get = [&]() { const uint32_t v = r[64*k]; ++k; return v; };
+    auto getd = [&]() { const unsigned long long lo = get(), hi = get(); return __longlong_as_double((long long)(lo | (hi << 32))); };
+#pragma unroll
+    for (int j = 0; j < W; ++j) { T.left.w[j] = get(); T.right.w[j] = get(); T.parent.w[j] = get(); T.pop.w[j] = get(); }
+    T.cf = get(); T.pf = get(); T.root = (int32_t)get(); T.tips = (int32_t)get();
+    { const unsigned long long lo = get(), hi = get(); rng.r = (a00_rng_t)(lo | (hi << 32)); }
+    lnl_cur = getd(); logpr_cur = getd(); t2h_cur = getd();
+    mync = get(); np = get(); pb = get(); gl_i = (int)get(); task = get(); act = get() != 0u;
+    nprop_done = get(); nacc = get(); w_nupd = get(); w_nbr = get(); a_nupd = get(); a_nbr = get(); a_neval = get(); pj_gage = get(); pj_gage_acc = get();
+    step = get();
+    tips = T.tips; n = 2*tips - 1; inner_i = li >= tips && li < n;
+    }
+  };
+  auto hand_over = [&](uint32_t role, uint32_t src, uint32_t seg, uint32_t it, bool prof)
+  {
+    if constexpr (HO) {
+    const uint32_t tag = it*(uint32_t)SCHED_SEGS + seg + 1u;
+    park();
+    if (lane == 0) __hip_atomic_store(&wg.handoff[role & 7u][seg & 3u], (tag << 4) | (uint32_t)(wl - wl_all), __ATOMIC_RELEASE, __HIP_MEMORY_SCOPE_WORKGROUP);
+    const long long c0 = prof ? clock64() : 0;
+    const unsigned long long t_wait = wall_clock64();
+    uint32_t v = 0; bool ok = true;
+    for (uint32_t rounds = 1;; ++rounds)
+    {
+      v = __hip_atomic_load(&wg.handoff[src & 7u][seg & 3u], __ATOMIC_ACQUIRE, __HIP_MEMORY_SCOPE_WORKGROUP);
+      if ((v >> 4) == tag) break;
+      if (__hip_atomic_load(&wg.abort_, __ATOMIC_RELAXED, __HIP_MEMORY_SCOPE_WORKGROUP) != 0u) { ok = false; break; }
+      if ((rounds & 63u) == 0 && (wall_clock64() - t_wait > 50000000ull || __hip_atomic_load(A.err, __ATOMIC_RELAXED, __HIP_MEMORY_SCOPE_AGENT) != 0)) { ok = false; break; }
+      __builtin_amdgcn_s_sleep(1);
+    }
+    if (prof) wg.hwait[wv & 7u] += clock64() - c0;
+    const uint32_t set = (uint32_t)__builtin_amdgcn_readfirstlane((int)(v & 15u));
+    if (ok && set < A.lwaves) pick_up(set);
+    else
+    {
+      if (lane == 0) { __hip_atomic_store(&wg.abort_, 1u, __ATOMIC_RELAXED, __HIP_MEMORY_SCOPE_WORKGROUP); (void)__hip_atomic_exchange(A.err, 1, __ATOMIC_RELEASE, __HIP_MEMORY_SCOPE_AGENT); }
+      act = false;
+      if (lane == 0) wg.roles[wv & 7u] &= ~0x1000u;
+    }
+    wsync();
+    }
+  };
+  auto segment_begin = [&](uint32_t seg, uint32_t it, uint32_t nprop, bool prof) -> uint32_t
+  {
+    if constexpr (HO)
+    {
+      const uint32_t role = (wg.roles[wv & 7u] >> 4) & 7u;
+      const uint32_t nseg = A.sched->nseg, src = A.sched->src[role][seg & 3u], nrun = A.sched->n[role][seg & 3u];
+      if (seg && src != role) hand_over(role, src, seg, it, prof);
+      return (wg.roles[wv & 7u] & 0x1000u) && seg + 1u < nseg && step + nrun < nprop ? step + nrun : nprop;
+    }
+    return nprop;
+  };
   const bool declog = (A.dbg & 256u) && b == 0;
   uint32_t ndec = 0;
   const bool wgprof = (A.dbg & 32u) && tid == 0;
@@ -1147,11 +1277,17 @@
   if constexpr (PROG) __syncthreads();
   for (uint32_t it = 0; it < A.niter && !aborted; ++it)
   {
-    const uint32_t nprop = A.nsteps_gage + A.nsteps_gspr;
+    const uint32_t nprop = HO && lw >= A.lwaves ? 0u : A.nsteps_gage + A.nsteps_gspr;
     const long long wg_t0 = wgprof ? clock64() : 0;
     const bool wvprof = (A.dbg & 16u) && b == 0 && lane == 0;
     const long long wv_t0 = wvprof ? clock64() : 0;
-    for (uint32_t step = 0; step < nprop; ++step)
+    step = 0;
+    uint32_t seg = 0;
+    do
+    {
+    uint32_t seg_end = nprop;
+    if constexpr (HO) { if (wg.roles[wv & 7u] & 0x1000u) seg_end = segment_begin(seg, it, nprop, wvprof); ++seg; }
+    for (; step < seg_end; ++step)
     {
       const GTree<NT> U = T;
       double tsave = 0, lnl = 0, lp_new = 0;
@@ -1159,10 +1295,10 @@
       bool ok = false;
       if (act)
       {
-        tsave = S.time[li];
+        tsave = S->time[li];
         ok = step < A.nsteps_gage
-          ? propose_gage<NT, BPP>(T, rng, S.time, (int)step, pl, wg.anc, wg.tau, SP.ft_gage, li, gbase, pr)
-          : propose_gspr<NT, BPP>(T, rng, S.time, (int)(step - A.nsteps_gage), pl, gl_i, wg.anc, wg.tau, wg.lograt, SP.ft_gspr, li, gbase, pr);
+          ? propose_gage<NT, BPP>(T, rng, S->time, (int)step, pl, wg.anc, wg.tau, SP.ft_gage, li, gbase, pr)
+          : propose_gspr<NT, BPP>(T, rng, S->time, (int)(step - A.nsteps_gage), pl, gl_i, wg.anc, wg.tau, wg.lograt, SP.ft_gspr, li, gbase, pr);
       }
       SMP2_TICK(0);
       if (ok)
@@ -1179,14 +1315,21 @@
         const bool gage_step = step < A.nsteps_gage;
         pj_gage += gage_step ? 1u : 0u;
         if (rng.accept(lnacc)) { lnl_cur = lnl; logpr_cur = lp_new; ++nacc; pj_gage_acc += gage_step ? 1u : 0u; commit_density(pr.chain); }
-        else { T = U; S.time[li] = tsave; }
+        else { T = U; S->time[li] = tsave; }
         wsync();
         SMP2_TICK(2);
       }
-      else if (act) { T = U; S.time[li] = tsave; wsync(); }
-    }
+      else if (act) { T = U; S->time[li] = tsave; wsync(); }
+    }
+    } while (HO && step < nprop);
+    (void)seg;
     if (wgprof) wg_sweep += clock64() - wg_t0;
-    if (wvprof) wg.wsweep[wv] += clock64() - wv_t0;
+    if (wvprof)
+    {
+      const long long t1 = clock64();
+      wg.wsweep[wv] += t1 - wv_t0;
+      if constexpr (HO) (void)__hip_atomic_fetch_max(&wg.b1abs, (unsigned long long)t1, __ATOMIC_RELAXED, __HIP_MEMORY_SCOPE_WORKGROUP);
+    }
     if (!A.do_allloci) continue;
 
     constexpr bool program = PROG;
@@ -1239,7 +1382,7 @@
     auto step_locus = [&](int base)
     {
       cf0 = T.cf; pf0 = T.pf;
-      tsave = act ? S.time[li] : 0.0;
+      tsave = act ? S->time[li] : 0.0;
       lnl_new = lnl_cur; lp_new = logpr_cur;
       evaluated = false;
       if (act)
@@ -1253,7 +1396,7 @@
           const double tk_ = tsave;
           const bool moved = inner_i && (pk == q || pk == cl || pk == cr) && !(tk_ < tq_lo || tk_ > tq_hi);
           const bool up = moved && tk_ >= tq_old;
-          if (moved) S.time[li] = up ? tq_hi + maxf*(tk_ - tq_hi) : tq_lo + minf*(tk_ - tq_lo);
+          if (moved) S->time[li] = up ? tq_hi + maxf*(tk_ - tq_hi) : tq_lo + minf*(tk_ - tq_lo);
           const uint32_t mm = gballot<G>(moved, gbase);
           const int above = __popc(gballot<G>(up, gbase)), below = __popc(mm) - above;
           const int par = T.parent[li];
@@ -1267,7 +1410,7 @@
         }
         else
         {
-          if (inner_i) S.time[li] = tsave*mix_c;
+          if (inner_i) S->time[li] = tsave*mix_c;
           pr.ndm = gballot<G>(inner_i, gbase);
           pr.brm = gballot<G>(li < n && (int)T.parent[li] >= 0, gbase);
           hast = (double)(tips - 1)*mix_lnc;
@@ -1320,16 +1463,16 @@
         }
       }
       if (accept) { if (act) { lnl_cur = lnl_new; logpr_cur = lp_new; commit_density(allpop); } }
-      else if (act) { T.cf = cf0; T.pf = pf0; S.time[li] = tsave; }
+      else if (act) { T.cf = cf0; T.pf = pf0; S->time[li] = tsave; }
       if constexpr (!PROG) __syncthreads();
       load_pop();
       wsync();
       if (PROG && (refresh || accept) && act)
       {
-        if (li < npop) S.contrib[li] = msc_term((int)mync, t2h_cur, pl.theta, pl.l2t);
+        if (li < npop) S->contrib[li] = msc_term((int)mync, t2h_cur, pl.theta, pl.l2t);
         wsync();
         double lp = 0;
-        for (int p = 0; p < npop; ++p) lp += S.contrib[p];
+        for (int p = 0; p < npop; ++p) lp += S->contrib[p];
         logpr_cur = lp;
         wsync();
       }
@@ -1345,6 +1488,7 @@
         if (first && act && on) { fx_add(2*kidx, (double)mync, false); fx_add(2*kidx + 1, t2h_cur, false); }
         step_locus(first ? nth : 0);
         __syncthreads();
+        if constexpr (HO) if (first && wvprof && lw == 0u) wg.b1last += (long long)wg.b1abs - wv_t0;
         __syncthreads();
         const bool ab = wg.abort_ != 0u;
         accept = wg.dec.acc_step != 0u;
@@ -1378,12 +1522,12 @@
         SMP2_TICK(6);
         if (BPP)
         {
-          if (on) { wl.term[li] = tnew; wl.term[16 + li] = told; }
+          if (on) { wl->term[li] = tnew; wl->term[16 + li] = told; }
           wsync();
           for (int p = 0; p < npop; ++p)
             if ((A.theta_mask >> p) & 1u)
             {
-              const double tn = wl.term[p], to = wl.term[16 + p];
+              const double tn = wl->term[p], to = wl->term[16 + p];
               const double lnacc = wg.xtot[p] + ((SP.theta_alpha - 1)*log(tn/to) - SP.theta_beta*(tn - to));
               const bool acc = tn > 0 && grng.accept(lnacc);
               if (p == li) { accept = acc; my_lnacc = lnacc; }
@@ -1414,10 +1558,10 @@
       __syncthreads();
       if (act)
       {
-        if (li < npop) S.contrib[li] = msc_term((int)mync, t2h_cur, pl.theta, pl.l2t);
+        if (li < npop) S->contrib[li] = msc_term((int)mync, t2h_cur, pl.theta, pl.l2t);
         wsync();
         double lp = 0;
-        for (int p = 0; p < npop; ++p) lp += S.contrib[p];
+        for (int p = 0; p < npop; ++p) lp += S->contrib[p];
         logpr_cur = lp;
         wsync();
       }
@@ -1468,7 +1612,7 @@
         reinterpret_cast<uint32_t *>(tr.parent)[li] = wp_; reinterpret_cast<uint32_t *>(tr.pop)[li] = wq_;
       }
     }
-    if (li < n) { tr.time[li] = S.time[li]; tr.clv[li] = (int8_t)T.cidx(li); tr.pmat[li] = (int8_t)T.pidx(li); }
+    if (li < n) { tr.time[li] = S->time[li]; tr.clv[li] = (int8_t)T.cidx(li); tr.pmat[li] = (int8_t)T.pidx(li); }
     if (li == 0)
     {
       tr.lnl = lnl_cur; tr.logpr = logpr_cur; tr.rng = rng.r; tr.root = T.root;
@@ -1478,12 +1622,12 @@
       (void)atomicAdd(A.pj + 2, (unsigned long long)(nprop_done - pj_gage)); (void)atomicAdd(A.pj + 3, (unsigned long long)(nacc - pj_gage_acc));
     }
     if (li < npop) { A.pop_nc[(size_t)li*A.ntasks + task] = (int8_t)mync; A.pop_t2h[(size_t)li*A.ntasks + task] = t2h_cur; }
-    for (uint32_t i = (uint32_t)li; i < (uint32_t)(4*(2*tips - 2)); i += G) g_pmat[i] = (&S.ab[0][0])[i];
+    for (uint32_t i = (uint32_t)li; i < (uint32_t)(4*(2*tips - 2)); i += G) g_pmat[i] = (&S->ab[0][0])[i];
     const uint32_t nbuf = 2u*(uint32_t)(tips - 1);
     for (uint32_t i = (uint32_t)li; i < nbuf*np; i += G)
     {
       const uint32_t c = i/np, q = i - c*np;
-      const double * d = wl.clv[c][pb + q];
+      const double * d = wl->clv[c][pb + q];
       double2 u, w; u.x = d[0]; u.y = d[1]; w.x = d[2]; w.y = d[3];
       double2 * dst = reinterpret_cast<double2 *>(g_clv + ((size_t)c*np + q)*4);
       dst[0] = u; dst[1] = w;
@@ -1502,6 +1646,7 @@
   if (b == 0 && tid < (uint32_t)(3*MAXPOP)) A.taus[tid] = wg.tau[tid];
   if (prof_on) for (int i = 0; i < 24; ++i) A.prof[(i < 16 ? 0 : (int)A.nwg) + i] = (double)wg.prof[i];
   if (prof_on) for (int i = 0; i < 16; ++i) A.prof[(int)A.nwg + 24 + i] = (double)wg.wsweep[i];
+  if (HO && prof_on) { for (int i = 0; i < 8; ++i) { A.prof[(int)A.nwg + 40 + i] = (double)wg.hwait[i]; A.prof[(int)A.nwg + 49 + i] = (double)wg.roles[i]; } A.prof[(int)A.nwg + 48] = (double)wg.b1last; }
   if (wgprof) A.prof[16 + b] = (double)wg_sweep;
 }
 
diff --git a/include/bpp_amd.h b/include/bpp_amd.h
--- a/include/bpp_amd.h
+++ b/include/bpp_amd.h
@@ -167,6 +167,7 @@
 int  bpa_sampler_adapt_finetune(bpa_sampler_t *, double * pjump, double * finetune);
 int  bpa_sampler_burnin(bpa_sampler_t *, unsigned iterations, double * finetune);
 unsigned bpa_burnin_schedule(unsigned burnin, unsigned * after, unsigned cap);
+int bpa_sweep_schedule(unsigned lwaves, unsigned steps, double cost_alone, double cost_young, unsigned hand_overs, unsigned char * out);
 #define BPA_KERNEL_UNIFORM 0
 #define BPA_KERNEL_BPP     1
 int  bpa_sampler_set_proposal_kernel(bpa_sampler_t *, int kind);
```

Result: faster. 8263 iterations/s, median of 6 (+2.3%).
